# lh3/minimap2

Hardware: AMD Instinct MI355X
Metric: aligned Gbases/sec (map-ont, 10 kb reads, -a) (higher is better)
Workload: dtype int8 (ksw2 difference DP) / int32+f32 (chaining)

## Files before the change

### minimap2_amd/__init__.py

```python
import ctypes as C
import os

_HERE = os.path.dirname(os.path.abspath(__file__))
LIB_PATH = os.path.join(_HERE, "libmm2amd.so")


class Mm2AmdError(RuntimeError):
    pass


class KswJob(C.Structure):
    _fields_ = [("query", C.c_void_p), ("target", C.c_void_p), ("qlen", C.c_int32), ("tlen", C.c_int32), ("w", C.c_int32),
                ("zdrop", C.c_int32), ("end_bonus", C.c_int32), ("flag", C.c_int32)]


class FinJob(C.Structure):
    _fields_ = [("query", C.c_void_p), ("target", C.c_void_p), ("qlen", C.c_int32), ("tlen", C.c_int32), ("n_pieces", C.c_int32),
                ("piece", C.POINTER(C.POINTER(C.c_uint32))), ("piece_len", C.POINTER(C.c_int32))]


class FinRes(C.Structure):
    _fields_ = [("n_cigar", C.c_int32), ("blen", C.c_int32), ("mlen", C.c_int32), ("n_ambi", C.c_int32), ("dp_max", C.c_int32), ("qshift", C.c_int32),
                ("tshift", C.c_int32), ("is_spliced", C.c_int32), ("cigar_off", C.c_uint32)]

# ... 667 lines not shown
            q_staged.put(None)

        def mapper():
            try:
                k = 0
                while True:
                    b = q_staged.get()
                    if b is None:
                        break
                    m = max(1, len(b.items))
                    n_reg, reg, rep_len, frag_gap = (C.c_int * m)(), (C.c_void_p * m)(), (C.c_int * m)(), (C.c_int * m)()
                    t0 = time.time()
                    _check(L.mm_gpu_map_staged(n_reg, reg, rep_len, frag_gap))
                    if trace is not None:
                        trace.append(("map", k, t0, time.time()))
                    k += 1
                    q_mapped.put((b, n_reg, reg, rep_len))
            except Exception as e:
                errors.append(e)
                while True:
                    L.mm_gpu_batch_discard()
                    try:
                        if q_staged.get(timeout=0.05) is None:
                            break
                    except queue.Empty:
                        pass
            q_mapped.put(None)

        def output():
            k = -1
            while True:
                it = q_mapped.get()
                if it is None:
                    break
                b, n_reg, reg, rep_len = it
                k += 1
                t0 = time.time()
                try:
                    if not errors:
                        if on_mapped:
                            on_mapped(b, n_reg, reg, rep_len)
                        if text:
                            out, out_len = C.c_void_p(), C.c_size_t()
                            _check(L.mm_gpu_format_batch_view(b.n, b.seg_off, b.n_seg, b.arr, n_reg, reg, rep_len, C.byref(out), C.byref(out_len)))
                            total[0] += out_len.value
                            if on_text:
                                on_text(b, out.value, out_len.value)
                except Exception as e:
                    errors.append(e)
                t1 = time.time()
                L.mm2amd_free_regs(len(n_reg), n_reg, reg)
                if trace is not None:
                    trace.append(("output", k, t0, t1)), trace.append(("free", k, t1, time.time()))

        def named(f, nm):
            def g():
                try:
                    C.CDLL(None).prctl(15, nm, 0, 0, 0)
                except Exception:
                    pass
                f()
            return g
        th = [threading.Thread(target=named(f, nm)) for f, nm in ((stager, b"mm2-stager"), (mapper, b"mm2-mapper"), (output, b"mm2-output"))]
        for t in th:
            t.start()
        for t in th:
            t.join()
        self._staged = None
        if errors:
            raise errors[0]
        return total[0]

    def run(self, raw=False, cs=False, MD=False):
        if self._staged is None:
            raise Mm2AmdError("run() without stage()")
        self._active()
        n, _, items, seg_off, n_seg = self._staged
        m = max(1, len(items))
        n_reg, reg, rep_len, frag_gap = (C.c_int * m)(), (C.c_void_p * m)(), (C.c_int * m)(), (C.c_int * m)()
        _check(lib().mm_gpu_map_staged(n_reg, reg, rep_len, frag_gap))
        if raw:
            return n_reg, reg, rep_len
        out = []
        for i in range(n):
            per = []
            for k in range(seg_off[i], seg_off[i] + n_seg[i]):
                regs = C.cast(reg[k], C.POINTER(Reg1)) if n_reg[k] else None
                per.append(_regs_to_alignments(n_reg[k], regs, self.names, self.lens))
            out.append(per[0] if n_seg[i] == 1 else tuple(per))
        try:
            if cs or MD:
                flat = [a for per in out for seg in (per if isinstance(per, tuple) else (per,)) for a in seg]
                segs = [k for i in range(n) for k in range(seg_off[i], seg_off[i] + n_seg[i])]
                ptrs = [reg[k] + j * C.sizeof(Reg1) for k in segs for j in range(n_reg[k])]
                rds = [items[k][1] for k in segs for j in range(n_reg[k])]
                for want, what, field in ((cs, TXT_CS, "cs"), (MD, TXT_MD, "MD")):
                    if want and ptrs:
                        for a, t in zip(flat, hits_text(self._idx, ptrs, rds, what)):
                            setattr(a, field, t or "")
        finally:
            lib().mm2amd_free_regs(len(items), n_reg, reg)
        return out

    def free_raw(self, n_reg, reg):
        lib().mm2amd_free_regs(len(n_reg), n_reg, reg)

    def format_raw(self, n_reg, reg, rep_len=None, device=False):
        n, arr, _, seg_off, n_seg = self._staged
        out, out_len = C.c_void_p(), C.c_size_t()
        if device:
            path = C.c_int(-1)
            _check(lib().mm_gpu_format_batch_dev(n, seg_off, n_seg, arr, n_reg, reg, rep_len, C.byref(out), C.byref(out_len), C.byref(path)))
            self.last_format_path = path.value
            return C.string_at(out, out_len.value)
        _check(lib().mm_gpu_format_batch(n, seg_off, n_seg, arr, n_reg, reg, rep_len, C.byref(out), C.byref(out_len)))
        try:
            return C.string_at(out, out_len.value)
        finally:
            _libc_free(out)

    def map_batch(self, reads, cs=False, MD=False):
        self.stage(reads)
        return self.run(cs=cs, MD=MD)

    def map(self, seq, seq2=None, name="query", cs=False, MD=False):
        if seq2 is not None:
            return self.map_pairs([(name, seq, seq2)], cs=cs, MD=MD)[0]
        return self.map_batch([(name, seq)], cs=cs, MD=MD)[0]

    def seq(self, name, start=0, end=0x7fffffff):
        if not self._idx or self.index_stat()["flag"] & I_NO_SEQ or name not in self.names:
            return None
        rid = self.names.index(name)
        if start < 0 or start >= self.lens[rid] or start >= end:
            return None
        end = min(end, self.lens[rid])
        buf = C.create_string_buffer(end - start)
        rc = lib().mm2amd_idx_getseq(self._idx, rid, start, end, buf)
        if rc < 0:
            _check(rc)
        return buf.raw.translate(_CODE_TO_BASE).decode("ascii")

    def map_pairs(self, pairs, text=False, cs=False, MD=False):
        self.stage(pairs)
        if not text:
            return self.run(cs=cs, MD=MD)
        n_reg, reg, rep_len = self.run(raw=True)
        try:
            return self.format_raw(n_reg, reg, rep_len)
        finally:
            self.free_raw(n_reg, reg)

    def last_stats(self):
        v = (C.c_double * 40)()
        k = lib().mm2amd_last_stats(v, 40)
        names = ["t_seed_chain", "t_host_pre", "t_plan", "t_ksw", "t_consume", "t_finish", "n_jobs", "n_rounds", "dp_cells", "dev_allocs", "pin_allocs",
                 "alloc_ns", "cpu_seed_chain", "cpu_host_pre", "cpu_plan", "cpu_ksw", "cpu_consume", "cpu_finish", "n_long_join_dev", "n_long_join_host",
                 "drv_cpu_seed_chain", "drv_cpu_host_pre", "drv_cpu_plan", "drv_cpu_ksw", "drv_cpu_consume", "drv_cpu_finish", "n_early_sub",
                 "n_region_reads_dev", "n_region_reads_host", "n_band128", "n_band256", "n_band_widened", "n_band_rectangle",
                 "arena_dev_bytes", "arena_pin_bytes", "arena_dev_used", "arena_pin_used", "n_band512", "n_band_rectangle_big"]
        return dict(zip(names, list(v)[:k]))


def band_counters():
    L = lib()
    if not hasattr(L, "mm2amd_alloc_counter"):
        return {"band128": 0, "band256": 0, "widened": 0, "rectangle": 0, "band512": 0, "rectangle_big": 0}
    L.mm2amd_alloc_counter.restype = C.c_longlong
    L.mm2amd_alloc_counter.argtypes = [C.c_int]
    return {"band128": L.mm2amd_alloc_counter(3), "band256": L.mm2amd_alloc_counter(4), "widened": L.mm2amd_alloc_counter(5), "rectangle": L.mm2amd_alloc_counter(6),
            "band512": L.mm2amd_alloc_counter(11), "rectangle_big": L.mm2amd_alloc_counter(12)}


def profile_enable(on=True):
    lib().mm2amd_profile_enable(1 if on else 0)


def profile_get():
    arr = (KernelStat * 64)()
    n = lib().mm2amd_profile_get(arr, 64)
    return {arr[i].name.decode(): {"ms": arr[i].ms, "alg_bytes": arr[i].alg_bytes, "launches": arr[i].launches, "units": arr[i].units} for i in range(n)}
```

### minimap2_amd/csrc/backend_hip.cpp

```cpp
#include <atomic>
#include <condition_variable>
#include <algorithm>
#include <cstdio>
#include <cstring>
#include <memory>
#include <mutex>
#include <numeric>
#include <stdexcept>
#include <thread>
#include "backend.hpp"
#include "chain_dump.hpp"
#include "chain_host.hpp"
#include "device_ctx.hpp"
#include "ksw_host.hpp"
#include "seed_chain_dev.hpp"
#include "index_build.hpp"
#include "kernel_prof.hpp"
#include "threads.hpp"
#include "trace.hpp"
#include "sdust_core.hpp"
#include "sdust.hpp"

namespace mm2amd {

extern const uint8_t kNt4Table[256];

namespace {

bool env_on(const char *name) { const char *e = getenv(name); return e && *e && strcmp(e, "0") != 0; }

struct Lane {
	int id = 0;
	int set = 0;
	hipStream_t stream = nullptr;
	SeedChainBuffers B{};
	KswRunner ksw;
	DevBuf<uint64_t> d_a_off, d_mp_off, d_mz_x, d_mz_y, d_minipos, d_skey_in, d_sval_in, d_skey_out, d_sval_out;
	DevBuf<uint32_t> d_sdust_list;
	DevBuf<SdustCounters> d_sdust_cnt;
	PinBuf<SdustCounters> h_sdust_cnt;
	DevBuf<uint32_t> d_mz_cnt, d_sd_n, d_sd_off, d_sd_aoff, d_sd_qpos, d_sd_info, d_n_anchor, d_n_minipos, d_n_seedhit, d_tie;
	DevBuf<int32_t> d_rep_len, d_f, d_p, d_t;
	DevBuf<Anchor> d_anchors;
	DevBuf<uint8_t> d_tbytes;
	DevBuf<uint32_t> d_sort_list;
	PinBuf<uint32_t> h_sort_list;
	DevBuf<uint32_t> d_pieces;
	PinBuf<uint32_t> h_pieces, h_lj_pieces;
	DevBuf<Anchor> d_lj_out_a;
	DevBuf<uint64_t> d_lj_src;
	PinBuf<Anchor> h_lj_a;
	PinBuf<uint64_t> h_lj_u, h_lj_off, h_lj_aoff, h_lj_uoff;
	PinBuf<int32_t> h_lj_nu, h_lj_nv;
	PinBuf<uint32_t> h_lj_tie, h_lj_list;
	PinBuf<unsigned long long> h_lj_cursor;
	DevBuf<FinRegion> d_fin_regions; DevBuf<FinPiece> d_fin_pieces; DevBuf<uint32_t> d_fin_out; DevBuf<FinResult> d_fin_res;
	PinBuf<FinRegion> h_fin_regions; PinBuf<FinPiece> h_fin_pieces; PinBuf<uint32_t> h_fin_out; PinBuf<FinResult> h_fin_res;
	long rg_lo = 0; size_t rg_n = 0; uint64_t rg_n_v = 0, rg_n_v2 = 0, rg_n_u = 0, rg_n_u2 = 0;
	std::vector<int8_t> rg_src; std::vector<uint64_t> rg_aoff, rg_uoff; std::vector<int32_t> rg_nu, rg_nv;
	DevBuf<uint64_t> d_lj_out_u;
	bool rg_lazy = false;
	DevBuf<int32_t> d_span; PinBuf<int32_t> h_span;
	DevBuf<RgnGather> d_gather; PinBuf<RgnGather> h_gather; DevBuf<Anchor> d_fetch_a; DevBuf<uint64_t> d_fetch_mp; PinBuf<Anchor> h_fetch_a; PinBuf<uint64_t> h_fetch_mp;
	DevBuf<RgnRead> d_rg_reads; PinBuf<RgnRead> h_rg_reads;
	DevBuf<Anchor> d_rg_sq; DevBuf<ref::Reg1> d_rg_regs; DevBuf<RgnAux> d_rg_aux; DevBuf<RgnReadOut> d_rg_rout; DevBuf<unsigned int> d_rg_cur;
	DevBuf<RgnPlan> d_rg_plan; DevBuf<RgnWin> d_rg_win; DevBuf<KswJob> d_rg_jobs; DevBuf<int32_t> d_rg_sites; DevBuf<FinRegion> d_rg_fin; DevBuf<FinPiece> d_rg_pieces;
	DevBuf<FinResult> d_rg_finres; DevBuf<uint32_t> d_rg_out;
	PinBuf<ref::Reg1> h_rg_regs; PinBuf<RgnAux> h_rg_aux; PinBuf<RgnReadOut> h_rg_rout; PinBuf<unsigned int> h_rg_cur; PinBuf<RgnPlan> h_rg_plan; PinBuf<KswJob> h_rg_jobs;
	PinBuf<FinRegion> h_rg_fin; PinBuf<FinResult> h_rg_finres; PinBuf<uint32_t> h_rg_out;
	PinBuf<Anchor> h_anchors, h_redo;
	PinBuf<int32_t> h_rep, h_nu, h_nv;
	PinBuf<uint64_t> h_minipos, h_off, h_u, h_aoff, h_uoff;
	PinBuf<unsigned long long> h_cursor;
	DevBuf<unsigned long long> d_bt_cursor;
	DevBuf<Anchor> d_bt_out_a;
	DevBuf<uint64_t> d_bt_out_u, d_bt_aoff, d_bt_uoff;
	DevBuf<int32_t> d_bt_nu, d_bt_nv;
	PinBuf<uint32_t> h_na, h_nmp, h_dust_n, h_dust_s, h_dust_e, h_tie;
	std::vector<uint64_t> a_off, mp_off;
	~Lane() { if (stream) (void)hipStreamDestroy(stream); }
};

class HipBackend : public Backend {
public:
	HipBackend(const FlatIndex &fi, DeviceIndexTables *tables, int n_threads, int device, int replica, int tables_device) : T_(tables)
	{
		replica_ = replica;
		DeviceCtx &d = device_ctx(device);
		std::lock_guard<std::mutex> lk(d.mu);
		ensure_device(d);
		dev_ = d.device_id;
		stream_ = d.stream;
		n_cu_ = d.n_cu;
		n_threads_ = n_threads > 0 ? n_threads : (int)std::max(1u, std::thread::hardware_concurrency());
		if (!T_) { own_.upload(fi, stream_); T_ = &own_; }
		else if (tables_device >= 0 && tables_device != dev_) { own_.clone_from(*T_, tables_device, dev_); T_ = &own_; }
		I_.bucket_start = T_->bucket_start.p, I_.keys = T_->keys.p, I_.val_off = T_->val_off.p, I_.slots = T_->slots.p, I_.first = getenv("MM2AMD_NO_FIRST_SLOT") ? nullptr : T_->first.p, I_.pos = T_->pos.p, I_.S = T_->S.p;
		I_.bucket_bits = T_->bucket_bits, I_.key_shift = T_->key_shift;
		I_.name_rank = nullptr, I_.seq_len = nullptr;
		fi_names_ = &fi.names, fi_seq_len_ = &fi.seq_len, fi_seq_off_ = &fi.seq_off;
		while ((1ull << rid_bits_) < fi.n_seq) ++rid_bits_;
		n_lanes_ = 8;
		if (const char *e = getenv("MM2AMD_LANES")) n_lanes_ = std::max(1, std::min(kMaxProfLanes - 1, atoi(e)));
		for (int i = 0; i < n_lanes_; ++i) {
			lanes_.emplace_back(new Lane);
			lanes_.back()->id = i;
			HIP_CHECK(hipStreamCreateWithFlags(&lanes_.back()->stream, hipStreamNonBlocking));
			lanes_.back()->ksw.n_cu = n_cu_;
			lanes_.back()->ksw.disable_fast = getenv("MM2AMD_KSW_EXACT_ONLY") != nullptr;
		}
		{
			size_t free_b = 0, total_b = 0, want = arena_env_gb("MM2AMD_ARENA_DEV_GB", 112) << 30;
			if (hipMemGetInfo(&free_b, &total_b) == hipSuccess) want = std::min(want, free_b / 2);
			const size_t want_pin = arena_env_gb("MM2AMD_ARENA_PIN_GB", 4) << 30;
			const int dev = dev_;
			if (MemArena::enabled() && (want || want_pin)) std::thread([dev, want, want_pin] {
				if (hipSetDevice(dev) != hipSuccess) return;
				try { pin_arena().reserve(want_pin); dev_arena().reserve(want); } catch (...) {}
			}).detach();
		}
	}

	~HipBackend() override
	{
		(void)hipSetDevice(dev_);
		if (stage_stream_) (void)hipStreamDestroy(stage_stream_);
		for (int l = 0; l < n_lanes_; ++l) kernel_profiler(l, replica_).drop_events();
		kernel_profiler(kMaxProfLanes - 1, replica_).drop_events();
	}
	int n_lanes() const override { return n_lanes_; }
	void enable_name_rules() override
	{
		HIP_CHECK(hipSetDevice(dev_));
		if (name_rules_ || fi_names_->empty()) return;
		const std::vector<std::string> &nm = *fi_names_;
		sorted_names_ = nm;
		std::sort(sorted_names_.begin(), sorted_names_.end());
		sorted_names_.erase(std::unique(sorted_names_.begin(), sorted_names_.end()), sorted_names_.end());
		std::vector<int32_t> rank(nm.size());
		for (size_t i = 0; i < nm.size(); ++i) rank[i] = (int32_t)(std::lower_bound(sorted_names_.begin(), sorted_names_.end(), nm[i]) - sorted_names_.begin());
		d_name_rank_.ensure(nm.size()), d_ref_len_.ensure(nm.size());
		HIP_CHECK(hipMemcpyAsync(d_name_rank_.p, rank.data(), nm.size() * 4, hipMemcpyHostToDevice, stream_));
		HIP_CHECK(hipMemcpyAsync(d_ref_len_.p, fi_seq_len_->data(), nm.size() * 4, hipMemcpyHostToDevice, stream_));
		stream_wait(stream_);
		I_.name_rank = d_name_rank_.p, I_.seq_len = d_ref_len_.p;
		name_rules_ = true;
	}
	void enable_seq_len() override
	{
		HIP_CHECK(hipSetDevice(dev_));
		if (I_.seq_len) return;
		d_ref_len_.ensure(fi_seq_len_->size());
		HIP_CHECK(hipMemcpyAsync(d_ref_len_.p, fi_seq_len_->data(), fi_seq_len_->size() * 4, hipMemcpyHostToDevice, stream_));
		stream_wait(stream_);
		I_.seq_len = d_ref_len_.p;
	}
	bool supports_rmq() const override { return getenv("MM2AMD_RMQ_ON_HOST") == nullptr; }
	void set_active_lanes(int n) override { active_lanes_ = std::max(1, std::min(n, n_lanes_)); }

	void begin_batch(const std::vector<ReadView> &reads, std::vector<uint64_t> &qpool_off) override
	{
		HIP_CHECK(hipSetDevice(dev_));
		Resident &R = res_[1 - cur_];
		if (!stage_stream_) HIP_CHECK(hipStreamCreateWithFlags(&stage_stream_, hipStreamNonBlocking));
		hipStream_t stream_ = stage_stream_;
		std::vector<uint64_t> &seq_off_ = R.seq_off, &unit_off_ = R.unit_off;
		std::vector<int32_t> &unit_first_ = R.unit_first, &name_key_ = R.name_key;
		bool &has_pairs_ = R.has_pairs, &have_read_names_ = R.have_read_names;
		size_t &n_units_ = R.n_units;
		PinBuf<char> &h_ascii_ = R.h_ascii;
		DevBuf<uint8_t> &d_qpool_ = R.d_qpool;
		DevBuf<uint64_t> &d_seq_off_ = R.d_seq_off, &d_unit_off_ = R.d_unit_off;
		DevBuf<int32_t> &d_unit_first_ = R.d_unit_first, &d_name_key_ = R.d_name_key;
		std::vector<const char *> &read_names_ = R.read_names;
		const size_t n = reads.size();
		seq_off_.resize(n + 1);
		seq_off_[0] = 0;
		has_pairs_ = false;
		for (size_t i = 0; i < n; ++i) seq_off_[i + 1] = seq_off_[i] + (uint64_t)reads[i].total(), has_pairs_ |= reads[i].paired();
		const uint64_t total = seq_off_[n];
		qpool_off.resize(n);
		for (size_t i = 0; i < n; ++i) qpool_off[i] = 2 * seq_off_[i];
		char *h = h_ascii_.ensure(total + 1);
		parallel_for_side(n_threads_, (long)n, [&](long i, int) {
			memcpy(h + seq_off_[i], reads[i].seq, reads[i].len);
			if (reads[i].paired()) memcpy(h + seq_off_[i] + reads[i].len, reads[i].seq2, reads[i].len2);
		}, 64);
		d_qpool_.ensure(2 * total + 16);
		d_seq_off_.ensure(n + 1);
		n_units_ = n;
		if (has_pairs_) {
			unit_first_.resize(n + 1);
			unit_first_[0] = 0;
			for (size_t i = 0; i < n; ++i) unit_first_[i + 1] = unit_first_[i] + (reads[i].paired() ? 2 : 1);
			n_units_ = (size_t)unit_first_[n];
			unit_off_.resize(n_units_ + 1);
			for (size_t i = 0; i < n; ++i) {
				unit_off_[unit_first_[i]] = seq_off_[i];
				if (reads[i].paired()) unit_off_[unit_first_[i] + 1] = seq_off_[i] + (uint64_t)reads[i].len;
			}
			unit_off_[n_units_] = total;
			d_unit_off_.ensure(n_units_ + 1), d_unit_first_.ensure(n + 1);
			HIP_CHECK(hipMemcpyAsync(d_unit_off_.p, unit_off_.data(), (n_units_ + 1) * 8, hipMemcpyHostToDevice, stream_));
			HIP_CHECK(hipMemcpyAsync(d_unit_first_.p, unit_first_.data(), (n + 1) * 4, hipMemcpyHostToDevice, stream_));
		}
		HIP_CHECK(hipMemcpyAsync(d_seq_off_.p, seq_off_.data(), (n + 1) * 8, hipMemcpyHostToDevice, stream_));
		read_names_.clear();
		if (getenv("MM2AMD_SEED_DUMP") || chain_dump_path()) for (size_t i = 0; i < n; ++i) read_names_.push_back(reads[i].name);
		have_read_names_ = false;
		if (name_rules_ && n > 0) {
			have_read_names_ = true;
			for (size_t i = 0; i < n; ++i) if (!reads[i].name) { have_read_names_ = false; break; }
		}
		if (have_read_names_) {
			name_key_.resize(2 * n);
			parallel_for_side(n_threads_, (long)n, [&](long i, int) {
				const std::string q(reads[i].name);
				const size_t lb = (size_t)(std::lower_bound(sorted_names_.begin(), sorted_names_.end(), q) - sorted_names_.begin());
				name_key_[i] = (int32_t)lb;
				name_key_[n + i] = lb < sorted_names_.size() && sorted_names_[lb] == q ? (int32_t)lb : -1;
			}, 256);
			d_name_key_.ensure(2 * n);
			HIP_CHECK(hipMemcpyAsync(d_name_key_.p, name_key_.data(), 2 * n * 4, hipMemcpyHostToDevice, stream_));
		}
		stream_wait(stream_);
	}
	void activate_batch() override { cur_ = 1 - cur_; }
	int current_set() const override { return cur_; }
	void bind_lane(int lane, int set) override { lanes_.at(lane)->set = set; }
	bool stages_beside_mapping() const override { return true; }

	void seed_chain(const SeedChainParams &P, long lo, long hi, int lane_id, int n_threads, std::vector<ReadChains> &out) override
	{
		HIP_CHECK(hipSetDevice(dev_));
		Lane &ln = *lanes_.at(lane_id);
		hipStream_t st = ln.stream;
		SeedChainBuffers &B = ln.B;
		const Resident &R = res_[ln.set];
		const std::vector<uint64_t> &seq_off_ = R.seq_off, &unit_off_ = R.unit_off;
		const std::vector<int32_t> &unit_first_ = R.unit_first;
		const bool has_pairs_ = R.has_pairs, have_read_names_ = R.have_read_names;
		const DevBuf<uint8_t> &d_qpool_ = R.d_qpool;
		const DevBuf<uint64_t> &d_seq_off_ = R.d_seq_off, &d_unit_off_ = R.d_unit_off;
		const DevBuf<int32_t> &d_unit_first_ = R.d_unit_first, &d_name_key_ = R.d_name_key;
		const PinBuf<char> &h_ascii_ = R.h_ascii;
		const std::vector<const char *> &read_names_ = R.read_names;
		const size_t n = (size_t)(hi - lo);
		out.clear();
		out.resize(n);
		if (n == 0) return;
		B = SeedChainBuffers();
		B.n_reads = (int)n, B.seq_off = d_seq_off_.p + lo, B.ascii = h_ascii_.p, B.qpool = d_qpool_.p;
		if (have_read_names_) B.name_lb = d_name_key_.p + lo, B.name_eq = d_name_key_.p + seq_off_.size() - 1 + lo;
		KernelProfiler &kp = kernel_profiler(lane_id, replica_);
		double tt = Trace::now();
		const double L = (double)(seq_off_[hi] - seq_off_[lo]);
		SeedChainBuffers Bu = B;
		const size_t ulo = has_pairs_ ? (size_t)unit_first_[lo] : (size_t)lo, n_unit = has_pairs_ ? (size_t)unit_first_[hi] - ulo : n;
		if (has_pairs_) Bu.n_reads = (int)n_unit, Bu.seq_off = d_unit_off_.p + ulo;
		kp.begin(st); launch_encode(Bu, st); kp.end(st, "encode_kernel", 3 * L);
		const uint64_t base0 = seq_off_[lo], cap_mz = seq_off_[hi] - base0;
		ln.d_mz_cnt.ensure(n_unit);
		ln.d_mz_x.ensure(cap_mz + 1), ln.d_mz_y.ensure(cap_mz + 1);
		ln.d_sd_n.ensure(cap_mz + 1), ln.d_sd_off.ensure(cap_mz + 1), ln.d_sd_aoff.ensure(cap_mz + 1), ln.d_sd_qpos.ensure(cap_mz + 1), ln.d_sd_info.ensure(cap_mz + 1);
		B.mz_cnt = ln.d_mz_cnt.p, B.mz_off = B.seq_off, B.mz_x = ln.d_mz_x.p - base0, B.mz_y = ln.d_mz_y.p - base0;
		B.sd_n = ln.d_sd_n.p - base0, B.sd_off = ln.d_sd_off.p - base0, B.sd_aoff = ln.d_sd_aoff.p - base0, B.sd_qpos = ln.d_sd_qpos.p - base0, B.sd_info = ln.d_sd_info.p - base0;
		const double est_mz = 2.0 * L / (P.w + 1);
		Bu.mz_cnt = B.mz_cnt, Bu.mz_off = Bu.seq_off, Bu.mz_x = B.mz_x, Bu.mz_y = B.mz_y;
		int max_len = 0;
		for (size_t u = 0; u < n_unit; ++u) {
			const uint64_t l_u = has_pairs_ ? unit_off_[ulo + u + 1] - unit_off_[ulo + u] : seq_off_[lo + u + 1] - seq_off_[lo + u];
			max_len = (int)std::max<uint64_t>((uint64_t)max_len, l_u);
		}
		kp.begin(st); launch_sketch(Bu, P, max_len, st); kp.end(st, "sketch_kernel", L + 16.0 * est_mz);
		if (has_pairs_)
			B.unit_first = d_unit_first_.p + lo, B.unit_off = d_unit_off_.p, B.unit_cnt = ln.d_mz_cnt.p - ulo, B.mz_cnt = nullptr;
		const bool dev_sdust = P.sdust_thres > 0 && env_on("MM2AMD_DEVICE_SDUST"), sdust_no_narrow = env_on("MM2AMD_SDUST_NO_NARROW");
		if (dev_sdust) {
			ln.d_sdust_list.ensure(n_unit), ln.d_sdust_cnt.ensure(1);
			HIP_CHECK(hipMemsetAsync(ln.d_sdust_cnt.p, 0, sizeof(SdustCounters), st));
			SdustParams S;
			S.codes = B.qpool, S.off = Bu.seq_off, S.code_mul = 2, S.n_reads = (int)n_unit, S.T = P.sdust_thres < kSdustMaxT ? P.sdust_thres : kSdustMaxT;
			S.reg_n = B.sd_n, S.reg_s = B.sd_off, S.reg_e = B.sd_aoff, S.wide_list = ln.d_sdust_list.p, S.cnt = ln.d_sdust_cnt.p;
			const char *e_cap = getenv("MM2AMD_SDUST_NARROW_CAP");
			const long cap = e_cap && *e_cap ? strtol(e_cap, nullptr, 10) : kSdustNarrowCap;
			if (sdust_no_narrow) {
				S.cap = kSdustWideCap, S.wide = 2;
				kp.begin(st); sdust_launch(S, 0, st); kp.end(st, "sdust_kernel[wide]", 0.0);
			} else {
				S.cap = (int)(cap < 1 ? 1 : cap > kSdustWideCap ? kSdustWideCap : cap), S.wide = 0;
				kp.begin(st); sdust_launch(S, 0, st); kp.end(st, "sdust_kernel[narrow]", 0.0);
				S.cap = kSdustWideCap, S.wide = 1;
				kp.begin(st); sdust_launch(S, 0, st); kp.end(st, "sdust_kernel[wide]", 0.0);
			}
			HIP_CHECK(hipMemcpyAsync(ln.h_sdust_cnt.ensure(1), ln.d_sdust_cnt.p, sizeof(SdustCounters), hipMemcpyDeviceToHost, st));
			kp.begin(st); launch_dust_filter(B, st); kp.end(st, "dust_filter_kernel", 16.0 * est_mz);
		} else if (P.sdust_thres > 0) {
			uint32_t *h_n = ln.h_dust_n.ensure(cap_mz + 1), *h_s = ln.h_dust_s.ensure(cap_mz + 1), *h_e = ln.h_dust_e.ensure(cap_mz + 1);
			const char *asc = h_ascii_.p;
			parallel_for(n_threads, (long)n_unit, [&](long u, int) {
				const uint64_t o = has_pairs_ ? unit_off_[ulo + u] : seq_off_[lo + u];
				const int len = (int)((has_pairs_ ? unit_off_[ulo + u + 1] : seq_off_[lo + u + 1]) - o);
				thread_local std::vector<SdustState::Perf> perf(SdustState::PCAP);
				thread_local std::vector<uint8_t> codes;
				codes.resize((size_t)len + 1);
				for (int j = 0; j < len; ++j) codes[j] = kNt4Table[(uint8_t)asc[o + j]];
				SdustState S;
				S.P = perf.data();
				uint32_t k = 0;
				sdust_scan(codes.data(), len, P.sdust_thres, S, [&](int s0, int e0) { h_s[o - base0 + k] = (uint32_t)s0, h_e[o - base0 + k] = (uint32_t)e0; ++k; });
				if (len > 0) h_n[o - base0] = k;
			}, 16);
			HIP_CHECK(hipMemcpyAsync(ln.d_sd_n.p, h_n, cap_mz * 4, hipMemcpyHostToDevice, st));
			HIP_CHECK(hipMemcpyAsync(ln.d_sd_off.p, h_s, cap_mz * 4, hipMemcpyHostToDevice, st));
			HIP_CHECK(hipMemcpyAsync(ln.d_sd_aoff.p, h_e, cap_mz * 4, hipMemcpyHostToDevice, st));
			kp.begin(st); launch_dust_filter(B, st); kp.end(st, "dust_filter_kernel", 16.0 * est_mz);
		}
		ln.d_n_anchor.ensure(n), ln.d_n_minipos.ensure(n), ln.d_n_seedhit.ensure(n), ln.d_rep_len.ensure(n);
		B.n_anchor = ln.d_n_anchor.p, B.n_minipos = ln.d_n_minipos.p, B.n_seedhit = ln.d_n_seedhit.p, B.rep_len = ln.d_rep_len.p;
		kp.begin(st); launch_seed_collect(B, I_, P, st); kp.end(st, "seed_collect_kernel", 36.0 * est_mz);
		uint32_t *h_na = ln.h_na.ensure(n), *h_nmp = ln.h_nmp.ensure(n);
		int32_t *h_rep = ln.h_rep.ensure(n);
		HIP_CHECK(hipMemcpyAsync(h_na, ln.d_n_anchor.p, n * 4, hipMemcpyDeviceToHost, st));
		HIP_CHECK(hipMemcpyAsync(h_nmp, ln.d_n_minipos.p, n * 4, hipMemcpyDeviceToHost, st));
		HIP_CHECK(hipMemcpyAsync(h_rep, ln.d_rep_len.p, n * 4, hipMemcpyDeviceToHost, st));
		stream_wait(st);
		if (dev_sdust) {
			const SdustCounters &c = *ln.h_sdust_cnt.p;
			if (c.err) throw HipError("[mm2amd] sdust_kernel: a list of perfect intervals outgrew the wide capacity");
			kp.add_units("sdust_kernel[wide]", (double)c.wide_bases);
			if (!sdust_no_narrow) kp.add_units("sdust_kernel[narrow]", L - (double)c.wide_bases + (double)c.narrow_partial);
		}
		Trace::get().add(lane_id, "gpu:sketch+collect", tt, Trace::now()); tt = Trace::now();
		std::vector<uint64_t> &a_off = ln.a_off, &mp_off = ln.mp_off;
		a_off.resize(n + 1), mp_off.resize(n + 1);
		a_off[0] = mp_off[0] = 0;
		for (size_t i = 0; i < n; ++i) a_off[i + 1] = a_off[i] + h_na[i], mp_off[i + 1] = mp_off[i] + h_nmp[i];
		const uint64_t n_a = a_off[n], n_mp = mp_off[n];
		uint64_t *h_off = ln.h_off.ensure(2 * (n + 1));
		memcpy(h_off, a_off.data(), (n + 1) * 8), memcpy(h_off + n + 1, mp_off.data(), (n + 1) * 8);
		ln.d_a_off.ensure(n + 1), ln.d_mp_off.ensure(n + 1);
		HIP_CHECK(hipMemcpyAsync(ln.d_a_off.p, h_off, (n + 1) * 8, hipMemcpyHostToDevice, st));
		HIP_CHECK(hipMemcpyAsync(ln.d_mp_off.p, h_off + n + 1, (n + 1) * 8, hipMemcpyHostToDevice, st));
		ln.d_anchors.ensure(n_a + 1), ln.d_minipos.ensure(n_mp + 1), ln.d_f.ensure(n_a + 1), ln.d_p.ensure(n_a + 1), ln.d_t.ensure(n_a + 1);
		ln.d_skey_in.ensure(n_a + 1), ln.d_sval_in.ensure(n_a + 1), ln.d_skey_out.ensure(n_a + 1), ln.d_sval_out.ensure(n_a + 1), ln.d_tie.ensure(2 * n + 1);
		B.sort_key_in = ln.d_skey_in.p, B.sort_val_in = ln.d_sval_in.p, B.sort_key_out = ln.d_skey_out.p, B.sort_val_out = ln.d_sval_out.p, B.tie_flag = ln.d_tie.p;
		B.tie_list = ln.d_tie.p + n, B.tie_count = ln.d_tie.p + 2 * n;
		B.rid_bits = rid_bits_;
		int n_class[kAnchorSortClasses] = { 0 }, class_first[kAnchorSortClasses + 1] = { 0 };
		double a_class[kAnchorSortClasses] = { 0 };
		for (size_t i = 0; i < n; ++i) if (h_na[i]) { const int c = anchor_sort_class(h_na[i], rid_bits_); ++n_class[c], a_class[c] += h_na[i]; }
		for (int c = 0; c < kAnchorSortClasses; ++c) class_first[c + 1] = class_first[c] + n_class[c];
		uint32_t *h_list = ln.h_sort_list.ensure(n + 1);
		{
			int fill[kAnchorSortClasses];
			for (int c = 0; c < kAnchorSortClasses; ++c) fill[c] = class_first[c];
			for (size_t i = 0; i < n; ++i) if (h_na[i]) h_list[fill[anchor_sort_class(h_na[i], rid_bits_)]++] = (uint32_t)i;
		}
		ln.d_sort_list.ensure(n + 1);
		if (class_first[kAnchorSortClasses]) HIP_CHECK(hipMemcpyAsync(ln.d_sort_list.p, h_list, (size_t)class_first[kAnchorSortClasses] * 4, hipMemcpyHostToDevice, st));
		B.a_off = ln.d_a_off.p, B.mp_off = ln.d_mp_off.p, B.anchors = ln.d_anchors.p, B.mini_pos = ln.d_minipos.p;
		B.f = ln.d_f.p, B.p = ln.d_p.p, B.t = ln.d_t.p;
		kp.begin(st); launch_seed_expand(B, I_, P, st); kp.end(st, "seed_expand_kernel", 24.0 * n_a);
		launch_anchor_sort(B, I_, P, ln.d_sort_list.p, n_class, a_class, st, &kp);
		if (getenv("MM2AMD_TIE_COUNT")) {
			std::vector<uint32_t> tf(n);
			stream_wait(st);
			HIP_CHECK(hipMemcpy(tf.data(), ln.d_tie.p, n * 4, hipMemcpyDeviceToHost));
			size_t n_tied = 0;
			for (size_t i = 0; i < n; ++i) n_tied += tf[i] != 0;
			fprintf(stderr, "[mm2amd] anchor sort: %zu of %zu reads have duplicated keys (%d / %d / %d reads in the 7 k / 10 k / global classes)\n", n_tied, n, n_class[3], n_class[4], n_class[5]);
		}
		if (const char *dump = getenv("MM2AMD_SEED_DUMP")) {
			std::vector<Anchor> all(n_a + 1);
			stream_wait(st);
			if (n_a) HIP_CHECK(hipMemcpy(all.data(), ln.d_anchors.p, n_a * sizeof(Anchor), hipMemcpyDeviceToHost));
			static std::mutex dump_mu;
			std::lock_guard<std::mutex> lk(dump_mu);
			const bool dump_flags = getenv("MM2AMD_SEED_DUMP_FLAGS") != nullptr;
			if (FILE *fp = fopen(dump, "a")) {
				for (size_t i = 0; i < n; ++i) {
					fprintf(fp, "QR\t%s\t%d\nRS\t%d\n", read_names_.empty() || !read_names_[lo + i] ? "*" : read_names_[lo + i], P.mid_occ, h_rep[i]);
					for (uint64_t j = a_off[i]; j < a_off[i + 1]; ++j) {
						const Anchor &a = all[j];
						fprintf(fp, "SD\t%s\t%d\t%c\t%d\t%d\t%d", (*fi_names_)[a.x << 1 >> 33].c_str(), (int32_t)a.x, "+-"[a.x >> 63], (int32_t)a.y, (int32_t)(a.y >> 32 & 0xff),
						        j == a_off[i] ? 0 : ((int32_t)a.y - (int32_t)all[j - 1].y) - ((int32_t)a.x - (int32_t)all[j - 1].x));
						if (dump_flags) fprintf(fp, "\t%d", (int)(a.y >> 42 & 1));
						fputc('\n', fp);
					}
				}
				fclose(fp);
			}
		}
		const char *cdump = P.chain_dump ? chain_dump_path() : nullptr;
		auto dump_block = [&](size_t i) {
			ChainDumpBlock b;
			b.name = read_names_.empty() ? nullptr : read_names_[lo + i];
			b.qlen = (int)(seq_off_[lo + i + 1] - seq_off_[lo + i]), b.n_seg = has_pairs_ ? unit_first_[lo + i + 1] - unit_first_[lo + i] : 1;
			return b;
		};
		if (P.anchors_only) {
			Anchor *ha = ln.h_anchors.ensure(n_a + 1);
			uint64_t *hmp = ln.h_minipos.ensure(n_mp + 1);
			if (n_a) HIP_CHECK(hipMemcpyAsync(ha, ln.d_anchors.p, n_a * sizeof(Anchor), hipMemcpyDeviceToHost, st));
			if (n_mp) HIP_CHECK(hipMemcpyAsync(hmp, ln.d_minipos.p, n_mp * 8, hipMemcpyDeviceToHost, st));
			stream_wait(st);
			Trace::get().add(lane_id, "gpu:expand+sort, d2h:anchors", tt, Trace::now());
			kp.collect();
			if (cdump) {
				std::string txt;
				for (size_t i = 0; i < n; ++i) {
					ChainDumpBlock b = dump_block(i);
					b.handed_back = true, b.in = ha + a_off[i], b.n_in = (int64_t)(a_off[i + 1] - a_off[i]);
					chain_dump_format(txt, P, b);
				}
				chain_dump_flush(cdump, txt);
			}
			parallel_for(n_threads, (long)n, [&](long i, int) {
				ReadChains &c = out[i];
				c.rep_len = h_rep[i];
				c.mp_p = hmp + mp_off[i], c.n_mp = (int32_t)(mp_off[i + 1] - mp_off[i]);
				c.u_p = nullptr, c.n_u = 0, c.chained = false;
				c.a_p = ha + a_off[i], c.n_a = (int64_t)(a_off[i + 1] - a_off[i]);
			}, 64);
			return;
		}
		make_pieces(B, ln, ln.h_pieces, n, [&](size_t i) { return (uint64_t)h_na[i]; }, P.rmq ? rmq_piece_len() : fill_piece_len(), st);
		if (P.rmq) { kp.begin(st); launch_chain_rmq(B, P, st); kp.end(st, "chain_rmq_kernel", 32.0 * n_a); }
		else { kp.begin(st); launch_chain_fill(B, P, st); kp.end(st, "chain_fill_kernel", 24.0 * n_a); }
		B.pieces = nullptr, B.n_pieces = 0;
		ln.d_bt_cursor.ensure(2), ln.d_bt_out_a.ensure(n_a + 1), ln.d_bt_out_u.ensure((P.min_cnt >= 2 ? n_a / 2 : n_a) + n + 1);
		ln.d_bt_nu.ensure(n), ln.d_bt_nv.ensure(n), ln.d_bt_aoff.ensure(n), ln.d_bt_uoff.ensure(n);
		B.bt_cursor = ln.d_bt_cursor.p, B.bt_out_a = ln.d_bt_out_a.p, B.bt_out_u = ln.d_bt_out_u.p;
		B.bt_nu = ln.d_bt_nu.p, B.bt_nv = ln.d_bt_nv.p, B.bt_aoff = ln.d_bt_aoff.p, B.bt_uoff = ln.d_bt_uoff.p;
		kp.begin(st); launch_chain_backtrack(B, P, st); kp.end(st, "chain_backtrack_kernel", 8.0 * n_a);
		unsigned long long *h_cur = ln.h_cursor.ensure(2);
		int32_t *h_nu = ln.h_nu.ensure(n), *h_nv = ln.h_nv.ensure(n);
		uint64_t *h_aoff = ln.h_aoff.ensure(n), *h_uoff = ln.h_uoff.ensure(n);
		uint64_t *hmp = ln.h_minipos.ensure(n_mp + 1);
		uint32_t *h_tie = P.rmq ? ln.h_tie.ensure(n) : nullptr;
		HIP_CHECK(hipMemcpyAsync(h_cur, ln.d_bt_cursor.p, 16, hipMemcpyDeviceToHost, st));
		HIP_CHECK(hipMemcpyAsync(h_nu, ln.d_bt_nu.p, n * 4, hipMemcpyDeviceToHost, st));
		HIP_CHECK(hipMemcpyAsync(h_nv, ln.d_bt_nv.p, n * 4, hipMemcpyDeviceToHost, st));
		HIP_CHECK(hipMemcpyAsync(h_aoff, ln.d_bt_aoff.p, n * 8, hipMemcpyDeviceToHost, st));
		HIP_CHECK(hipMemcpyAsync(h_uoff, ln.d_bt_uoff.p, n * 8, hipMemcpyDeviceToHost, st));
		if (h_tie) HIP_CHECK(hipMemcpyAsync(h_tie, ln.d_tie.p, n * 4, hipMemcpyDeviceToHost, st));
		const bool lazy = P.lazy_chains != 0 && !P.anchors_only;
		ln.rg_lazy = lazy;
		int32_t *h_span = nullptr;
		if (lazy) {
			ln.d_span.ensure(2 * n), h_span = ln.h_span.ensure(2 * n);
			launch_first_chain_span((int)n, ln.d_bt_out_a.p, ln.d_bt_out_u.p, ln.d_bt_aoff.p, ln.d_bt_uoff.p, ln.d_bt_nu.p, ln.d_span.p, st);
			HIP_CHECK(hipMemcpyAsync(h_span, ln.d_span.p, 2 * n * 4, hipMemcpyDeviceToHost, st));
		} else if (n_mp) HIP_CHECK(hipMemcpyAsync(hmp, ln.d_minipos.p, n_mp * 8, hipMemcpyDeviceToHost, st));
		stream_wait(st);
		Trace::get().add(lane_id, "gpu:expand..backtrack", tt, Trace::now()); tt = Trace::now();
		const uint64_t n_v = h_cur[0], n_u = h_cur[1];
		Anchor *ha = ln.h_anchors.ensure(n_v + 1);
		uint64_t *hu = ln.h_u.ensure(n_u + 1);
		if (n_v && !lazy) HIP_CHECK(hipMemcpyAsync(ha, ln.d_bt_out_a.p, n_v * sizeof(Anchor), hipMemcpyDeviceToHost, st));
		if (n_u) HIP_CHECK(hipMemcpyAsync(hu, ln.d_bt_out_u.p, n_u * 8, hipMemcpyDeviceToHost, st));
		std::vector<std::pair<size_t, size_t>> redo;
		size_t redo_total = 0;
		if (h_tie) for (size_t i = 0; i < n; ++i) if (h_tie[i]) redo.emplace_back(i, redo_total), redo_total += (size_t)(a_off[i + 1] - a_off[i]);
		Anchor *h_redo = redo_total ? ln.h_redo.ensure(redo_total + 1) : nullptr;
		for (const auto &rd : redo) {
			const size_t cnt = (size_t)(a_off[rd.first + 1] - a_off[rd.first]);
			if (cnt) HIP_CHECK(hipMemcpyAsync(h_redo + rd.second, ln.d_anchors.p + a_off[rd.first], cnt * sizeof(Anchor), hipMemcpyDeviceToHost, st));
			const size_t n_pos = (size_t)(mp_off[rd.first + 1] - mp_off[rd.first]);
			if (lazy && n_pos) HIP_CHECK(hipMemcpyAsync(hmp + mp_off[rd.first], ln.d_minipos.p + mp_off[rd.first], n_pos * 8, hipMemcpyDeviceToHost, st));
		}
		stream_wait(st);
		if (cdump) {
			std::vector<Anchor> all(n_a + 1), bt(lazy ? n_v + 1 : 0);
			if (n_a) HIP_CHECK(hipMemcpyAsync(all.data(), ln.d_anchors.p, n_a * sizeof(Anchor), hipMemcpyDeviceToHost, st));
			if (lazy && n_v) HIP_CHECK(hipMemcpyAsync(bt.data(), ln.d_bt_out_a.p, n_v * sizeof(Anchor), hipMemcpyDeviceToHost, st));
			stream_wait(st);
			const Anchor *chained = lazy ? bt.data() : ha;
			std::string txt;
			for (size_t i = 0; i < n; ++i) {
				ChainDumpBlock b = dump_block(i);
				b.in = all.data() + a_off[i], b.n_in = (int64_t)(a_off[i + 1] - a_off[i]);
				b.handed_back = h_tie && h_tie[i];
				if (!b.handed_back) b.u = hu + h_uoff[i], b.n_u = h_nu[i], b.a = chained + h_aoff[i], b.n_a = h_nv[i];
				chain_dump_format(txt, P, b);
			}
			chain_dump_flush(cdump, txt);
		}
		Trace::get().add(lane_id, "d2h:chains", tt, Trace::now()); tt = Trace::now();
		kp.collect();
		TraceScope ts(lane_id, "host:chains->vectors");
		parallel_for(n_threads, (long)n, [&](long i, int) {
			ReadChains &c = out[i];
			c.rep_len = h_rep[i];
			c.mp_p = lazy ? nullptr : hmp + mp_off[i], c.n_mp = (int32_t)(mp_off[i + 1] - mp_off[i]);
			c.u_p = hu + h_uoff[i], c.n_u = h_nu[i];
			c.a_p = lazy ? nullptr : ha + h_aoff[i], c.n_a = h_nv[i];
			c.chained = true;
		}, 64);
		ln.rg_lo = lo, ln.rg_n = n, ln.rg_n_v = n_v, ln.rg_n_u = n_u, ln.rg_n_v2 = ln.rg_n_u2 = 0;
		for (size_t i = 0; i < n; ++i) out[i].dev_src = 0, out[i].dev_a_off = h_aoff[i], out[i].dev_u_off = h_uoff[i];
		for (const auto &rd : redo) {
			ReadChains &c = out[rd.first];
			c.u_p = nullptr, c.n_u = 0, c.chained = false, c.dev_src = -1;
			c.mp_p = hmp + mp_off[rd.first];
			c.a_p = h_redo + rd.second, c.n_a = (int64_t)(a_off[rd.first + 1] - a_off[rd.first]);
		}
		if (P.long_join && !has_pairs_ && !getenv("MM2AMD_LONG_JOIN_ON_HOST")) long_join(P, lo, n, ln, kp, out, ha, hu, h_nu, h_nv, h_aoff, h_uoff, h_span, cdump);
	}

	static int fill_piece_len() { const char *e = getenv("MM2AMD_CHAIN_PIECE"); return e ? atoi(e) : 4096; }
	static int rmq_piece_len() { const char *e = getenv("MM2AMD_RMQ_PIECE"); return e ? atoi(e) : 512; }
	template <class Count>
	static void make_pieces(SeedChainBuffers &B, Lane &ln, PinBuf<uint32_t> &hbuf, size_t n, Count count, int len, hipStream_t st)
	{
		B.pieces = nullptr, B.n_pieces = 0, B.piece_len = len;
		{ const char *e = getenv("MM2AMD_RMQ_RANK_MAX"); B.rmq_rank_max = e ? std::min(256, std::max(0, atoi(e))) : 256; }
		{ const char *e = getenv("MM2AMD_RMQ_DENSE"); B.piece_dense = e ? atoi(e) : 1024; }
		if (len <= 0) return;
		size_t n_p = 0;
		bool any = false;
		for (size_t i = 0; i < n; ++i) { const uint64_t c = count(i); n_p += (size_t)((c + len - 1) / len); any |= c > (uint64_t)len; }
		if (!any || n_p > (size_t)INT32_MAX) return;
		uint32_t *h = hbuf.ensure(2 * n_p);
		size_t k = 0;
		for (int pass = 0; pass < 2; ++pass)
			for (size_t i = 0; i < n; ++i) {
				const uint64_t c = count(i), m = (c + len - 1) / len;
				if (m == 0 || (m > 1) != (pass == 0)) continue;
				for (uint64_t q = 0; q < m; ++q) h[2 * k] = (uint32_t)i, h[2 * k + 1] = (uint32_t)q, ++k;
			}
		ln.d_pieces.ensure(2 * n_p);
		HIP_CHECK(hipMemcpyAsync(ln.d_pieces.p, h, 2 * n_p * 4, hipMemcpyHostToDevice, st));
		B.pieces = ln.d_pieces.p, B.n_pieces = (int)n_p;
		if (getenv("MM2AMD_PIECE_DEBUG")) fprintf(stderr, "[mm2amd] chaining work list: %zu reads in %zu pieces of %d anchors\n", n, n_p, len);
	}

	void long_join(const SeedChainParams &P, long lo, size_t n, Lane &ln, KernelProfiler &kp, std::vector<ReadChains> &out, const Anchor *ha, const uint64_t *hu,
	               const int32_t *h_nu, const int32_t *h_nv, const uint64_t *h_aoff, const uint64_t *h_uoff, const int32_t *h_span, const char *cdump)
	{
		const bool lazy = h_span != nullptr;
		hipStream_t st = ln.stream;
		const std::vector<uint64_t> &seq_off = res_[ln.set].seq_off;
		std::vector<uint32_t> sel;
		for (size_t i = 0; i < n; ++i) {
			ReadChains &c = out[i];
			if (!c.chained) continue;
			c.long_join_done = true;
			if (h_nu[i] <= 1) continue;
			const int qlen = (int)(seq_off[lo + i + 1] - seq_off[lo + i]);
			const int32_t a0 = lazy ? h_span[2 * i] : (int32_t)ha[h_aoff[i]].y, a1 = lazy ? h_span[2 * i + 1] : (int32_t)ha[h_aoff[i] + (uint64_t)((int32_t)hu[h_uoff[i]] - 1)].y;
			if (qlen - (a1 - a0) > P.rmq_rescue_size || a1 - a0 > qlen * P.rmq_rescue_ratio) sel.push_back((uint32_t)i);
		}
		const size_t n2 = sel.size();
		if (n2 == 0) return;
		uint64_t *h_off = ln.h_lj_off.ensure(2 * (n2 + 1));
		uint64_t *h_src = h_off + n2 + 1;
		h_off[0] = 0;
		for (size_t k = 0; k < n2; ++k) h_off[k + 1] = h_off[k] + (uint64_t)h_nv[sel[k]], h_src[k] = h_aoff[sel[k]];
		const uint64_t n_a2 = h_off[n2];
		SeedChainBuffers B2 = ln.B;
		B2.n_reads = (int)n2, B2.seq_off = nullptr, B2.mz_cnt = nullptr, B2.unit_first = nullptr;
		ln.d_lj_src.ensure(n2 + 1), ln.d_lj_out_a.ensure(n_a2 + 1);
		HIP_CHECK(hipMemcpyAsync(ln.d_a_off.p, h_off, (n2 + 1) * 8, hipMemcpyHostToDevice, st));
		HIP_CHECK(hipMemcpyAsync(ln.d_lj_src.p, h_src, n2 * 8, hipMemcpyHostToDevice, st));
		B2.a_off = ln.d_a_off.p;
		int n_class[kAnchorSortClasses] = { 0 }, class_first[kAnchorSortClasses + 1] = { 0 };
		double a_class[kAnchorSortClasses] = { 0 };
		for (size_t k = 0; k < n2; ++k) { const int c = anchor_sort_class((uint64_t)h_nv[sel[k]], rid_bits_); ++n_class[c], a_class[c] += h_nv[sel[k]]; }
		for (int c = 0; c < kAnchorSortClasses; ++c) class_first[c + 1] = class_first[c] + n_class[c];
		uint32_t *h_list = ln.h_lj_list.ensure(n2 + 1);
		{
			int fill[kAnchorSortClasses];
			for (int c = 0; c < kAnchorSortClasses; ++c) fill[c] = class_first[c];
			for (size_t k = 0; k < n2; ++k) h_list[fill[anchor_sort_class((uint64_t)h_nv[sel[k]], rid_bits_)]++] = (uint32_t)k;
		}
		HIP_CHECK(hipMemcpyAsync(ln.d_sort_list.p, h_list, n2 * 4, hipMemcpyHostToDevice, st));
		kp.begin(st); launch_rechain_gather(B2, ln.d_bt_out_a.p, ln.d_lj_src.p, st); kp.end(st, "rechain_gather_kernel", 32.0 * n_a2);
		SeedChainParams P2 = P;
		P2.rmq = 1, P2.bw = P.bw_long, P2.flag &= ~(int64_t)ref::F_HEAP_SORT;
		launch_anchor_sort(B2, I_, P2, ln.d_sort_list.p, n_class, a_class, st, &kp);
		make_pieces(B2, ln, ln.h_lj_pieces, n2, [&](size_t k) { return (uint64_t)h_nv[sel[k]]; }, rmq_piece_len(), st);
		kp.begin(st); launch_chain_rmq(B2, P2, st); kp.end(st, "chain_rmq_kernel[long-join]", 32.0 * n_a2);
		ln.d_lj_out_u.ensure((P2.min_cnt >= 2 ? n_a2 / 2 : n_a2) + n2 + 1);
		B2.bt_out_a = ln.d_lj_out_a.p, B2.bt_out_u = ln.d_lj_out_u.p;
		kp.begin(st); launch_chain_backtrack(B2, P2, st); kp.end(st, "chain_backtrack_kernel[long-join]", 8.0 * n_a2);
		unsigned long long *h_cur = ln.h_lj_cursor.ensure(2);
		int32_t *nu2 = ln.h_lj_nu.ensure(n2), *nv2 = ln.h_lj_nv.ensure(n2);
		uint64_t *aoff2 = ln.h_lj_aoff.ensure(n2), *uoff2 = ln.h_lj_uoff.ensure(n2);
		uint32_t *tie2 = ln.h_lj_tie.ensure(n2);
		HIP_CHECK(hipMemcpyAsync(h_cur, ln.d_bt_cursor.p, 16, hipMemcpyDeviceToHost, st));
		HIP_CHECK(hipMemcpyAsync(nu2, ln.d_bt_nu.p, n2 * 4, hipMemcpyDeviceToHost, st));
		HIP_CHECK(hipMemcpyAsync(nv2, ln.d_bt_nv.p, n2 * 4, hipMemcpyDeviceToHost, st));
		HIP_CHECK(hipMemcpyAsync(aoff2, ln.d_bt_aoff.p, n2 * 8, hipMemcpyDeviceToHost, st));
		HIP_CHECK(hipMemcpyAsync(uoff2, ln.d_bt_uoff.p, n2 * 8, hipMemcpyDeviceToHost, st));
		HIP_CHECK(hipMemcpyAsync(tie2, ln.d_tie.p, n2 * 4, hipMemcpyDeviceToHost, st));
		stream_wait(st);
		const uint64_t n_v2 = h_cur[0], n_u2 = h_cur[1];
		Anchor *ha2 = ln.h_lj_a.ensure(n_v2 + 1);
		uint64_t *hu2 = ln.h_lj_u.ensure(n_u2 + 1);
		if (n_v2 && !lazy) HIP_CHECK(hipMemcpyAsync(ha2, ln.d_lj_out_a.p, n_v2 * sizeof(Anchor), hipMemcpyDeviceToHost, st));
		if (n_u2) HIP_CHECK(hipMemcpyAsync(hu2, ln.d_lj_out_u.p, n_u2 * 8, hipMemcpyDeviceToHost, st));
		ln.rg_n_v2 = n_v2, ln.rg_n_u2 = n_u2;
		stream_wait(st);
		kp.collect();
		if (cdump) {
			std::vector<Anchor> bt(lazy ? n_v2 + 1 : 0);
			if (lazy && n_v2) {
				HIP_CHECK(hipMemcpyAsync(bt.data(), ln.d_lj_out_a.p, n_v2 * sizeof(Anchor), hipMemcpyDeviceToHost, st));
				stream_wait(st);
			}
			const Anchor *chained = lazy ? bt.data() : ha2;
			const Resident &R = res_[ln.set];
			std::string txt;
			for (size_t k = 0; k < n2; ++k) {
				const size_t i = sel[k];
				ChainDumpBlock b;
				b.name = R.read_names.empty() ? nullptr : R.read_names[lo + i];
				b.qlen = (int)(seq_off[lo + i + 1] - seq_off[lo + i]), b.pass = 2, b.handed_back = tie2[k] != 0;
				if (!b.handed_back) b.u = hu2 + uoff2[k], b.n_u = nu2[k], b.a = chained + aoff2[k], b.n_a = nv2[k];
				chain_dump_format(txt, P, b);
			}
			chain_dump_flush(cdump, txt);
		}
		for (size_t k = 0; k < n2; ++k) {
			ReadChains &c = out[sel[k]];
			if (tie2[k]) { c.long_join_done = false; continue; }
			c.u_p = hu2 + uoff2[k], c.n_u = nu2[k];
			c.a_p = lazy ? nullptr : ha2 + aoff2[k], c.n_a = nv2[k];
			c.long_joined = true;
			c.dev_src = 1, c.dev_a_off = aoff2[k], c.dev_u_off = uoff2[k];
		}
	}

	void ksw(const std::vector<KswJob> &jobs, const KswScoring &sc, int lane_id, int n_threads, std::vector<KswRes> &res, const uint32_t **cigar) override
	{
		HIP_CHECK(hipSetDevice(dev_));
		Lane &ln = *lanes_.at(lane_id);
		res.resize(jobs.size());
		size_t n_cig = 0;
		ln.ksw.n_threads = n_threads;
		ln.ksw.prof = &kernel_profiler(lane_id, replica_);
		size_t dir_gb = 160;
		if (const char *e = getenv("MM2AMD_DIR_BUDGET_GB")) dir_gb = atol(e) > 0 ? (size_t)atol(e) : dir_gb;
		ln.ksw.dir_budget = std::min<size_t>((dir_gb << 30) / (size_t)active_lanes_, (size_t)96 << 30);
		ln.ksw.lane = lane_id;
		const uint8_t *d_tbytes = nullptr;
		if (sc.n_tbytes) {
			ln.d_tbytes.ensure(sc.n_tbytes + 1);
			HIP_CHECK(hipMemcpyAsync(ln.d_tbytes.p, sc.tbytes, sc.n_tbytes, hipMemcpyHostToDevice, ln.stream));
			d_tbytes = ln.d_tbytes.p;
		}
		ln.ksw.run(jobs, res_[ln.set].d_qpool.p, d_tbytes, T_->S.p, sc, res.data(), cigar, &n_cig, ln.stream);
		kernel_profiler(lane_id, replica_).collect();
	}

	void fetch_chains(int lane_id, const std::vector<long> &reads, std::vector<ReadChains> &chains) override
	{
		if (reads.empty()) return;
		HIP_CHECK(hipSetDevice(dev_));
		Lane &ln = *lanes_.at(lane_id);
		hipStream_t st = ln.stream;
		RgnGather *g = ln.h_gather.ensure(reads.size());
		uint64_t na = 0, nmp = 0;
		for (size_t k = 0; k < reads.size(); ++k) {
			const ReadChains &c = chains[reads[k]];
			RgnGather &G = g[k];
			G.a_src = c.dev_a_off, G.a_dst = na, G.mp_src = ln.mp_off[reads[k]], G.mp_dst = nmp;
			G.n_a = (int32_t)c.n_a, G.n_mp = c.n_mp, G.src = c.dev_src == 1 ? 1u : 0u, G.pad = 0;
			na += (uint64_t)c.n_a, nmp += (uint64_t)c.n_mp;
		}
		ln.d_gather.ensure(reads.size()), ln.d_fetch_a.ensure(na + 1), ln.d_fetch_mp.ensure(nmp + 1);
		Anchor *ha = ln.h_fetch_a.ensure(na + 1);
		uint64_t *hmp = ln.h_fetch_mp.ensure(nmp + 1);
		HIP_CHECK(hipMemcpyAsync(ln.d_gather.p, g, reads.size() * sizeof(RgnGather), hipMemcpyHostToDevice, st));
		launch_gather_chains((int)reads.size(), ln.d_gather.p, ln.d_bt_out_a.p, ln.d_lj_out_a.p, ln.d_minipos.p, ln.d_fetch_a.p, ln.d_fetch_mp.p, st);
		if (na) HIP_CHECK(hipMemcpyAsync(ha, ln.d_fetch_a.p, na * sizeof(Anchor), hipMemcpyDeviceToHost, st));
		if (nmp) HIP_CHECK(hipMemcpyAsync(hmp, ln.d_fetch_mp.p, nmp * 8, hipMemcpyDeviceToHost, st));
		stream_wait(st);
		for (size_t k = 0; k < reads.size(); ++k) {
			ReadChains &c = chains[reads[k]];
			c.a_p = ha + g[k].a_dst, c.mp_p = hmp + g[k].mp_dst;
		}
	}

	bool aligns_regions() const override
	{
		const char *e = getenv("MM2AMD_DEVICE_REGIONS");
		return !(e && *e == '0');
	}
	void align_regions(int lane_id, const RgnOpts &O, const KswScoring &sc, bool log_gap, const std::vector<ReadChains> &chains, const std::vector<RegionReadIn> &in, int n_threads,
	                   RegionBatchOut &out) override
	{
		HIP_CHECK(hipSetDevice(dev_));
		Lane &ln = *lanes_.at(lane_id);
		hipStream_t st = ln.stream;
		const Resident &R = res_[ln.set];
		const size_t n = ln.rg_n;
		out = RegionBatchOut();
		if (n == 0 || chains.size() < n || in.size() < n) return;
		if (!ref_ready_.load(std::memory_order_acquire)) {
			std::lock_guard<std::mutex> lk(ref_mu_);
			if (!ref_ready_.load(std::memory_order_relaxed)) {
				d_ref_off_.ensure(fi_seq_off_->size() + 1), d_ref_len2_.ensure(fi_seq_len_->size() + 1);
				HIP_CHECK(hipMemcpyAsync(d_ref_off_.p, fi_seq_off_->data(), fi_seq_off_->size() * 8, hipMemcpyHostToDevice, st));
				HIP_CHECK(hipMemcpyAsync(d_ref_len2_.p, fi_seq_len_->data(), fi_seq_len_->size() * 4, hipMemcpyHostToDevice, st));
				stream_wait(st);
				ref_ready_.store(true, std::memory_order_release);
			}
		}
		KernelProfiler &kp = kernel_profiler(lane_id, replica_);
		double tt = Trace::now();
		RgnRead *hr = ln.h_rg_reads.ensure(n);
		uint64_t sq = 0, n_chain = 0;
		int max_nu = 1;
// ... 119 lines not shown
	void finish_regions(int lane_id, const std::vector<FinRegion> &regions, const std::vector<FinPiece> &pieces, size_t out_words, const int8_t *mat25, int q, int e, bool log_gap,
	                    std::vector<FinResult> &results, const uint32_t **cigars) override
	{
		HIP_CHECK(hipSetDevice(dev_));
		Lane &ln = *lanes_.at(lane_id);
		const size_t n = regions.size();
		results.resize(n);
		*cigars = nullptr;
		if (n == 0) return;
		memcpy(ln.h_fin_regions.ensure(n), regions.data(), n * sizeof(FinRegion));
		memcpy(ln.h_fin_pieces.ensure(pieces.size() + 1), pieces.data(), pieces.size() * sizeof(FinPiece));
		ln.d_fin_regions.ensure(n), ln.d_fin_pieces.ensure(pieces.size() + 1), ln.d_fin_out.ensure(out_words + 1), ln.d_fin_res.ensure(n);
		ln.h_fin_out.ensure(out_words + 1), ln.h_fin_res.ensure(n);
		HIP_CHECK(hipMemcpyAsync(ln.d_fin_regions.p, ln.h_fin_regions.p, n * sizeof(FinRegion), hipMemcpyHostToDevice, ln.stream));
		HIP_CHECK(hipMemcpyAsync(ln.d_fin_pieces.p, ln.h_fin_pieces.p, pieces.size() * sizeof(FinPiece), hipMemcpyHostToDevice, ln.stream));
		FinParams P;
		P.regions = ln.d_fin_regions.p, P.n_regions = (int)n, P.pieces = ln.d_fin_pieces.p, P.cigar_pool = ln.ksw.d_cigar.p, P.out_pool = ln.d_fin_out.p, P.results = ln.d_fin_res.p;
		P.qpool = res_[ln.set].d_qpool.p, P.S = T_->S.p;
		memcpy(P.mat, mat25, 25);
		P.q = (int8_t)q, P.e = (int8_t)e, P.log_gap = log_gap ? 1 : 0;
		uint32_t longest = 1;
		for (size_t i = 0; i < n; ++i) longest = std::max<uint32_t>(longest, (uint32_t)((i + 1 < n ? regions[i + 1].out_off : (uint32_t)out_words) - regions[i].out_off));
		P.cap_ops = (int)std::min<uint32_t>((longest + 63) & ~63u, (uint32_t)kFinMaxOps);
		KernelProfiler &prof = kernel_profiler(lane_id, replica_);
		prof.begin(ln.stream);
		region_finish_launch(P, ln.stream);
		prof.end(ln.stream, "region_finish_kernel", (double)out_words * 8.0 + (double)n * (sizeof(FinRegion) + sizeof(FinResult)), (double)n);
		HIP_CHECK(hipMemcpyAsync(ln.h_fin_res.p, ln.d_fin_res.p, n * sizeof(FinResult), hipMemcpyDeviceToHost, ln.stream));
		HIP_CHECK(hipMemcpyAsync(ln.h_fin_out.p, ln.d_fin_out.p, out_words * sizeof(uint32_t), hipMemcpyDeviceToHost, ln.stream));
		stream_wait(ln.stream);
		memcpy(results.data(), ln.h_fin_res.p, n * sizeof(FinResult));
		*cigars = ln.h_fin_out.p;
		static const bool check = getenv("MM2AMD_FIN_CHECK") != nullptr;
		if (check)
			for (size_t i = 0; i < n; ++i) {
				const FinResult &f = results[i];
				long q = f.qshift, t = f.tshift;
				for (int k = 0; k < f.n_cigar; ++k) {
					const uint32_t c = ln.h_fin_out.p[regions[i].out_off + k], op = c & 0xf, len = c >> 4;
					if (op == 0 || op == 7 || op == 8) q += len, t += len;
					else if (op == 1) q += len;
					else if (op == 2 || op == 3) t += len;
				}
				if (f.n_cigar < 0 || q != regions[i].q_len || t != regions[i].t_len)
					fprintf(stderr, "[mm2amd] FIN_CHECK lane %d region %zu of %zu: n_cigar %d qshift %d tshift %d covers %ld/%ld of %d/%d (pieces %u from %u, out_off %u)\n", lane_id, i, n,
					        f.n_cigar, f.qshift, f.tshift, q, t, regions[i].q_len, regions[i].t_len, regions[i].n_pieces, regions[i].piece0, regions[i].out_off);
			}
		prof.collect();
	}

	bool writes_records() const override { return true; }
	RecTextBufs rec_text_begin(const RecTextSizes &sz) override
	{
		HIP_CHECK(hipSetDevice(dev_));
		RecText &R = rt_;
		if (!R.stream) HIP_CHECK(hipStreamCreateWithFlags(&R.stream, hipStreamNonBlocking));
		if (!R.targets_ready) {
			const size_t n_seq = fi_seq_len_->size();
			uint64_t tot = 0;
			for (size_t i = 0; i < n_seq; ++i) tot += (*fi_names_)[i].size();
			char *nm = R.h_tnames.ensure(tot + 1);
			uint64_t *to = R.h_tname_off.ensure(n_seq + 1);
			uint32_t *tl = R.h_tlen.ensure(n_seq + 1);
			tot = 0;
			for (size_t i = 0; i < n_seq; ++i) {
				to[i] = tot, tl[i] = (*fi_seq_len_)[i];
				memcpy(nm + tot, (*fi_names_)[i].data(), (*fi_names_)[i].size());
				tot += (*fi_names_)[i].size();
			}
			to[n_seq] = tot;
			R.d_tnames.ensure(tot + 1), R.d_tname_off.ensure(n_seq + 1), R.d_tlen.ensure(n_seq + 1);
			if (tot) HIP_CHECK(hipMemcpyAsync(R.d_tnames.p, nm, tot, hipMemcpyHostToDevice, R.stream));
			HIP_CHECK(hipMemcpyAsync(R.d_tname_off.p, to, (n_seq + 1) * 8, hipMemcpyHostToDevice, R.stream));
			if (n_seq) HIP_CHECK(hipMemcpyAsync(R.d_tlen.p, tl, n_seq * 4, hipMemcpyHostToDevice, R.stream));
			stream_wait(R.stream);
			R.targets_ready = true;
		}
		R.sz = sz;
		RecTextBufs b;
		b.jobs = R.h_jobs.ensure(sz.n_jobs + 1), b.hits = R.h_hits.ensure(sz.n_hits + 1), b.names = R.h_names.ensure(sz.name_bytes + 1);
		b.q = R.h_q.ensure(sz.q_bytes + 1), b.cigar = R.h_cigar.ensure(sz.cigar_words + 1), b.off = R.h_off.ensure(sz.n_jobs + 1);
		R.h_res.ensure(sz.n_jobs + 1);
		return b;
	}
	const RecRes *rec_text_size(int64_t flag) override
	{
		HIP_CHECK(hipSetDevice(dev_));
		RecText &R = rt_;
		const RecTextSizes &sz = R.sz;
		if (sz.n_jobs == 0) return R.h_res.p;
		R.d_jobs.ensure(sz.n_jobs), R.d_hits.ensure(sz.n_hits + 1), R.d_names.ensure(sz.name_bytes + 1), R.d_q.ensure(sz.q_bytes + 1), R.d_cigar.ensure(sz.cigar_words + 1);
		R.d_res.ensure(sz.n_jobs), R.d_off.ensure(sz.n_jobs);
		HIP_CHECK(hipMemcpyAsync(R.d_jobs.p, R.h_jobs.p, sz.n_jobs * sizeof(RecJob), hipMemcpyHostToDevice, R.stream));
		if (sz.n_hits) HIP_CHECK(hipMemcpyAsync(R.d_hits.p, R.h_hits.p, sz.n_hits * sizeof(RecHit), hipMemcpyHostToDevice, R.stream));
		if (sz.name_bytes) HIP_CHECK(hipMemcpyAsync(R.d_names.p, R.h_names.p, sz.name_bytes, hipMemcpyHostToDevice, R.stream));
		if (sz.q_bytes) HIP_CHECK(hipMemcpyAsync(R.d_q.p, R.h_q.p, sz.q_bytes, hipMemcpyHostToDevice, R.stream));
		if (sz.cigar_words) HIP_CHECK(hipMemcpyAsync(R.d_cigar.p, R.h_cigar.p, sz.cigar_words * 4, hipMemcpyHostToDevice, R.stream));
		RecParams &P = R.P;
		P.jobs = R.d_jobs.p, P.n_jobs = (int)sz.n_jobs, P.hits = R.d_hits.p, P.flag = flag, P.names = R.d_names.p, P.qpool = R.d_q.p, P.S = T_->S.p, P.cigar = R.d_cigar.p;
		P.tnames = R.d_tnames.p, P.tname_off = R.d_tname_off.p, P.tlen = R.d_tlen.p, P.res = R.d_res.p, P.off = nullptr, P.out = nullptr;
		KernelProfiler &prof = kernel_profiler(kMaxProfLanes - 1, replica_);
		prof.begin(R.stream);
		rec_text_launch(P, false, R.stream);
		prof.end(R.stream, "rec_text_kernel[size]", (double)sz.cigar_words * 4.0 + (double)sz.q_bytes, (double)sz.n_jobs);
		HIP_CHECK(hipMemcpyAsync(R.h_res.p, R.d_res.p, sz.n_jobs * sizeof(RecRes), hipMemcpyDeviceToHost, R.stream));
		stream_wait(R.stream);
		prof.collect();
		return R.h_res.p;
	}
	const char *rec_text_write(uint64_t total) override
	{
		HIP_CHECK(hipSetDevice(dev_));
		RecText &R = rt_;
		const RecTextSizes &sz = R.sz;
		R.h_out.ensure(total + 1);
		if (sz.n_jobs == 0 || total == 0) return R.h_out.p;
		R.d_out.ensure(total + 8);
		HIP_CHECK(hipMemcpyAsync(R.d_off.p, R.h_off.p, sz.n_jobs * 8, hipMemcpyHostToDevice, R.stream));
		R.P.off = R.d_off.p, R.P.out = R.d_out.p;
		KernelProfiler &prof = kernel_profiler(kMaxProfLanes - 1, replica_);
		prof.begin(R.stream);
		rec_text_launch(R.P, true, R.stream);
		prof.end(R.stream, "rec_text_kernel[write]", (double)total + (double)sz.cigar_words * 4.0 + (double)sz.q_bytes, (double)sz.n_jobs);
		HIP_CHECK(hipMemcpyAsync(R.h_out.p, R.d_out.p, total, hipMemcpyDeviceToHost, R.stream));
		stream_wait(R.stream);
		prof.collect();
		return R.h_out.p;
	}

private:
	struct RecText {
		hipStream_t stream = nullptr;
		bool targets_ready = false;
		RecTextSizes sz;
		RecParams P{};
		PinBuf<char> h_tnames; PinBuf<uint64_t> h_tname_off; PinBuf<uint32_t> h_tlen;
		DevBuf<char> d_tnames; DevBuf<uint64_t> d_tname_off; DevBuf<uint32_t> d_tlen;
		PinBuf<RecJob> h_jobs; PinBuf<RecHit> h_hits; PinBuf<char> h_names; PinBuf<uint8_t> h_q; PinBuf<uint32_t> h_cigar; PinBuf<uint64_t> h_off; PinBuf<RecRes> h_res; PinBuf<char> h_out;
		DevBuf<RecJob> d_jobs; DevBuf<RecHit> d_hits; DevBuf<char> d_names; DevBuf<uint8_t> d_q; DevBuf<uint32_t> d_cigar; DevBuf<uint64_t> d_off; DevBuf<RecRes> d_res; DevBuf<char> d_out;
		~RecText() { if (stream) (void)hipStreamDestroy(stream); }
	};
	RecText rt_;
	struct DpGate {
		HipBackend &b;
		explicit DpGate(HipBackend &be) : b(be) { if (b.dp_gate_ > 0) { std::unique_lock<std::mutex> lk(b.gate_mu_); b.gate_cv_.wait(lk, [&] { return b.gate_in_ < b.dp_gate_; }); ++b.gate_in_; } }
		~DpGate() { if (b.dp_gate_ > 0) { { std::lock_guard<std::mutex> lk(b.gate_mu_); --b.gate_in_; } b.gate_cv_.notify_one(); } }
	};
	int dp_gate_ = getenv("MM2AMD_DP_GATE") ? atoi(getenv("MM2AMD_DP_GATE")) : 4, gate_in_ = 0;
	std::mutex gate_mu_;
	std::condition_variable gate_cv_;
	hipStream_t stream_ = nullptr;
	int n_threads_ = 1, n_cu_ = 256, n_lanes_ = 1, rid_bits_ = 1, dev_ = 0, replica_ = 0;
	std::atomic<int> active_lanes_{1};
	DevIndex I_{};
	DeviceIndexTables own_;
	DeviceIndexTables *T_ = nullptr;
	std::vector<std::unique_ptr<Lane>> lanes_;
	struct Resident {
		DevBuf<uint8_t> d_qpool;
		DevBuf<uint64_t> d_seq_off;
		PinBuf<char> h_ascii;
		std::vector<uint64_t> seq_off;
		bool has_pairs = false;
		size_t n_units = 0;
		std::vector<uint64_t> unit_off;
		std::vector<int32_t> unit_first;
		DevBuf<uint64_t> d_unit_off;
		DevBuf<int32_t> d_unit_first;
		bool have_read_names = false;
		std::vector<int32_t> name_key;
		DevBuf<int32_t> d_name_key;
		std::vector<const char *> read_names;
	};
	Resident res_[2];
	int cur_ = 0;
	hipStream_t stage_stream_ = nullptr;
	bool name_rules_ = false;
	const std::vector<std::string> *fi_names_ = nullptr;
	const std::vector<uint32_t> *fi_seq_len_ = nullptr;
	const std::vector<uint64_t> *fi_seq_off_ = nullptr;
	DevBuf<uint64_t> d_ref_off_;
	DevBuf<uint32_t> d_ref_len2_;
	std::mutex ref_mu_;
	std::atomic<bool> ref_ready_{false};
	std::vector<std::string> sorted_names_;
	DevBuf<int32_t> d_name_rank_;
	DevBuf<uint32_t> d_ref_len_;
};

}

Backend *make_backend(const FlatIndex &fi, void *device_tables, int n_threads, int device, int replica, int tables_device)
{
	return new HipBackend(fi, (DeviceIndexTables *)device_tables, n_threads, device, replica, tables_device);
}
void apply_hw_queue_default();
int backend_device_count() { apply_hw_queue_default(); int n = 0; return hipGetDeviceCount(&n) == hipSuccess ? n : 0; }

void *backend_build_index_tables(FlatIndex &fi, int device, int *on_device)
{
	DeviceCtx &d = device_ctx(device);
	std::lock_guard<std::mutex> lk(d.mu);
	ensure_device(d);
	std::unique_ptr<DeviceIndexTables> T(new DeviceIndexTables);
	DeviceIndexBuilder::build_from_packed(fi, *T, d.stream);
	if (on_device) *on_device = d.device_id;
	return T.release();
}
void backend_free_index_tables(void *tables) { delete (DeviceIndexTables *)tables; }
const char *backend_name() { return "hip:gfx950"; }

}
```

### minimap2_amd/csrc/capi_kernels.cpp

```cpp
#include <mutex>
#include <string>
#include <vector>
#include <cstring>
#include "../../include/mm2amd.h"
#include "hip_util.hpp"
#include "device_ctx.hpp"
#include "ksw_host.hpp"
#include "kernel_prof.hpp"
#include "region_finish.hpp"
#include "aln_text.hpp"
#include "ksw_ll.hpp"
#include "sdust.hpp"
#include "sdust_core.hpp"
#include "threads.hpp"
#include "trace.hpp"
#include "device_sort.hpp"
#include "seed_chain_dev.hpp"
#include <map>

namespace mm2amd { int capi_fail(int code, const std::string &msg); }
using namespace mm2amd;
namespace mm2amd { extern const uint8_t kNt4Table[256]; }

namespace {
// ... 474 lines not shown
				P.cap = kSdustWideCap, P.wide = 1;
				prof.begin(dc.stream);
				sdust_launch(P, (int)std::min<uint32_t>(hc.n_wide, (uint32_t)kSdustWideGrid), dc.stream);
				prof.end(dc.stream, "sdust_kernel[wide]", 0.0, 0.0);
				HIP_CHECK(hipStreamSynchronize(dc.stream));
				for (uint32_t k = 0; k < hc.n_wide; ++k) {
					if (h_list[k] >= (uint32_t)n_jobs) return fail(MM2AMD_EHIP, "[mm2amd] sdust_batch: the device listed a job outside the batch");
					res[h_list[k]].path = MM2AMD_SDUST_PATH_WIDE, wide_bases += (double)jobs[h_list[k]].len;
				}
				prof.add_units("sdust_kernel[wide]", wide_bases);
			}
			prof.add_units("sdust_kernel[narrow]", (double)total - wide_bases + (double)hc.narrow_partial);
		}
		sdust_count_launch(P, d.d_cnt_out.p, dc.stream);
		uint32_t *const h_n = h_list + n;
		HIP_CHECK(hipMemcpyAsync(h_n, d.d_cnt_out.p, n * 4, hipMemcpyDeviceToHost, dc.stream));
		HIP_CHECK(hipMemcpyAsync(&hc, d.d_cnt.p, sizeof hc, hipMemcpyDeviceToHost, dc.stream));
		HIP_CHECK(hipStreamSynchronize(dc.stream));
		prof.collect();
		if (hc.err) return fail(MM2AMD_EHIP, "[mm2amd] sdust_batch: a list of perfect intervals outgrew the wide capacity");
		uint64_t *const out_off = h_off + n + 1;
		uint64_t n_out = 0;
		for (size_t i = 0; i < n; ++i) {
			if (h_n[i] > (uint32_t)jobs[i].len) return fail(MM2AMD_EHIP, "[mm2amd] sdust_batch: more regions than bases");
			out_off[i] = n_out, res[i].off = n_out, res[i].n = h_n[i];
			n_out += h_n[i];
		}
		if (!pool || n_out == 0) return 0;
		if (n_out > pool_cap) return fail(MM2AMD_ENOMEM, "[mm2amd] sdust_batch: pool too small (a call with pool == NULL gives the counts)");
		d.d_out.ensure(n_out);
		HIP_CHECK(hipMemcpyAsync(d.d_out_off.p, out_off, n * 8, hipMemcpyHostToDevice, dc.stream));
		sdust_pack_launch(P, d.d_out_off.p, d.d_out.p, dc.stream);
		HIP_CHECK(hipMemcpyAsync(pool, d.d_out.p, n_out * 8, hipMemcpyDeviceToHost, dc.stream));
		HIP_CHECK(hipStreamSynchronize(dc.stream));
		return 0;
	});
}

int mm2amd_sdust_host_batch(int n_jobs, const mm2amd_sdust_job_t *jobs, int T, int n_threads, mm2amd_sdust_res_t *res, uint64_t *pool, size_t pool_cap,
                            double *core_seconds)
{
	if (const int rc = sdust_check_args("sdust_host_batch", n_jobs, jobs, T, res)) return rc;
	if (core_seconds) *core_seconds = 0;
	if (n_jobs == 0) return 0;
	return guarded([&]() -> int {
		std::vector<std::vector<uint64_t>> regs((size_t)n_jobs);
		std::vector<double> busy((size_t)std::max(n_threads, 1), 0.0);
		parallel_for(n_threads, (long)n_jobs, [&](long i, int tid) {
			const double t0 = Trace::now();
			thread_local std::vector<SdustState::Perf> perf(SdustState::PCAP);
			std::vector<uint8_t> codes((size_t)jobs[i].len + 1);
			for (int32_t k = 0; k < jobs[i].len; ++k) codes[k] = kNt4Table[(uint8_t)jobs[i].seq[k]];
			SdustState S;
			S.P = perf.data();
			sdust_scan(codes.data(), jobs[i].len, T, S, [&](int s0, int e0) { regs[i].push_back((uint64_t)(uint32_t)s0 << 32 | (uint32_t)e0); });
			busy[tid] += Trace::now() - t0;
		}, 1);
		uint64_t n_out = 0;
		for (int i = 0; i < n_jobs; ++i) res[i].off = n_out, res[i].n = (uint32_t)regs[i].size(), res[i].path = -1, n_out += regs[i].size();
		if (core_seconds) for (double b : busy) *core_seconds += b;
		if (!pool || n_out == 0) return 0;
		if (n_out > pool_cap) return fail(MM2AMD_ENOMEM, "[mm2amd] sdust_host_batch: pool too small (a call with pool == NULL gives the counts)");
		for (int i = 0; i < n_jobs; ++i) if (!regs[i].empty()) memcpy(pool + res[i].off, regs[i].data(), regs[i].size() * 8);
		return 0;
	});
}

int mm2amd_sort_pairs_u64(uint64_t *keys, uint64_t *vals, uint64_t n, int bits)
{
	if ((n > 0 && (!keys || !vals)) || bits < 0 || bits > 64 || n >= (1ull << 32)) return fail(MM2AMD_EINVAL, "[mm2amd] sort_pairs_u64: bad arguments (n < 2^32, 0 <= bits <= 64)");
	if (n == 0) return 0;
	return guarded([&]() -> int {
		DeviceCtx &dc = device_ctx();
		std::lock_guard<std::mutex> lk(dc.mu);
		ensure_device(dc);
		DevBuf<uint64_t> k0, v0, k1, v1;
		k0.ensure(n, 1.0), v0.ensure(n, 1.0), k1.ensure(n, 1.0), v1.ensure(n, 1.0);
		HIP_CHECK(hipMemcpyAsync(k0.p, keys, n * 8, hipMemcpyHostToDevice, dc.stream));
		HIP_CHECK(hipMemcpyAsync(v0.p, vals, n * 8, hipMemcpyHostToDevice, dc.stream));
		const int where = device_sort_pairs_u64(k0.p, v0.p, k1.p, v1.p, n, bits, dc.stream);
		HIP_CHECK(hipMemcpyAsync(keys, where ? k1.p : k0.p, n * 8, hipMemcpyDeviceToHost, dc.stream));
		HIP_CHECK(hipMemcpyAsync(vals, where ? v1.p : v0.p, n * 8, hipMemcpyDeviceToHost, dc.stream));
		HIP_CHECK(hipStreamSynchronize(dc.stream));
		return 0;
	});
}

int mm2amd_exclusive_sum_u32(const uint32_t *in, uint32_t *out, uint64_t n)
{
	if (!out || (n > 0 && !in) || n >= (1ull << 32)) return fail(MM2AMD_EINVAL, "[mm2amd] exclusive_sum_u32: bad arguments (n < 2^32)");
	return guarded([&]() -> int {
		DeviceCtx &dc = device_ctx();
		std::lock_guard<std::mutex> lk(dc.mu);
		ensure_device(dc);
		DevBuf<uint32_t> d;
		d.ensure(n + 1, 1.0);
		if (n) HIP_CHECK(hipMemcpyAsync(d.p, in, n * 4, hipMemcpyHostToDevice, dc.stream));
		device_exclusive_sum_u32(d.p, d.p, n, dc.stream);
		HIP_CHECK(hipMemcpyAsync(out, d.p, (n + 1) * 4, hipMemcpyDeviceToHost, dc.stream));
		HIP_CHECK(hipStreamSynchronize(dc.stream));
		return 0;
	});
}

int mm2amd_encode_batch(int n, const char *const *seqs, const int32_t *lens, const int32_t *lens2, uint8_t *out) { return mm2amd_encode_range(n, seqs, lens, lens2, 0, n, out); }

int mm2amd_encode_range(int n, const char *const *seqs, const int32_t *lens, const int32_t *lens2, int lo, int hi, uint8_t *out)
{
	if (n < 0 || !out || (n > 0 && (!seqs || !lens)) || lo < 0 || hi < lo || hi > n) return fail(MM2AMD_EINVAL, "[mm2amd] encode_batch: bad arguments");
	std::vector<uint64_t> unit_off(1, 0);
	std::vector<size_t> frag_unit(1, 0);
	for (int i = 0; i < n; ++i) {
		const int32_t l2 = lens2 ? lens2[i] : 0;
		if (lens[i] < 0 || l2 < 0 || (lens[i] + (int64_t)l2 > 0 && !seqs[i])) return fail(MM2AMD_EINVAL, "[mm2amd] encode_batch: bad read (negative length or null sequence)");
		unit_off.push_back(unit_off.back() + (uint64_t)lens[i]);
		if (l2 > 0) unit_off.push_back(unit_off.back() + (uint64_t)l2);
		frag_unit.push_back(unit_off.size() - 1);
	}
	const uint64_t total = unit_off.back();
	const size_t n_units = unit_off.size() - 1;
	return guarded([&]() -> int {
		DeviceCtx &dc = device_ctx();
		std::lock_guard<std::mutex> lk(dc.mu);
		ensure_device(dc);
		PinBuf<char> h_ascii;
		DevBuf<uint8_t> d_pool;
		DevBuf<uint64_t> d_off;
		char *h = h_ascii.ensure(total + 32, 1.0);
		uint64_t o = 0;
		for (int i = 0; i < n; ++i) {
			const uint64_t l = (uint64_t)lens[i] + (uint64_t)(lens2 ? lens2[i] : 0);
			if (l) memcpy(h + o, seqs[i], l);
			o += l;
		}
		d_pool.ensure(2 * total + 32, 1.0), d_off.ensure(n_units + 1, 1.0);
		HIP_CHECK(hipMemsetAsync(d_pool.p, 0xff, 2 * total + 32, dc.stream));
		HIP_CHECK(hipMemcpyAsync(d_off.p, unit_off.data(), (n_units + 1) * 8, hipMemcpyHostToDevice, dc.stream));
		SeedChainBuffers B;
		B.n_reads = (int)(frag_unit[hi] - frag_unit[lo]), B.seq_off = d_off.p + frag_unit[lo], B.ascii = h, B.qpool = d_pool.p + 16;
		launch_encode(B, dc.stream);
		HIP_CHECK(hipMemcpyAsync(out, d_pool.p, 2 * total + 32, hipMemcpyDeviceToHost, dc.stream));
		HIP_CHECK(hipStreamSynchronize(dc.stream));
		return 0;
	});
}

long long mm2amd_alloc_counter(int which)
{
	AllocStats &a = alloc_stats();
	BandCounters &b = band_counters();
	return which == 0 ? a.dev_allocs.load() : which == 1 ? a.pin_allocs.load() : which == 2 ? a.ns.load() : which == 3 ? (long long)b.n_band1.load() : which == 4 ? (long long)b.n_band2.load() :
	       which == 5 ? (long long)b.n_widened.load() : which == 6 ? (long long)b.n_retried.load() :
	       which == 7 ? (long long)dev_arena().held_bytes() : which == 8 ? (long long)pin_arena().held_bytes() : which == 9 ? (long long)dev_arena().used_bytes() : which == 10 ? (long long)pin_arena().used_bytes() :
	       which == 11 ? (long long)b.n_band4.load() : (long long)b.n_retried_big.load();
}

void mm2amd_profile_enable(int on)
{
	for (int r = 0; r < kMaxReplicas; ++r) for (int l = 0; l < kMaxProfLanes; ++l) kernel_profiler(l, r).reset();
	KernelProfiler::enabled_flag() = on != 0;
}

int mm2amd_profile_get(mm2amd_kernel_stat_t *out, int cap)
{
	std::map<std::string, KernelStat> all;
	for (int r = 0; r < kMaxReplicas; ++r) for (int l = 0; l < kMaxProfLanes; ++l)
		for (const auto &kv : kernel_profiler(l, r).stats()) {
			KernelStat &k = all[kv.first];
			k.ms += kv.second.ms, k.alg_bytes += kv.second.alg_bytes, k.units += kv.second.units, k.launches += kv.second.launches;
		}
	int n = 0;
	for (const auto &kv : all) {
		if (n >= cap) break;
		mm2amd_kernel_stat_t &o = out[n++];
		memset(&o, 0, sizeof o);
		strncpy(o.name, kv.first.c_str(), sizeof o.name - 1);
		o.ms = kv.second.ms, o.alg_bytes = kv.second.alg_bytes, o.launches = kv.second.launches, o.units = kv.second.units;
	}
	return n;
}

}
```

### minimap2_amd/csrc/capi_map.cpp

```cpp
#include <algorithm>
#include <condition_variable>
#include <cstdlib>
#include <cstring>
#include <memory>
#include <atomic>
#include <mutex>
#include <shared_mutex>
#include <string>
#include <thread>
#include "../../include/mm2amd.h"
#include "mapper.hpp"
#include "format.hpp"
#include "index_handle.hpp"
#include "threads.hpp"

namespace mm2amd {
int effective_cpus();
Backend *make_backend(const FlatIndex &fi, void *device_tables, int n_threads, int device, int replica, int tables_device);
int backend_device_count();
void *backend_build_index_tables(FlatIndex &fi, int device, int *on_device);
void backend_free_index_tables(void *tables);
const char *backend_name();
void capi_set_error(const std::string &msg);
int capi_fail(int code, const std::string &msg);
// ... 537 lines not shown
	return need;
}

int mm2amd_unpack_regs(const uint8_t *buf, int64_t size, int n_frag, int *n_reg, void **reg)
{
	if (!buf || size < 0 || n_frag < 0 || (n_frag > 0 && (!n_reg || !reg))) return capi_fail(MM2AMD_EINVAL, "[mm2amd] mm2amd_unpack_regs: bad arguments");
	for (int i = 0; i < n_frag; ++i) n_reg[i] = 0, reg[i] = nullptr;
	auto bail = [&](int code, const char *msg) { mm2amd_free_regs(n_frag, n_reg, reg); return capi_fail(code, msg); };
	const uint8_t *o = buf, *end = buf + size;
	for (int i = 0; i < n_frag; ++i) {
		int32_t n;
		if (end - o < 4) return bail(MM2AMD_EINVAL, "[mm2amd] mm2amd_unpack_regs: truncated payload");
		memcpy(&n, o, 4), o += 4;
		if (n < 0 || (int64_t)n > (end - o) / (int64_t)(sizeof(ref::Reg1) + 4)) return bail(MM2AMD_EINVAL, "[mm2amd] mm2amd_unpack_regs: hit count beyond the payload");
		if (n == 0) continue;
		ref::Reg1 *r = (ref::Reg1 *)calloc(n, sizeof(ref::Reg1));
		if (!r) return bail(MM2AMD_ENOMEM, "[mm2amd] mm2amd_unpack_regs: out of memory");
		reg[i] = r, n_reg[i] = n;
		for (int j = 0; j < n; ++j) {
			uint32_t has;
			if (end - o < (int64_t)sizeof(ref::Reg1) + 4) return bail(MM2AMD_EINVAL, "[mm2amd] mm2amd_unpack_regs: truncated payload");
			memcpy(&r[j], o, sizeof(ref::Reg1)), o += sizeof(ref::Reg1);
			memcpy(&has, o, 4), o += 4;
			r[j].p = nullptr;
			if (has) {
				ref::Extra hd;
				if (end - o < (int64_t)sizeof hd) return bail(MM2AMD_EINVAL, "[mm2amd] mm2amd_unpack_regs: truncated payload");
				memcpy(&hd, o, sizeof hd);
				const size_t nb = sizeof(ref::Extra) + 4ull * hd.n_cigar;
				if ((size_t)(end - o) < nb) return bail(MM2AMD_EINVAL, "[mm2amd] mm2amd_unpack_regs: truncated payload");
				size_t words = (nb + 3) / 4;
				if ((size_t)hd.capacity >= words && (size_t)hd.capacity <= 2 * words + 16) words = hd.capacity;
				r[j].p = (ref::Extra *)calloc(words, 4);
				if (!r[j].p) return bail(MM2AMD_ENOMEM, "[mm2amd] mm2amd_unpack_regs: out of memory");
				memcpy(r[j].p, o, nb), o += nb;
				r[j].p->capacity = (uint32_t)words;
			}
		}
	}
	return 0;
}

int mm_gpu_map_batch(int n_frag, const int *seg_off, const int *n_seg, const void *seq_, int *n_reg, void **reg, int *rep_len, int *frag_gap)
{
	std::shared_lock<std::shared_mutex> lk(g_ctx_mu);
	std::lock_guard<std::mutex> lk_map(g_map_mu);
	if (!g_ctx) return capi_fail(MM2AMD_ESTATE, "[mm2amd] mm_gpu_map_batch called before mm_gpu_init");
	if (n_frag < 0 || (n_frag > 0 && (!seg_off || !n_seg || !seq_ || !n_reg || !reg))) return capi_fail(MM2AMD_EINVAL, "[mm2amd] mm_gpu_map_batch: bad arguments");
	MapContext &c = *g_ctx;
	try {
		StagedBatch *bt;
		{
			std::lock_guard<std::mutex> lk_st(c.stage_mu);
			c.pending = false;
			bt = &c.batch[1 - c.cur];
			if (int rc = collect_views(n_frag, seg_off, n_seg, seq_, c.opt, c.n_threads, bt->views, bt->slots, bt->flipped)) return rc;
			stage_replicas(c, *bt);
			c.pending = true;
			take_staged(c);
		}
		std::vector<ReadResult> out;
		run_replicas(c, *bt, out);
		if (inject_batch_failure()) { free_results(out); throw std::runtime_error("[mm2amd] MM2AMD_INJECT_BATCH_FAILURE: this batch is reported as failed (test knob)"); }
		hand_over(bt->slots, out, n_reg, reg, rep_len, frag_gap);
		c.has_current = false;
		return 0;
	} catch (const std::invalid_argument &e) {
		return capi_fail(MM2AMD_EINVAL, e.what());
	} catch (const std::exception &e) {
		return capi_fail(MM2AMD_EHIP, e.what());
	}
}

struct TbufView { void *km; int rep_len, frag_gap; };

static std::mutex g_single_mu;

static int ensure_context_for(const void *mi, const void *opt)
{
	{
		std::shared_lock<std::shared_mutex> lk(g_ctx_mu);
		const ref::Idx *rmi = (const ref::Idx *)mi;
		if (g_ctx && g_ctx->mi_ptr == mi && memcmp(&g_ctx->opt, opt, sizeof(ref::MapOpt)) == 0 && g_ctx->mi_stamp[0] == g_stamp_hash(rmi) &&
		    g_ctx->mi_stamp[1] == (uint64_t)(uintptr_t)rmi->S && g_ctx->mi_stamp[2] == (uint64_t)(uintptr_t)rmi->seq && g_ctx->mi_stamp[3] == (uint64_t)rmi->n_alt) return 0;
	}
	return mm_gpu_init(mi, opt, 0);
}

void mm_gpu_map_frag(const void *mi, int n_segs, const int *qlens, const char **seqs, int *n_regs, void **regs, void *b, const void *opt, const char *qname)
{
	for (int s = 0; s < n_segs; ++s) n_regs[s] = 0, regs[s] = nullptr;
	if (!mi || !opt || n_segs < 1 || n_segs > 2) { capi_fail(MM2AMD_EINVAL, "[mm2amd] mm_gpu_map_frag: one or two segments, non-null index and options"); return; }
	std::lock_guard<std::mutex> lk_single(g_single_mu);
	if (ensure_context_for(mi, opt) != 0) return;
	ref::Bseq1 rec[2];
	for (int s = 0; s < n_segs; ++s) {
		rec[s].l_seq = qlens[s], rec[s].rid = s;
		rec[s].name = const_cast<char *>(qname), rec[s].seq = const_cast<char *>(seqs[s]), rec[s].qual = rec[s].comment = nullptr;
	}
	const int seg_off = 0;
	int rep_len[2] = { 0, 0 }, frag_gap[2] = { 0, 0 };
	if (mm_gpu_map_batch(1, &seg_off, &n_segs, rec, n_regs, regs, rep_len, frag_gap) != 0) {
		for (int s = 0; s < n_segs; ++s) n_regs[s] = 0, regs[s] = nullptr;
		return;
	}
	if (b) ((TbufView *)b)->rep_len = rep_len[0], ((TbufView *)b)->frag_gap = frag_gap[0];
}

int mm_gpu_map_batch_with(const void *mi, const void *opt, int n_frag, const int *seg_off, const int *n_seg, const void *seq, int *n_reg, void **reg, int *rep_len, int *frag_gap)
{
	if (!mi || !opt) return capi_fail(MM2AMD_EINVAL, "[mm2amd] mm_gpu_map_batch_with: non-null index and options");
	std::lock_guard<std::mutex> lk_single(g_single_mu);
	if (int rc = ensure_context_for(mi, opt)) return rc;
	return mm_gpu_map_batch(n_frag, seg_off, n_seg, seq, n_reg, reg, rep_len, frag_gap);
}

void *mm_gpu_map(const void *mi, int qlen, const char *seq, int *n_regs, void *b, const void *opt, const char *qname)
{
	void *regs = nullptr;
	mm_gpu_map_frag(mi, 1, &qlen, &seq, n_regs, &regs, b, opt, qname);
	return regs;
}

void mm_gpu_destroy(void)
{
	std::unique_lock<std::shared_mutex> lk(g_ctx_mu);
	g_ctx.reset();
}

int mm_gpu_destroy_if(uint64_t generation)
{
	std::unique_lock<std::shared_mutex> lk(g_ctx_mu);
	if (!g_ctx || g_ctx->generation != generation) return 0;
	g_ctx.reset();
	return 1;
}

const char *mm2amd_backend_name(void) { return backend_name(); }
int mm2amd_format_fraction(double v, char *buf) { return buf ? format_fraction_for_test(v, buf) : 0; }

int mm2amd_last_stats(double *v, int n)
{
	std::shared_lock<std::shared_mutex> lk(g_ctx_mu);
	if (!g_ctx) return 0;
	std::lock_guard<std::mutex> lk_stats(g_ctx->stats_mu);
	const MapperStats &s = g_ctx->stats;
	const double a[] = { s.t_seed_chain, s.t_host_pre, s.t_plan, s.t_ksw, s.t_consume, s.t_finish, (double)s.n_jobs, (double)s.n_rounds, s.dp_cells,
	                     (double)mm2amd_alloc_counter(0), (double)mm2amd_alloc_counter(1), (double)mm2amd_alloc_counter(2),
	                     s.c_seed_chain, s.c_host_pre, s.c_plan, s.c_ksw, s.c_consume, s.c_finish, (double)s.n_long_join_dev, (double)s.n_long_join_host,
	                     s.d_seed_chain, s.d_host_pre, s.d_plan, s.d_ksw, s.d_consume, s.d_finish, (double)s.n_early_sub,
	                     (double)s.n_region_reads_dev, (double)s.n_region_reads_host,
	                     (double)mm2amd_alloc_counter(3), (double)mm2amd_alloc_counter(4), (double)mm2amd_alloc_counter(5), (double)mm2amd_alloc_counter(6),
	                     (double)mm2amd_alloc_counter(7), (double)mm2amd_alloc_counter(8), (double)mm2amd_alloc_counter(9), (double)mm2amd_alloc_counter(10),
	                     (double)mm2amd_alloc_counter(11), (double)mm2amd_alloc_counter(12) };
	int k = 0;
	for (; k < n && k < (int)(sizeof a / sizeof a[0]); ++k) v[k] = a[k];
	return k;
}

}
```

### minimap2_amd/csrc/chain_dump.hpp

```cpp
#pragma once
#include <cstdio>
#include <cstdlib>
#include <mutex>
#include <string>

#include "backend.hpp"

namespace mm2amd {

inline const char *chain_dump_path() { return getenv("MM2AMD_CHAIN_DUMP"); }

struct ChainDumpBlock {
	const char *name = nullptr;
	int qlen = 0, n_seg = 1, pass = 1;
	bool host = false, handed_back = false;
	const Anchor *in = nullptr;
	int64_t n_in = 0;
	const uint64_t *u = nullptr;
	int32_t n_u = 0;
	const Anchor *a = nullptr;
	int64_t n_a = 0;
};

inline void chain_dump_words(std::string &s, const char *tag, int64_t n, const uint64_t *w, int64_t n_words)
{
	char buf[40];
	snprintf(buf, sizeof(buf), "%s\t%lld\t", tag, (long long)n);
	s += buf;
	for (int64_t i = 0; i < n_words; ++i) {
		snprintf(buf, sizeof(buf), i ? " %llx" : "%llx", (unsigned long long)w[i]);
		s += buf;
	}
	s += '\n';
}

inline void chain_dump_format(std::string &s, const SeedChainParams &P, const ChainDumpBlock &b)
{
	static_assert(sizeof(Anchor) == 16, "an anchor is two 64-bit words");
	char buf[512];
	int gap_ref, gap_qry;
	chain_gaps(P, b.qlen, &gap_ref, &gap_qry);
	snprintf(buf, sizeof(buf), "CH\t%s\t%d\t%d\t%s\t%s\n", b.name ? b.name : "*", b.qlen, b.pass, b.host ? "host" : "dev", b.handed_back ? "handed-back" : "chained");
	s += buf;
	snprintf(buf, sizeof(buf), "PR\t%d\t%d\t%d\t%d\t%d\t%d\t%d\t%a\t%a\t%d\t%d\t%d\t%d\t%d\t%d\t%d\n", gap_ref, gap_qry, P.bw, P.max_chain_skip, P.max_chain_iter, P.min_cnt,
	         P.min_chain_score, (double)P.chn_pen_gap, (double)P.chn_pen_skip, P.is_cdna, b.n_seg, P.rmq || P.anchors_only ? 1 : 0, P.rmq_inner_dist, P.rmq_size_cap, P.bw_long, P.mid_occ);
	s += buf;
	if (b.in) chain_dump_words(s, "IN", b.n_in, (const uint64_t *)b.in, 2 * b.n_in);
	else s += "IN\t-\n";
	int64_t n_a = 0;
	for (int32_t k = 0; k < b.n_u; ++k) n_a += (int32_t)b.u[k];
	if (n_a != b.n_a) { snprintf(buf, sizeof(buf), "ERR\tchains of %lld anchors, %lld anchors\n", (long long)n_a, (long long)b.n_a); s += buf; n_a = n_a < b.n_a ? n_a : b.n_a; }
	chain_dump_words(s, "U", b.n_u, b.u, b.n_u);
	chain_dump_words(s, "A", n_a, (const uint64_t *)b.a, 2 * n_a);
	s += "END\n";
}

inline void chain_dump_flush(const char *path, const std::string &s)
{
	static std::mutex mu;
	std::lock_guard<std::mutex> lk(mu);
	if (FILE *fp = fopen(path, "a")) {
		fwrite(s.data(), 1, s.size(), fp);
		fclose(fp);
	}
}

}
```

### minimap2_amd/csrc/hip_util.hpp

```cpp
#pragma once
#include <hip/hip_runtime.h>
#include <time.h>
#include <cstdio>
#include <cstdlib>
#include <cstdint>
#include <stdexcept>
#include <string>
#include <atomic>
#include <chrono>
#include <map>
#include <mutex>
#include <vector>
#include <iterator>

#ifdef MM2AMD_WAVE_EMU
#define MM2_DYN_LDS(T, name) T *const name = (T *)wave_emu::dyn_shared()
#define MM2_LOCKSTEP() __builtin_amdgcn_wave_barrier()
#else
#define MM2_DYN_LDS(T, name) extern __shared__ __attribute__((aligned(16))) T name[]
#define MM2_LOCKSTEP() ((void)0)
#endif

namespace mm2amd {

struct HipError : std::runtime_error {
	using std::runtime_error::runtime_error;
};

inline void hip_check(hipError_t e, const char *what, const char *file, int line)
{
	if (e != hipSuccess) {
		char buf[512];
		snprintf(buf, sizeof buf, "[mm2amd] HIP error %d (%s) at %s:%d: %s", (int)e, hipGetErrorString(e), file, line, what);
		throw HipError(buf);
	}
}
#define HIP_CHECK(x) ::mm2amd::hip_check((x), #x, __FILE__, __LINE__)

inline void stream_wait(hipStream_t s)
{
	struct PerDevice { int dev = -1; hipEvent_t ev = nullptr; ~PerDevice() { if (ev) (void)hipEventDestroy(ev); } };
	thread_local PerDevice cache[4];
	int dev = 0;
	HIP_CHECK(hipGetDevice(&dev));
	PerDevice *slot = nullptr;
	for (PerDevice &c : cache) if (c.dev == dev) { slot = &c; break; }
	if (!slot) {
		for (PerDevice &c : cache) if (c.dev < 0) { slot = &c; break; }
		if (!slot) { HIP_CHECK(hipStreamSynchronize(s)); return; }
		HIP_CHECK(hipEventCreateWithFlags(&slot->ev, hipEventDisableTiming));
		slot->dev = dev;
	}
	HIP_CHECK(hipEventRecord(slot->ev, s));
	static const long max_ns = [] { const char *e = getenv("MM2AMD_WAIT_MAX_US"); const long us = e ? atol(e) : 500; return (us < 20 ? 20 : us) * 1000L; }();
	long ns = 20000;
	for (int it = 0;; ++it) {
		const hipError_t e = hipEventQuery(slot->ev);
		if (e == hipSuccess) return;
		if (e != hipErrorNotReady) HIP_CHECK(e);
		if (it < 4) continue;
		timespec ts = { 0, ns };
		nanosleep(&ts, nullptr);
		if (ns < max_ns) ns += ns / 2;
	}
}

int effective_cpus();

struct AllocStats { std::atomic<long> dev_allocs{0}, pin_allocs{0}; std::atomic<double> dummy{0}; std::atomic<long long> dev_bytes{0}, pin_bytes{0}; std::atomic<long long> ns{0}; };
inline AllocStats &alloc_stats() { static AllocStats s; return s; }
struct BandCounters { std::atomic<unsigned long long> n_band1{0}, n_band2{0}, n_band4{0}, n_widened{0}, n_retried{0}, n_retried_big{0}; };
inline BandCounters &band_counters() { static BandCounters s; return s; }

class MemArena {
public:
	MemArena(bool pinned, size_t chunk_bytes) : pinned_(pinned), chunk_bytes_(chunk_bytes) {}
	~MemArena() { for (Chunk &c : chunks_) raw_free(c.base); for (auto &kv : solo_) raw_free(kv.first); }
	static bool enabled()
	{
#ifdef MM2AMD_WAVE_EMU
		static const bool on = getenv("MM2AMD_ARENA") != nullptr;
#else
		static const bool on = getenv("MM2AMD_NO_ARENA") == nullptr;
#endif
		return on;
	}
	void *alloc(size_t bytes)
	{
		bytes = (bytes + 255) & ~(size_t)255;
		if (bytes == 0) bytes = 256;
		int dev = 0;
		(void)hipGetDevice(&dev);
		if (!enabled() || bytes > chunk_bytes_ / 2) {
			char *p = raw_alloc(bytes);
			std::lock_guard<std::mutex> lk(mu_);
			solo_[p] = bytes;
			return p;
		}
		for (int pass = 0;; ++pass) {
			{
				std::lock_guard<std::mutex> lk(mu_);
				for (Chunk &c : chunks_) {
					if (c.dev != dev) continue;
					for (auto it = c.free_.begin(); it != c.free_.end(); ++it) {
						if (it->second < bytes) continue;
						const size_t off = it->first, len = it->second;
						c.free_.erase(it);
						if (len > bytes) c.free_[off + bytes] = len - bytes;
						c.used[off] = bytes;
						return c.base + off;
					}
				}
			}
			if (pass >= 2) throw HipError("[mm2amd] MemArena: fresh chunks did not hold the request");
			add_chunk(dev);
		}
	}
	void release(void *p)
	{
		if (!p) return;
		std::lock_guard<std::mutex> lk(mu_);
		auto so = solo_.find((char *)p);
		if (so != solo_.end()) { raw_free(so->first); solo_.erase(so); return; }
		for (Chunk &c : chunks_) {
			if ((char *)p < c.base || (char *)p >= c.base + c.size) continue;
			const size_t off = (size_t)((char *)p - c.base);
			auto u = c.used.find(off);
			if (u == c.used.end()) return;
			size_t len = u->second, beg = off;
			c.used.erase(u);
			auto nx = c.free_.lower_bound(beg);
			if (nx != c.free_.end() && nx->first == beg + len) { len += nx->second; nx = c.free_.erase(nx); }
			if (nx != c.free_.begin()) { auto pv = std::prev(nx); if (pv->first + pv->second == beg) { beg = pv->first, len += pv->second; c.free_.erase(pv); } }
			c.free_[beg] = len;
			return;
		}
	}
	size_t held_bytes() { std::lock_guard<std::mutex> lk(mu_); size_t n = 0; for (const Chunk &c : chunks_) n += c.size; return n; }
	size_t used_bytes() { std::lock_guard<std::mutex> lk(mu_); size_t n = 0; for (const Chunk &c : chunks_) for (auto &u : c.used) n += u.second; return n; }
	void reserve(size_t bytes)
	{
		if (!enabled()) return;
		int dev = 0;
		(void)hipGetDevice(&dev);
		for (;;) {
			size_t have = 0;
			{ std::lock_guard<std::mutex> lk(mu_); for (const Chunk &c : chunks_) if (c.dev == dev) have += c.size; }
			if (have >= bytes) return;
			add_chunk(dev);
		}
	}
private:
	struct Chunk { char *base; size_t size; int dev; std::map<size_t, size_t> free_, used; };
	char *raw_alloc(size_t bytes)
	{
		void *p = nullptr;
		const auto t0_ = std::chrono::steady_clock::now();
		if (pinned_) { HIP_CHECK(hipHostMalloc(&p, bytes, hipHostMallocDefault)); alloc_stats().pin_allocs++, alloc_stats().pin_bytes += (long long)bytes; }
		else { HIP_CHECK(hipMalloc(&p, bytes)); alloc_stats().dev_allocs++, alloc_stats().dev_bytes += (long long)bytes; }
		alloc_stats().ns += std::chrono::duration_cast<std::chrono::nanoseconds>(std::chrono::steady_clock::now() - t0_).count();
		return (char *)p;
	}
	void raw_free(char *p) { if (pinned_) (void)hipHostFree(p); else (void)hipFree(p); }
	void add_chunk(int dev)
	{
		Chunk c;
		c.base = raw_alloc(chunk_bytes_), c.size = chunk_bytes_, c.dev = dev;
		c.free_[0] = chunk_bytes_;
		std::lock_guard<std::mutex> lk(mu_);
		chunks_.push_back(std::move(c));
	}
	const bool pinned_;
	const size_t chunk_bytes_;
	std::mutex mu_;
	std::vector<Chunk> chunks_;
	std::map<char *, size_t> solo_;
};
inline size_t arena_env_gb(const char *name, size_t dflt) { const char *e = getenv(name); return e ? (size_t)atol(e) : dflt; }
inline MemArena &dev_arena() { static MemArena *a = new MemArena(false, (size_t)4 << 30); return *a; }
inline MemArena &pin_arena() { static MemArena *a = new MemArena(true, (size_t)1 << 30); return *a; }

template <typename T>
struct DevBuf {
	T *p = nullptr;
	size_t cap = 0;
	DevBuf() = default;
	DevBuf(const DevBuf &) = delete;
	DevBuf &operator=(const DevBuf &) = delete;
	~DevBuf() { if (p) dev_arena().release(p); }
	T *ensure(size_t n, double slack = 1.25)
	{
		if (n > cap) {
			if (p) dev_arena().release(p);
			p = nullptr;
			cap = (size_t)(n * slack) + 64;
			p = (T *)dev_arena().alloc(cap * sizeof(T));
		}
		return p;
	}
	void release() { if (p) dev_arena().release(p); p = nullptr; cap = 0; }
};

template <typename T>
struct PinBuf {
	T *p = nullptr;
	size_t cap = 0;
	PinBuf() = default;
	PinBuf(const PinBuf &) = delete;
	PinBuf &operator=(const PinBuf &) = delete;
	~PinBuf() { if (p) pin_arena().release(p); }
	T *ensure(size_t n, double slack = 1.25)
	{
		if (n > cap) {
			if (p) pin_arena().release(p);
			p = nullptr;
			cap = (size_t)(n * slack) + 64;
			p = (T *)pin_arena().alloc(cap * sizeof(T));
		}
		return p;
	}
};

}
```

### minimap2_amd/csrc/kernel_prof.hpp

```cpp
#pragma once
#include <map>
#include <string>
#include <vector>
#include "hip_util.hpp"

namespace mm2amd {

struct KernelStat { double ms = 0, alg_bytes = 0, units = 0; long launches = 0; };

class KernelProfiler {
public:
	static bool &enabled_flag() { static bool on = false; return on; }
	bool active_ = false;
	void begin(hipStream_t s)
	{
		active_ = enabled_flag();
		if (!active_) return;
		Pending p;
		p.e0 = get_event(), p.e1 = get_event();
		HIP_CHECK(hipEventRecord(p.e0, s));
		pending_.push_back(p);
	}
	void end(hipStream_t s, const char *name, double alg_bytes, double units = 0)
	{
		if (!active_) return;
		Pending &p = pending_.back();
		p.name = name, p.bytes = alg_bytes, p.units = units;
		HIP_CHECK(hipEventRecord(p.e1, s));
	}
	void add_units(const char *name, double units) { if (enabled_flag()) stats_[name].units += units; }
	void collect()
	{
		for (Pending &p : pending_) {
			float ms = 0;
			if (p.name && hipEventElapsedTime(&ms, p.e0, p.e1) == hipSuccess) {
				KernelStat &k = stats_[p.name];
				k.ms += ms, k.alg_bytes += p.bytes, k.units += p.units, ++k.launches;
			}
			free_.push_back(p.e0), free_.push_back(p.e1);
		}
		pending_.clear();
	}
	void reset() { collect(); stats_.clear(); }
	void drop_events() { collect(); for (hipEvent_t e : free_) (void)hipEventDestroy(e); free_.clear(); }
	const std::map<std::string, KernelStat> &stats() const { return stats_; }
private:
	struct Pending { hipEvent_t e0, e1; const char *name = nullptr; double bytes = 0, units = 0; };
	hipEvent_t get_event()
	{
		if (!free_.empty()) { hipEvent_t e = free_.back(); free_.pop_back(); return e; }
		hipEvent_t e;
		HIP_CHECK(hipEventCreate(&e));
		return e;
	}
	std::vector<Pending> pending_;
	std::vector<hipEvent_t> free_;
	std::map<std::string, KernelStat> stats_;
};

constexpr int kMaxProfLanes = 16, kMaxReplicas = 16;
KernelProfiler &kernel_profiler(int lane = 0, int replica = 0);

}
```

### minimap2_amd/csrc/seed_chain.hip

```cpp
#include <hip/hip_runtime.h>
#include "hip_util.hpp"
#include "seed_chain_dev.hpp"
#include "index_build.hpp"
#include "heap_order.hpp"
#include "sdust_core.hpp"
#include "sketch_dev.hpp"
#include "sdust_dev.hpp"
#include "kernel_prof.hpp"

namespace mm2amd {

#define WAVE_SYNC() do { __builtin_amdgcn_fence(__ATOMIC_ACQ_REL, "wavefront"); __builtin_amdgcn_wave_barrier(); } while (0)

__constant__ uint8_t c_nt4[256];
extern const uint8_t kNt4Table[256];
static bool g_nt4_uploaded = false;

static void upload_tables(hipStream_t s)
{
	if (g_nt4_uploaded) return;
	HIP_CHECK(hipMemcpyToSymbolAsync(HIP_SYMBOL(c_nt4), kNt4Table, 256, 0, hipMemcpyHostToDevice, s));
	g_nt4_uploaded = true;
}

// ... 927 lines not shown
							if (p == regB) s.put(p, s.get(fr.b + (int32_t)posx[0]));
							else if (pf) s.put(p, s.get(fr.b + (int32_t)posx[cz]));
							else s.put(p, k > 0 ? el[k > 0 ? k - 1 : 0] : prev_el);
						}
					}
					if (fmask >> k & 1u) ++r;
				}
			}
			__syncthreads();
			{
				uint32_t r = base;
#pragma unroll
				for (int k = 0; k < TWO_PER; ++k) {
					const int32_t p = p0 + k;
					if (fmask >> k & 1u) {
						if (p >= regB) s.put(fr.b + (int32_t)posx[r - m], el[k]);
						++r;
					}
				}
			}
			__syncthreads();
		}
		if (tape.cap > 0 && tape.tab[768]) {
#ifdef MM2AMD_WAVE_EMU
			if (tid == 0 && getenv("MM2AMD_TWO_BUCKET_TRACE")) fprintf(stderr, "[mm2amd] tape walk: %d elements at shift %d\n", (int)len, (int)fr.shift);
#endif
			uint16_t *const tpos = tape.pos, *const via = tape.via;
			uint8_t *const tdig = tape.dig;
			uint32_t *const ent = head;
			uint32_t *const Fs = tape.tab, *const Fe = tape.tab + 256, *const m1 = tape.tab + 512, *const wave_tot = tape.tab + 769, *const has_tape = tape.tab + 785;
			const int32_t per = (len + nt - 1) / nt, p0 = fr.b + tid * per, p1 = p0 + per < fr.e ? p0 + per : fr.e;
			typename S::Elem el[TWO_PER];
			uint32_t rg[TWO_PER];
			uint32_t fmask = 0, mine = 0;
			if (tid < 256) Fs[tid] = 0, Fe[tid] = 0;
			if (tid < 8) has_tape[tid] = 0;
			{
				int32_t reg = 0;
				if (p0 < p1) {
					const uint32_t q0 = (uint32_t)(p0 - fr.b);
					int lo = 0, hi = 255;
					while (lo < hi) { const int mid = (lo + hi) >> 1; if (cnt[mid] > q0) hi = mid; else lo = mid + 1; }
					reg = lo;
				}
#pragma unroll
				for (int k = 0; k < TWO_PER; ++k) {
					const int32_t p = p0 + k;
					el[k] = typename S::Elem();
					rg[k] = 0;
					if (p < p1) {
						while (cnt[reg] <= (uint32_t)(p - fr.b)) ++reg;
						rg[k] = (uint32_t)reg;
						el[k] = s.get(p);
						if ((uint32_t)(s.xk(el[k]) >> fr.shift & 255) != (uint32_t)reg) fmask |= 1u << k, ++mine;
					}
				}
			}
			const uint32_t incl = wave_prefix_add_u32(mine);
			const int wv = tid >> 6, n_wv = (nt + 63) >> 6;
			if ((tid & 63) == 63) wave_tot[wv] = incl;
			__syncthreads();
			uint32_t base = incl - mine, total = 0;
			for (int w2 = 0; w2 < n_wv; ++w2) { const uint32_t t = wave_tot[w2]; if (w2 < wv) base += t; total += t; }
			{
				uint32_t r = base;
#pragma unroll
				for (int k = 0; k < TWO_PER; ++k) {
					const int32_t p = p0 + k;
					if (p < p1) {
						const uint32_t q = (uint32_t)(p - fr.b);
						if (q == start[rg[k]]) Fs[rg[k]] = r;
						if (fmask >> k & 1u) { tpos[r] = (uint16_t)q, tdig[r] = (uint8_t)(s.xk(el[k]) >> fr.shift & 255); ++r; }
						if (q + 1 == cnt[rg[k]]) Fe[rg[k]] = r;
					}
				}
			}
			__syncthreads();
			if (tid < 256) {
				ent[tid] = Fs[tid] << 8 | (Fs[tid] < Fe[tid] ? (uint32_t)tdig[Fs[tid]] : 0u);
				m1[tid] = Fs[tid];
				if (Fs[tid] < Fe[tid]) atomicOr(&has_tape[tid >> 5], 1u << (tid & 31));
			}
			__syncthreads();
			if (tid == 0) {
				const uint32_t last = total ? total - 1 : 0;
				for (uint32_t kw = 0; kw < 8; ++kw)
				for (uint32_t km = has_tape[kw]; km; km &= km - 1) {
					const uint32_t k = kw * 32 + (uint32_t)__builtin_ctz(km);
					uint32_t wk = ent[k];
					const uint32_t fe = Fe[k];
					m1[k] = wk >> 8;
					while ((wk >> 8) < fe) {
						const uint32_t e0 = wk >> 8, nk = e0 + 1;
						uint32_t dst = wk & 255u, src = e0;
						uint32_t w2 = ent[dst];
						wk = nk << 8 | (nk < fe ? (uint32_t)tdig[nk] : 0u);
						for (;;) {
							const uint32_t t = w2 >> 8, nxt = w2 & 255u;
							uint32_t w3 = 0;
							if (nxt != k) w3 = ent[nxt];
							const uint32_t nd = tdig[t < last ? t + 1 : t];
							via[src] = (uint16_t)t;
							ent[dst] = (t + 1) << 8 | nd;
							src = t;
							if (nxt == k) break;
							dst = nxt, w2 = w3;
						}
						via[src] = (uint16_t)e0;
					}
				}
			}
			__syncthreads();
			{
				uint32_t r = base;
				int32_t dpos[TWO_PER];
#pragma unroll
				for (int k = 0; k < TWO_PER; ++k) {
					const int32_t p = p0 + k;
					dpos[k] = -1;
					if (p < p1) {
						const uint32_t q = (uint32_t)(p - fr.b);
						if (fmask >> k & 1u) {
							const uint32_t d = (uint32_t)(s.xk(el[k]) >> fr.shift & 255), t = via[r];
							if (t < m1[d]) dpos[k] = t == Fs[d] ? (int32_t)start[d] : (int32_t)tpos[t - 1] + 1;
							else dpos[k] = (int32_t)tpos[t];
							++r;
						} else dpos[k] = (int32_t)q + (r < m1[rg[k]] ? 1 : 0);
					}
				}
#pragma unroll
				for (int k = 0; k < TWO_PER; ++k) if (dpos[k] >= 0 && dpos[k] != p0 + k - fr.b) s.put(fr.b + dpos[k], el[k]);
			}
			__syncthreads();
		}
		if (fr.shift == 0) continue;
		const int ns = fr.shift > 8 ? fr.shift - 8 : 0;
		if (tid == 0) head[0] = (uint32_t)sp;
		__syncthreads();
		for (int k = tid; k < 256; k += nt) {
			const int32_t cb = fr.b + (int32_t)start[k], ce = fr.b + (int32_t)cnt[k];
			if (ce - cb <= 1) continue;
			if (!replay_all && !(child_mask[k >> 5] >> (k & 31) & 1u)) continue;
			if (ce - cb > 64) {
				const uint32_t slot = atomicAdd(&head[0], 1u);
				if ((int)slot < stack_cap) stack[slot] = TieFrame{cb, ce, ns};
			} else insertion(cb, ce);
		}
		__syncthreads();
		sp = (int)head[0] < stack_cap ? (int)head[0] : stack_cap;
	}
}

template <int THREADS, int ROUNDS, bool IN_LDS>
__global__ void __launch_bounds__(THREADS, (THREADS == 1024 && IN_LDS && ROUNDS <= 7) ? 8 : 4)  anchor_sort_kernel(SeedChainBuffers B, const uint32_t *list, int heap_sort)
{
	MM2_DYN_LDS(uint64_t, as_lds);
	__shared__ uint32_t tab[(THREADS / 64) * 256];
	__shared__ uint32_t dig_tot[256], child_mask[8];
	__shared__ uint64_t tied[TIE_MAX_KEYS];
	__shared__ TieFrame lstack[AS_STACK];
	__shared__ uint32_t n_tied_s;
	uint32_t *const cnt = tab, *const head = tab + 256, *const start = tab + 512;
	const int32_t tid = (int32_t)threadIdx.x;
	const int r = (int)list[blockIdx.x];
	const uint64_t ao = B.a_off[r];
	const int32_t n = (int32_t)(B.a_off[r + 1] - ao);
	const uint64_t *kin = B.sort_key_in + ao, *vin = B.sort_val_in + ao;
	Anchor *out = B.anchors + ao;
	if (n == 0) return;
	auto run = [&](auto s, TieFrame *stack, int stack_cap) {
		for (int32_t i = tid; i < n; i += THREADS) s.set(i, kin[i], (uint32_t)i);
		if (tid == 0) n_tied_s = 0;
		__syncthreads();
		if constexpr (IN_LDS) lds_radix_sort<THREADS, ROUNDS>(as_lds, n, 33 + B.rid_bits, tab, dig_tot);
		else bitonic_sort(s, n);
		for (int32_t i = tid; i < n; i += THREADS) {
			const uint64_t x = s.xkey(i);
			Anchor a;
			a.x = x, a.y = vin[s.index(i)];
			out[i] = a;
			if (i + 1 < n && s.xkey(i + 1) == x && (i == 0 || s.xkey(i - 1) != x)) {
				const uint32_t slot = atomicAdd(&n_tied_s, 1u);
				if (slot < (uint32_t)TIE_MAX_KEYS) tied[slot] = x;
			}
		}
		__syncthreads();
		const uint32_t n_tied_all = n_tied_s;
#ifdef MM2AMD_WAVE_EMU
		if (tid == 0 && getenv("MM2AMD_TIE_TRACE")) fprintf(stderr, "[mm2amd] anchor sort: read %d, %d anchors, %u duplicated keys\n", r, (int)n, n_tied_all);
#endif
		if (n_tied_all == 0) return;
		if (tid == 0) B.tie_flag[r] = 1u;
		if (heap_sort & 1) return;
		if (IN_LDS && (heap_sort & 4)) {
			if (tid == 0) B.tie_list[atomicAdd(B.tie_count, 1u)] = (uint32_t)r;
			return;
		}
		const bool replay_all = n_tied_all > (uint32_t)TIE_MAX_KEYS;
		const int n_tied = replay_all ? TIE_MAX_KEYS : (int)n_tied_all;
		for (int32_t i = tid; i < n; i += THREADS) s.set(i, kin[i], (uint32_t)i);
		__syncthreads();
		tie_exact_replay<decltype(s), ROUNDS>(s, n, tied, n_tied, replay_all, cnt, head, start, child_mask, stack, stack_cap, IN_LDS && !(heap_sort & 2) ? tab + 768 : nullptr, IN_LDS ? ((THREADS / 64) * 256 - 768 - 20) * 2 : 0);
		for (int32_t i = tid; i < n; i += THREADS) {
			const uint64_t x = s.xkey(i);
			bool dup = replay_all;
			for (int t = 0; t < n_tied && !dup; ++t) dup = tied[t] == x;
			if (dup) { Anchor a; a.x = x, a.y = vin[s.index(i)]; out[i] = a; }
		}
	};
	if (IN_LDS) run(PackedStore{as_lds, B.rid_bits}, lstack, AS_STACK);
	else {
		uint32_t *I = (uint32_t *)(B.sort_val_out + ao);
		run(SplitStore{B.sort_key_out + ao, I, B.rid_bits}, (TieFrame *)(I + n), (int)((size_t)n * 4 / sizeof(TieFrame)));
	}
}

constexpr int AST_THREADS = 1024, AST_PER = AS_LDS_MAX / AST_THREADS;
constexpr size_t AST_LDS_BYTES = (size_t)AS_LDS_MAX * (8 + 2 + 2 + 1);
__global__ void __launch_bounds__(AST_THREADS, 4) anchor_sort_ties_kernel(SeedChainBuffers B, int mode)
{
	MM2_DYN_LDS(uint64_t, ast_lds);
	__shared__ uint32_t tab[768], tape_tab[768 + 32], child_mask[8];
	__shared__ uint64_t tied[TIE_MAX_KEYS];
	__shared__ TieFrame lstack[AS_STACK];
	__shared__ uint32_t n_tied_s;
	const int32_t tid = (int32_t)threadIdx.x;
	TapeScratch tape;
	tape.pos = (uint16_t *)(ast_lds + AS_LDS_MAX), tape.via = tape.pos + AS_LDS_MAX, tape.dig = (uint8_t *)(tape.via + AS_LDS_MAX), tape.tab = tape_tab, tape.cap = AS_LDS_MAX;
	const bool split = !(mode & 16);
	const uint32_t n_list = *B.tie_count * (split ? 2u : 1u);
	for (uint32_t li = blockIdx.x; li < n_list; li += gridDim.x) {
		const int r = (int)B.tie_list[split ? li >> 1 : li];
		const uint64_t strand = li & 1u;
		const uint64_t ao = B.a_off[r];
		const int32_t n = (int32_t)(B.a_off[r + 1] - ao);
		const uint64_t *kin = B.sort_key_in + ao, *vin = B.sort_val_in + ao;
		Anchor *out = B.anchors + ao;
		PackedStore s{ast_lds, B.rid_bits};
		__syncthreads();
		if (tid == 0) n_tied_s = 0;
		__syncthreads();
		for (int32_t i = tid; i < n; i += AST_THREADS) {
			const uint64_t x = out[i].x;
			if (i + 1 < n && out[i + 1].x == x && (i == 0 || out[i - 1].x != x) && (!split || x >> 63 == strand)) {
				const uint32_t slot = atomicAdd(&n_tied_s, 1u);
				if (slot < (uint32_t)TIE_MAX_KEYS) tied[slot] = x;
			}
			s.set(i, kin[i], (uint32_t)i);
		}
		__syncthreads();
		const uint32_t n_tied_all = n_tied_s;
		if (n_tied_all == 0) continue;
		const bool replay_all = n_tied_all > (uint32_t)TIE_MAX_KEYS;
		const int n_tied = replay_all ? TIE_MAX_KEYS : (int)n_tied_all;
		tie_exact_replay<PackedStore, AST_PER>(s, n, tied, n_tied, replay_all, tab, tab + 256, tab + 512, child_mask, lstack, AS_STACK,
		                                       (mode & 2) ? nullptr : (uint32_t *)tape.via, AS_LDS_MAX - 40, (mode & 8) ? TapeScratch() : tape);
		for (int32_t i = tid; i < n; i += AST_THREADS) {
			const uint64_t x = s.xkey(i);
			bool dup = replay_all;
			for (int t = 0; t < n_tied && !dup; ++t) dup = tied[t] == x;
			if (dup) { Anchor a; a.x = x, a.y = vin[s.index(i)]; out[i] = a; }
		}
	}
}

__global__ void __launch_bounds__(64) anchor_heap_order_kernel(SeedChainBuffers B, DevIndex I, SeedChainParams P)
{
	for (int r = blockIdx.x * 64 + threadIdx.x; r < B.n_reads; r += gridDim.x * 64) {
		if (!B.tie_flag[r]) continue;
		const uint64_t mo = B.mz_off[r], ao = B.a_off[r];
		const uint32_t *sd_n = B.sd_n + mo, *sd_off = B.sd_off + mo, *sd_aoff = B.sd_aoff + mo, *sd_qpos = B.sd_qpos + mo, *sd_info = B.sd_info + mo;
		const uint32_t n_m0 = B.n_seedhit[r];
		const int qlen = (int)(B.seq_off[r + 1] - B.seq_off[r]);
		const uint32_t n = (uint32_t)(B.a_off[r + 1] - ao);
		HIT_RULES_SETUP();
		Anchor *out = B.anchors + ao;
		uint32_t n_for = 0, n_rev = 0;
		heap_merge_order(n_m0, B.mz_x + mo, B.mz_y + mo,
			[&](uint32_t i, uint32_t *cnt) { *cnt = sd_aoff[i] == 0xffffffffu ? 0u : sd_n[i]; return I.pos + sd_off[i]; },
			[&](uint32_t i, uint64_t rr) {
				const uint32_t info = sd_info[i], span = info & 0xff, qp = sd_qpos[i], rpos = (uint32_t)rr >> 1;
				bool is_self = false;
				if (hit_rules && skip_hit(P.flag, rr, qp, qlen, nm_lb, nm_eq, I, &is_self)) return;
				Anchor p;
				if ((rr & 1) == (qp & 1)) {
					p.x = (rr & 0xffffffff00000000ULL) | rpos;
					p.y = (uint64_t)span << 32 | (uint64_t)(qp >> 1);
				} else {
					p.x = 1ULL << 63 | (rr & 0xffffffff00000000ULL) | rpos;
					p.y = (uint64_t)span << 32 | (uint64_t)(uint32_t)(qlen - ((int)(qp >> 1) + 1 - (int)span) - 1);
				}
				if (info & SD_SEG1) p.y |= 1ULL << ref::SEED_SEG_SHIFT;
				if (info & SD_TANDEM) p.y |= ref::SEED_TANDEM;
				if (is_self) p.y |= ref::SEED_SELF;
				if (p.x >> 63) { if (n_for + n_rev < n) out[n - (++n_rev)] = p; }
				else if (n_for + n_rev < n) out[n_for++] = p;
			});
		for (uint32_t j = 0; j < n_rev >> 1; ++j) {
			const Anchor t = out[n - 1 - j];
			out[n - 1 - j] = out[n - n_rev + j];
			out[n - n_rev + j] = t;
		}
	}
}

const int kAnchorSortCap[kAnchorSortClasses] = { 1024, 2048, 4096, 7168, AS_LDS_MAX, 0 };

int anchor_sort_class(uint64_t n_anchors, int rid_bits)
{
	static const int force = getenv("MM2AMD_SORT_MIN_CLASS") ? atoi(getenv("MM2AMD_SORT_MIN_CLASS")) : 0;
	if (33 + rid_bits + AS_IDX_BITS > 64) return kAnchorSortClasses - 1;
	if (force > 0) { for (int c = std::min(force, kAnchorSortClasses - 1); c + 1 < kAnchorSortClasses; ++c) if (n_anchors <= (uint64_t)kAnchorSortCap[c]) return c; return kAnchorSortClasses - 1; }
	for (int c = 0; c + 1 < kAnchorSortClasses; ++c) if (n_anchors <= (uint64_t)kAnchorSortCap[c]) return c;
	return kAnchorSortClasses - 1;
}

void launch_anchor_sort(const SeedChainBuffers &B, const DevIndex &I, const SeedChainParams &P, const uint32_t *d_list, const int *n_class, const double *anchors_in_class, void *stream,
                        KernelProfiler *kp)
{
	hipStream_t s = (hipStream_t)stream;
	KernelProfiler none;
	if (!kp) kp = &none;
	HIP_CHECK(hipMemsetAsync(B.tie_flag, 0, (size_t)B.n_reads * 4, s));
	static const char *kNames[kAnchorSortClasses] = { "anchor_sort_kernel[n1k]", "anchor_sort_kernel[n2k]", "anchor_sort_kernel[n4k]", "anchor_sort_kernel[n7k]", "anchor_sort_kernel[n10k]", "anchor_sort_kernel[global]" };
	if (n_class[4] > 0) HIP_CHECK(hipFuncSetAttribute((const void *)anchor_sort_kernel<1024, 10, true>, hipFuncAttributeMaxDynamicSharedMemorySize, AS_LDS_MAX * 8));
	static const bool no_replay = getenv("MM2AMD_SORT_NO_REPLAY") != nullptr;
	const bool walk_only = getenv("MM2AMD_NO_TWO_BUCKET") != nullptr;
	static const bool replay_inline = getenv("MM2AMD_TIE_REPLAY_INLINE") != nullptr;
	const bool no_tape = getenv("MM2AMD_NO_TAPE_WALK") != nullptr;
	const bool no_split = getenv("MM2AMD_TIE_NO_STRAND_SPLIT") != nullptr;
	const int heap = ((P.flag & ref::F_HEAP_SORT) || no_replay ? 1 : 0) | (walk_only ? 2 : 0) | (replay_inline ? 0 : 4) | (no_tape ? 8 : 0) | (no_split ? 16 : 0);
	if (heap & 4) HIP_CHECK(hipMemsetAsync(B.tie_count, 0, 4, s));
	int first = 0;
	for (int c = 0; c < kAnchorSortClasses; first += n_class[c], ++c) {
		if (n_class[c] == 0) continue;
		kp->begin(s);
		const size_t lds = (size_t)kAnchorSortCap[c] * 8;
		const dim3 grid(n_class[c]);
		if (c == 0) hipLaunchKernelGGL((anchor_sort_kernel<256, 4, true>), grid, dim3(256), lds, s, B, d_list + first, heap);
		else if (c == 1) hipLaunchKernelGGL((anchor_sort_kernel<256, 8, true>), grid, dim3(256), lds, s, B, d_list + first, heap);
		else if (c == 2) hipLaunchKernelGGL((anchor_sort_kernel<512, 8, true>), grid, dim3(512), lds, s, B, d_list + first, heap);
		else if (c == 3) hipLaunchKernelGGL((anchor_sort_kernel<1024, 7, true>), grid, dim3(1024), lds, s, B, d_list + first, heap);
		else if (c == 4) hipLaunchKernelGGL((anchor_sort_kernel<1024, 10, true>), grid, dim3(1024), lds, s, B, d_list + first, heap);
		else hipLaunchKernelGGL((anchor_sort_kernel<1024, 1, false>), grid, dim3(1024), 0, s, B, d_list + first, heap);
		kp->end(s, kNames[c], 32.0 * anchors_in_class[c]);
		HIP_CHECK(hipGetLastError());
	}
	const int n_lds = n_class[0] + n_class[1] + n_class[2] + n_class[3] + n_class[4];
	if ((heap & 4) && !(heap & 1) && n_lds > 0) {
		kp->begin(s);
		HIP_CHECK(hipFuncSetAttribute((const void *)anchor_sort_ties_kernel, hipFuncAttributeMaxDynamicSharedMemorySize, (int)AST_LDS_BYTES));
		hipLaunchKernelGGL(anchor_sort_ties_kernel, dim3(std::min(2 * n_lds, 512)), dim3(AST_THREADS), AST_LDS_BYTES, s, B, heap);
		kp->end(s, "anchor_sort_kernel[ties]", 0.0);
		HIP_CHECK(hipGetLastError());
	}
	if (P.flag & ref::F_HEAP_SORT) {
		kp->begin(s);
		hipLaunchKernelGGL(anchor_heap_order_kernel, dim3(std::min((B.n_reads + 63) / 64, 4096)), dim3(64), 0, s, B, I, P);
		kp->end(s, "anchor_heap_order_kernel", 0.0);
		HIP_CHECK(hipGetLastError());
	}
}

__device__ __forceinline__ float fast_log2_dev(float x)
{
	uint32_t zi = __float_as_uint(x);
	float l = (float)((int)((zi >> 23) & 255) - 128);
	zi &= ~(255u << 23);
	zi += 127u << 23;
	const float zf = __uint_as_float(zi);
	l += (-0.34484843f * zf + 2.02466578f) * zf - 0.67487759f;
	return l;
}

template <bool PAIRS>
__device__ __forceinline__ int32_t link_score(uint64_t ix, uint64_t iy, uint64_t jx, uint64_t jy, int32_t max_dist_x, int32_t max_dist_y, int32_t bw,
                                              float pen_gap, float pen_skip, int is_cdna, int n_seg)
{
	const int32_t dq = (int32_t)iy - (int32_t)jy;
	const bool same = PAIRS ? ((iy ^ jy) & ref::SEED_SEG_MASK) == 0 : true;
	if (dq <= 0 || dq > max_dist_x) return INT32_MIN;
	const int32_t dr = (int32_t)(ix - jx);
	if (same && (dr == 0 || dq > max_dist_y)) return INT32_MIN;
	const int32_t dd = dr > dq ? dr - dq : dq - dr;
	if (same && dd > bw) return INT32_MIN;
	if (n_seg > 1 && !is_cdna && same && dr > max_dist_y) return INT32_MIN;
	const int32_t dg = dr < dq ? dr : dq, span = (int32_t)(jy >> 32 & 0xff);
	int32_t sc = span < dg ? span : dg;
	if (dd || dg > span) {
		const float lin = pen_gap * (float)dd + pen_skip * (float)dg;
		const float lg = dd >= 1 ? fast_log2_dev((float)(dd + 1)) : 0.0f;
		if (is_cdna || !same) {
			if (!same && dr == 0) ++sc;
			else if (dr > dq || !same) sc -= (int)(lin < lg ? lin : lg);
			else sc -= (int)(lin + .5f * lg);
		} else sc -= (int)(lin + .5f * lg);
	}
	return sc;
}

constexpr int CF_RING = 256;

__device__ __forceinline__ int64_t chain_first_head(const Anchor *a, int64_t n, int64_t from, int32_t max_dist, int lane)
{
	for (int64_t base = from; base < n; base += 64) {
		const int64_t g = base + lane;
		bool head = false;
		if (g < n) { const uint64_t gx = a[g].x, px = a[g - 1].x; head = gx >> 32 != px >> 32 || gx > px + (uint64_t)(int64_t)max_dist; }
		const unsigned long long m = __ballot(head);
		if (m) return base + (__ffsll((long long)m) - 1);
	}
	return n;
}

__device__ __forceinline__ void chain_piece_bounds(const Anchor *a, int64_t n, int64_t k, int64_t len, int32_t max_dist, int lane, int64_t *lo, int64_t *hi)
{
	*lo = k == 0 ? 0 : (k * len < n ? chain_first_head(a, n, k * len, max_dist, lane) : n);
	*hi = (k + 1) * len < n ? chain_first_head(a, n, (k + 1) * len, max_dist, lane) : n;
}

template <bool PAIRS, int RING>
__global__ void __launch_bounds__(256) chain_fill_kernel(SeedChainBuffers B, SeedChainParams P)
{
	constexpr int RN = RING ? RING : 1, RM = RN - 1;
	__shared__ uint64_t s_x[4][RN], s_y[4][RN];
	__shared__ int32_t s_f[4][RN], s_p[4][RN], s_t[4][RN];
	const int wave = threadIdx.x >> 6, lane = lane_id();
	const int w = blockIdx.x * 4 + wave;
	if (w >= (B.pieces ? B.n_pieces : B.n_reads)) return;
	const int r = B.pieces ? (int)B.pieces[2 * w] : w;
	uint64_t *const rx = s_x[wave], *const ry = s_y[wave];
	int32_t *const rf = s_f[wave], *const rp = s_p[wave], *const rt = s_t[wave];
	const Anchor *a = B.anchors + B.a_off[r];
	const int64_t n_all = (int64_t)(B.a_off[r + 1] - B.a_off[r]);
	int32_t *f = B.f + B.a_off[r], *p = B.p + B.a_off[r], *t = B.t + B.a_off[r];
	int32_t max_dist_x, max_dist_y;
	chain_gaps(P, (int)(B.seq_off[r + 1] - B.seq_off[r]), &max_dist_x, &max_dist_y);
	max_dist_x = __builtin_amdgcn_readfirstlane(max_dist_x), max_dist_y = __builtin_amdgcn_readfirstlane(max_dist_y);
	const int n_seg = PAIRS ? B.unit_first[r + 1] - B.unit_first[r] : 1;
	const int32_t bw = P.bw;
	if (max_dist_x < bw) max_dist_x = bw;
	if (max_dist_y < bw && !P.is_cdna) max_dist_y = bw;
	int64_t lo = 0, n = n_all;
	if (B.pieces) chain_piece_bounds(a, n_all, (int64_t)B.pieces[2 * w + 1], (int64_t)B.piece_len, max_dist_x, lane, &lo, &n);
	if (lo >= n) return;
	for (int64_t i = lo + lane; i < n; i += 64) t[i] = 0;
	__threadfence_block();

	int64_t st = lo, max_ii = -1;
	uint64_t mii_x = 0, mii_y = 0;
	int32_t mii_f = 0;
	uint64_t last_x = 0, last_y = 0;
	bool last_iso = false;
	for (int64_t blk = lo; blk < n; blk += 64) {
		const int64_t g = blk + lane;
		const int64_t ring_lo = RING ? (blk + 64 - lo > RN ? blk + 64 - RN : lo) : INT64_MAX;
		auto ax = [&](int64_t j) { return j >= ring_lo ? rx[j & RM] : a[j].x; };
		auto ay = [&](int64_t j) { return j >= ring_lo ? ry[j & RM] : a[j].y; };
		auto af = [&](int64_t j) { return j >= ring_lo ? rf[j & RM] : f[j]; };
		auto ap = [&](int64_t j) { return j >= ring_lo ? rp[j & RM] : p[j]; };
		uint64_t bx = 0, by = 0;
		if (g < n) { const Anchor v = a[g]; bx = v.x, by = v.y; }
		const uint64_t px = wave_shr1_u64(last_x, bx), py = wave_shr1_u64(last_y, by);
		const bool iso = g < n && (g == lo || (bx >> 32 != px >> 32 || bx > px + (uint64_t)(int64_t)max_dist_x));
		if (iso) f[g] = (int32_t)(by >> 32 & 0xff), p[g] = -1;
		if (RING && g < n) {
			rx[g & RM] = bx, ry[g & RM] = by, rt[g & RM] = -1;
			if (iso) rf[g & RM] = (int32_t)(by >> 32 & 0xff), rp[g & RM] = -1;
		}
		__threadfence_block();
		unsigned long long todo = __ballot(g < n && !iso);
		const unsigned long long iso_mask = __ballot(iso);
		while (todo) {
			const int bl = __ffsll((long long)todo) - 1;
			todo &= todo - 1;
			const int64_t i = blk + bl;
			const uint64_t ix = lane_get_u64(bx, bl), iy = lane_get_u64(by, bl);
			const bool head_before = bl == 0 ? last_iso : (iso_mask >> (bl - 1) & 1) != 0;
			if (head_before) {
				const uint64_t hx = lane_get_u64(px, bl), hy = lane_get_u64(py, bl);
				st = i - 1, max_ii = i - 1, mii_x = hx, mii_y = hy, mii_f = (int32_t)(hy >> 32 & 0xff);
			}
			while (st < i) {
				const int64_t c = st + lane;
				bool stop = true;
				if (c < i) { const uint64_t cx = ax(c); stop = !(ix >> 32 != cx >> 32 || ix > cx + (uint64_t)(int64_t)max_dist_x); }
				const unsigned long long m = __ballot(stop);
				if (m) { st += __ffsll((long long)m) - 1; break; }
				st += 64;
			}
			if (st > i) st = i;
			if (i - st > P.max_chain_iter) st = i - P.max_chain_iter;

			int32_t max_f = (int32_t)(iy >> 32 & 0xff), n_skip = 0;
			int64_t max_j = -1, end_j = st - 1;
			bool broke = false;
			for (int64_t base = i - 1; base >= st && !broke; base -= 64) {
				const int64_t j = base - lane;
				int32_t sc = INT32_MIN, pj = -1;
				if (j >= st) {
					sc = link_score<PAIRS>(ix, iy, ax(j), ay(j), max_dist_x, max_dist_y, bw, P.chn_pen_gap, P.chn_pen_skip, P.is_cdna, n_seg);
					if (sc != INT32_MIN) sc += af(j), pj = ap(j);
				}
				const bool has = sc != INT32_MIN;
				int32_t excl = wave_shr1_i32(INT32_MIN, wave_prefix_max_i32(has ? sc : INT32_MIN));
				excl = excl > max_f ? excl : max_f;
				const bool improve = has && sc > excl;
				if (has && pj >= 0) { if (pj >= ring_lo) rt[pj & RM] = (int32_t)i; else t[pj] = (int32_t)i; }
				__threadfence_block();
				const int64_t jm = j >= st ? j : st;
				const bool marked = has && !improve && (jm >= ring_lo ? rt[jm & RM] : t[jm]) == (int32_t)i;
				unsigned long long imp = __ballot(improve);
				const unsigned long long mk = __ballot(marked);
				int stop_lane = 64;
				for (int pos = 0; pos < 64;) {
					const unsigned long long later = imp >> pos;
					const int ni = later ? pos + (__ffsll((long long)later) - 1) : 64;
					unsigned long long seg = (mk >> pos) << pos;
					if (ni < 64) seg &= (1ull << ni) - 1ull;
					const int c = __popcll(seg);
					if (n_skip + c > P.max_chain_skip) {
						for (int k = P.max_chain_skip - n_skip; k > 0; --k) seg &= seg - 1;
						stop_lane = __ffsll((long long)seg) - 1;
						break;
					}
					n_skip += c;
					if (ni == 64) break;
					if (n_skip > 0) --n_skip;
					pos = ni + 1;
				}
				if (stop_lane < 64) {
					broke = true;
					end_j = base - stop_lane;
					imp &= (1ull << stop_lane) - 1ull;
				}
				if (imp) {
					const int last = 63 - __clzll((long long)imp);
					max_f = lane_get_i32(sc, last);
					max_j = base - last;
				}
			}
			bool recompute = max_ii < 0;
			if (!recompute) recompute = ix - mii_x > (uint64_t)(int64_t)max_dist_x;
			if (recompute) {
				long long best = INT64_MIN;
				for (int64_t base = i - 1; base >= st; base -= 64) {
					const int64_t j = base - lane;
					if (j >= st) { const long long key = (long long)af(j) << 32 | (long long)(uint32_t)j; best = key > best ? key : best; }
				}
				for (int o = 32; o > 0; o >>= 1) { const long long v = __shfl_xor(best, o, 64); best = v > best ? v : best; }
				max_ii = best == INT64_MIN ? -1 : (int64_t)(uint32_t)(best & 0xffffffffLL);
				if (max_ii >= 0) mii_x = ax(max_ii), mii_y = ay(max_ii), mii_f = (int32_t)(best >> 32);
			}
			if (max_ii >= 0 && max_ii < end_j) {
				const int32_t tmp = link_score<PAIRS>(ix, iy, mii_x, mii_y, max_dist_x, max_dist_y, bw, P.chn_pen_gap, P.chn_pen_skip, P.is_cdna, n_seg);
				if (tmp != INT32_MIN && max_f < tmp + mii_f) max_f = tmp + mii_f, max_j = max_ii;
			}
			if (RING) { if (lane == 0) rf[i & RM] = max_f, rp[i & RM] = (int32_t)max_j; WAVE_SYNC(); }
			else { if (lane == 0) f[i] = max_f, p[i] = (int32_t)max_j; __threadfence_block(); }
			if (max_ii < 0 || (ix - mii_x <= (uint64_t)(int64_t)max_dist_x && mii_f < max_f)) max_ii = i, mii_x = ix, mii_y = iy, mii_f = max_f;
		}
		if (RING) {
			if (g < n && !iso) f[g] = rf[g & RM], p[g] = rp[g & RM];
			__threadfence_block();
		}
		const int last_lane = (int)((n - blk < 64 ? n - blk : 64) - 1);
		last_x = lane_get_u64(bx, last_lane), last_y = lane_get_u64(by, last_lane);
		last_iso = (iso_mask >> last_lane & 1) != 0;
	}
}

void launch_chain_fill(const SeedChainBuffers &B, const SeedChainParams &P, void *stream)
{
	const char *ring_env = getenv("MM2AMD_CHAIN_RING");
	const int ring = getenv("MM2AMD_CHAIN_FILL_GLOBAL") ? 0 : ring_env ? atoi(ring_env) : CF_RING;
	const dim3 grid(((B.pieces ? B.n_pieces : B.n_reads) + 3) / 4), block(256);
	hipStream_t s = (hipStream_t)stream;
	if (B.unit_first) {
		if (ring == 0) hipLaunchKernelGGL((chain_fill_kernel<true, 0>), grid, block, 0, s, B, P);
		else if (ring == 128) hipLaunchKernelGGL((chain_fill_kernel<true, 128>), grid, block, 0, s, B, P);
		else hipLaunchKernelGGL((chain_fill_kernel<true, CF_RING>), grid, block, 0, s, B, P);
	} else {
		if (ring == 0) hipLaunchKernelGGL((chain_fill_kernel<false, 0>), grid, block, 0, s, B, P);
		else if (ring == 128) hipLaunchKernelGGL((chain_fill_kernel<false, 128>), grid, block, 0, s, B, P);
		else hipLaunchKernelGGL((chain_fill_kernel<false, CF_RING>), grid, block, 0, s, B, P);
	}
	HIP_CHECK(hipGetLastError());
}

constexpr int RMQ_NEAR_CAP = 4096;
constexpr int RMQ_RANK_MAX = 256;
constexpr int RMQ_NEAR_SMALL = 1024;

__device__ __forceinline__ int32_t simple_score_dev(uint64_t ix, uint64_t iy, uint64_t jx, uint64_t jy, float pen_gap, float pen_skip, bool *exact, int32_t *width)
{
// ... 289 lines not shown
			if (!exact && max_dist_inner > 0 && st_in < i0 && y_i > 0) {
				if (tid == 0) s_cnt = 0;
				__syncthreads();
				for (int64_t base = st_in; base < i0; base += THREADS) {
					const int64_t j = base + tid;
					bool in = false;
					int32_t y_j = 0;
					if (j < i0) { y_j = (int32_t)a[j].y; in = y_j <= y_i - 1 && y_j >= y_i - max_dist_inner; }
					const unsigned long long m = __ballot(in);
					int first = 0;
					if (lane == 0 && m) first = atomicAdd(&s_cnt, (int)__popcll(m));
					first = __shfl(first, 0, 64);
					if (in) { const int d = first + popc_below(m, lane); if (d < RMQ_NEAR_CAP) s_near[d] = (uint64_t)(uint32_t)y_j << 32 | (uint64_t)(uint32_t)j; }
				}
				__syncthreads();
				const int n_c = s_cnt;
				if (n_c > RMQ_NEAR_CAP) { give_up = true; break; }
				const uint64_t *sorted = s_near;
				if (n_c <= B.rmq_rank_max) {
					for (int e = tid; e < n_c; e += THREADS) {
						const uint64_t key = s_near[e];
						int rank = 0;
						for (int k = 0; k < n_c; ++k) rank += s_near[k] > key;
						s_rank[rank] = key;
					}
					sorted = s_rank;
					__syncthreads();
				} else {
				int n_pad = 64;
				while (n_pad < n_c) n_pad <<= 1;
				for (int k = n_c + tid; k < n_pad; k += THREADS) s_near[k] = 0;
				__syncthreads();
				for (int k2 = 2; k2 <= n_pad; k2 <<= 1)
					for (int j2 = k2 >> 1; j2 > 0; j2 >>= 1) {
						for (int e = tid; e < n_pad; e += THREADS) {
							const int partner = e ^ j2;
							if (partner > e) {
								const uint64_t u0 = s_near[e], u1 = s_near[partner];
								const bool desc = (e & k2) == 0;
								if (desc ? u0 < u1 : u0 > u1) s_near[e] = u1, s_near[partner] = u0;
							}
						}
						__syncthreads();
					}
				}
				if (wv == 0) {
					int32_t n_skip = 0;
					bool broke = false;
					for (int base = 0; base < n_c && !broke; base += 64) {
						const int c = base + lane;
						int32_t scc = INT32_MIN, pj = -1;
						int64_t j = -1;
						if (c < n_c) {
							j = (int64_t)(uint32_t)sorted[c];
							bool ex;
							int32_t wd;
							const Anchor cj = a[j];
							const int32_t v = simple_score_dev(ix, iy, cj.x, cj.y, P.chn_pen_gap, P.chn_pen_skip, &ex, &wd);
							if (wd <= bw) scc = f[j] + v, pj = p[j];
						}
						const bool has = scc != INT32_MIN;
						int32_t pm = has ? scc : INT32_MIN;
						for (int o = 1; o < 64; o <<= 1) { const int32_t v = __shfl_up(pm, o, 64); if (lane >= o) pm = v > pm ? v : pm; }
						int32_t excl = __shfl_up(pm, 1, 64);
						if (lane == 0) excl = INT32_MIN;
						excl = excl > max_f ? excl : max_f;
						const bool improve = has && scc > excl;
						if (has && pj >= 0) t[pj] = (int32_t)i;
						__threadfence_block();
						const bool marked = has && !improve && t[j] == (int32_t)i;
						unsigned long long imp = __ballot(improve), mk = __ballot(marked), ev = imp | mk;
						int stop_lane = 64;
						while (ev) {
							const int b = __ffsll((long long)ev) - 1;
							ev &= ev - 1;
							if (imp >> b & 1) { if (n_skip > 0) --n_skip; }
							else if (++n_skip > P.max_chain_skip) { stop_lane = b; break; }
						}
						if (stop_lane < 64) broke = true, imp &= (1ull << stop_lane) - 1ull;
						if (imp) {
							const int last = 63 - __clzll((long long)imp);
							max_f = __shfl(scc, last, 64);
							max_j = __shfl(j, last, 64);
						}
					}
				}
			}
		}
		if (tid == 0) f[i] = max_f, p[i] = (int32_t)max_j;
		__threadfence_block();
		__syncthreads();
	}
	if (tid == 0 && give_up) atomicOr(&B.tie_flag[r], 1u);
}

void launch_chain_rmq(const SeedChainBuffers &B, const SeedChainParams &P, void *stream)
{
	hipStream_t s = (hipStream_t)stream;
	const dim3 grid(B.pieces ? B.n_pieces : B.n_reads);
	HIP_CHECK(hipMemsetAsync(B.tie_flag, 0, (size_t)B.n_reads * 4, s));
	uint64_t *timing = nullptr;
	const int n_w = (int)grid.x < (1 << 20) ? (int)grid.x : 1 << 20;
	if (getenv("MM2AMD_RMQ_TIMING")) { HIP_CHECK(hipMalloc((void **)&timing, (size_t)n_w * 16)); HIP_CHECK(hipMemsetAsync(timing, 0, (size_t)n_w * 16, s)); }
	if (getenv("MM2AMD_RMQ_NEAR_TINY")) hipLaunchKernelGGL(chain_rmq_kernel<64>, grid, dim3(64), 0, s, B, P, timing);
	else hipLaunchKernelGGL(chain_rmq_kernel<RMQ_NEAR_SMALL>, grid, dim3(64), 0, s, B, P, timing);
	if (timing) {
		std::vector<uint64_t> h((size_t)n_w * 2);
		HIP_CHECK(hipStreamSynchronize(s));
		HIP_CHECK(hipMemcpy(h.data(), timing, h.size() * 8, hipMemcpyDeviceToHost));
		HIP_CHECK(hipFree(timing));
		std::vector<int> order(n_w);
		for (int i = 0; i < n_w; ++i) order[i] = i;
		std::sort(order.begin(), order.end(), [&](int x, int y) { return h[2 * x] > h[2 * y]; });
		double sum = 0, anchors = 0;
		for (int i = 0; i < n_w; ++i) sum += (double)h[2 * i], anchors += (double)(h[2 * i + 1] >> 32);
		fprintf(stderr, "[mm2amd] chain_rmq_kernel: %d wavefronts (%d reads), %.0f anchors, %.1f ms of wavefront time in all; the longest:", n_w, B.n_reads, anchors, sum / 1e5);
		for (int i = 0; i < 6 && i < n_w; ++i) fprintf(stderr, " %.2f ms / %llu anchors (read %u)", (double)h[2 * order[i]] / 1e5, (unsigned long long)(h[2 * order[i] + 1] >> 32), (unsigned)h[2 * order[i] + 1]);
		fprintf(stderr, "\n");
	}
	if (B.pieces && B.piece_dense > 0) {
		const char *e = getenv("MM2AMD_RMQ_DENSE_BIG");
		const int big = B.piece_dense * (e && atoi(e) > 0 ? atoi(e) : 4);
		hipLaunchKernelGGL(chain_rmq_wide_kernel<256>, grid, dim3(256), 0, s, B, P, B.piece_dense, big);
		hipLaunchKernelGGL(chain_rmq_wide_kernel<1024>, grid, dim3(1024), 0, s, B, P, big, INT32_MAX);
	}
	hipLaunchKernelGGL(chain_rmq_kernel<RMQ_NEAR_CAP>, grid, dim3(64), 0, s, B, P, (uint64_t *)nullptr);
	HIP_CHECK(hipGetLastError());
}

#ifndef MM2AMD_BT_LDS_CAP
#define MM2AMD_BT_LDS_CAP 512
#endif
constexpr int BT_LDS_CAP = MM2AMD_BT_LDS_CAP;
constexpr int BT_STACK = BT_LDS_CAP / 65 + 2;
constexpr int BT_PATH_CAP = 2048;

__device__ void bt_sort(uint64_t *K, uint32_t *I, int32_t n, uint32_t *cnt, uint32_t *head, uint32_t *start, uint32_t *child_mask, TieFrame *stack, int stack_cap)
{
	tie_exact_replay(SplitStore{K, I, -1}, n, nullptr, 0, true, cnt, head, start, child_mask, stack, stack_cap);
}

__global__ void __launch_bounds__(64) chain_backtrack_kernel(SeedChainBuffers B, int min_cnt, int min_sc, int max_drop, int rmq)
{
	__shared__ uint64_t lK[BT_LDS_CAP];
	__shared__ uint32_t lI[BT_LDS_CAP];
	__shared__ uint32_t cnt[256], head[256], start[256], child_mask[8];
	__shared__ TieFrame stack[BT_STACK];
	__shared__ uint16_t path[BT_PATH_CAP];
	__shared__ int32_t s_nu, s_nv;
	__shared__ uint64_t s_aoff, s_uoff;
	const int lane = threadIdx.x;
	const int r = blockIdx.x;
	const uint64_t ao = B.a_off[r];
	const int32_t n = (int32_t)(B.a_off[r + 1] - ao);
	const Anchor *a = B.anchors + ao;
	const int32_t *f = B.f + ao, *p = B.p + ao;
	int32_t *t = B.t + ao;
	if (rmq) {
		const uint32_t fl = B.tie_flag[r];
		if (lane == 0 && fl != (fl & 1u)) B.tie_flag[r] = fl & 1u;
		if (fl & 1u) { if (lane == 0) B.bt_nu[r] = 0, B.bt_nv[r] = 0, B.bt_aoff[r] = 0, B.bt_uoff[r] = 0; return; }
	}
	if (n == 0) { if (lane == 0) B.bt_nu[r] = 0, B.bt_nv[r] = 0, B.bt_aoff[r] = 0, B.bt_uoff[r] = 0; return; }
	int32_t n_z = 0;
	for (int32_t i = lane; i < n; i += 64) { t[i] = 0; n_z += f[i] >= min_sc; }
	for (int o = 32; o > 0; o >>= 1) n_z += __shfl_xor(n_z, o, 64);
	if (n_z == 0) { if (lane == 0) B.bt_nu[r] = 0, B.bt_nv[r] = 0, B.bt_aoff[r] = 0, B.bt_uoff[r] = 0; return; }
	uint64_t *K = n_z <= BT_LDS_CAP ? lK : B.sort_key_out + ao;
	uint32_t *I = n_z <= BT_LDS_CAP ? lI : (uint32_t *)(B.sort_val_out + ao);
	int32_t *v = (int32_t *)(B.sort_val_in + ao);
	uint64_t *u = B.sort_key_in + ao;
	{
		int32_t dst = 0;
		for (int32_t base = 0; base < n; base += 64) {
			const int32_t i = base + lane;
			const bool keep = i < n && f[i] >= min_sc;
			const unsigned long long m = __ballot(keep);
			if (keep) { const int32_t d = dst + popc_below(m, lane); K[d] = (uint64_t)(uint32_t)f[i], I[d] = (uint32_t)i; }
			dst += __popcll(m);
		}
	}
	__threadfence_block();
	__syncthreads();
	TieFrame *big_stack = (TieFrame *)(B.sort_val_in + ao + ((size_t)n + 1) / 2);
	const int big_cap = (int)(((size_t)n - ((size_t)n + 1) / 2) * 8 / sizeof(TieFrame));
	bt_sort(K, I, n_z, cnt, head, start, child_mask, n_z <= BT_LDS_CAP ? stack : big_stack, n_z <= BT_LDS_CAP ? BT_STACK : big_cap);
	__threadfence_block();
	__syncthreads();
	int32_t n_v = 0, n_u_acc = 0;
	const int32_t pcap = n <= 65536 ? BT_PATH_CAP : 0;
	for (int32_t k0 = n_z - 1; k0 >= 0; k0 -= 64) {
		const int32_t k = k0 - lane;
		int32_t zi = 0, zx = 0;
		if (k >= 0) zi = (int32_t)I[k], zx = (int32_t)K[k];
		unsigned long long todo = __ballot(k >= 0 && t[zi] == 0);
		while (todo) {
			const int src = __ffsll((long long)todo) - 1;
			const int32_t czi = __shfl(zi, src, 64), czx = __shfl(zx, src, 64);
			int32_t keep = 0, max_s = 0;
			if (lane == 0) {
				int32_t i = czi, pi = p[czi], len = 0;
				for (;;) {
					if (len < pcap) path[len] = (uint16_t)i;
					++len;
					const int32_t nxt = pi;
					int32_t fn = 0, tn = 0, pn = -1;
					if (nxt >= 0) fn = f[nxt], tn = t[nxt], pn = p[nxt];
					const int32_t sc = nxt < 0 ? czx : czx - fn;
					if (sc > max_s) max_s = sc, keep = len;
					else if (max_s - sc > max_drop) break;
					if (nxt < 0 || tn != 0) break;
					i = nxt, pi = pn;
				}
			}
			keep = __builtin_amdgcn_readfirstlane(keep), max_s = __builtin_amdgcn_readfirstlane(max_s);
			WAVE_SYNC();
			const int32_t n_rec = keep < pcap ? keep : pcap;
			for (int32_t q = lane; q < n_rec; q += 64) { const int32_t idx = path[q]; v[n_v + q] = idx, t[idx] = 1; }
			if (keep > pcap && lane == 0) {
				int32_t i = pcap > 0 ? p[path[pcap - 1]] : czi;
				for (int32_t q = pcap; q < keep; ++q) { v[n_v + q] = i, t[i] = 1; i = p[i]; }
			}
			if (max_s >= min_sc && keep > 0 && keep >= min_cnt) {
				if (lane == 0) u[n_u_acc] = (uint64_t)(uint32_t)max_s << 32 | (uint64_t)(uint32_t)keep;
				++n_u_acc, n_v += keep;
			}
			__threadfence_block();
			WAVE_SYNC();
			todo &= ~((2ull << src) - 1ull);
			todo = __ballot((todo >> lane & 1ull) != 0 && t[zi] == 0);
		}
	}
	if (lane == 0) {
		s_nu = n_u_acc, s_nv = n_v;
		s_aoff = n_v ? atomicAdd((unsigned long long *)&B.bt_cursor[0], (unsigned long long)n_v) : 0;
		s_uoff = n_u_acc ? atomicAdd((unsigned long long *)&B.bt_cursor[1], (unsigned long long)n_u_acc) : 0;
		B.bt_nu[r] = n_u_acc, B.bt_nv[r] = n_v, B.bt_aoff[r] = s_aoff, B.bt_uoff[r] = s_uoff;
	}
	__threadfence_block();
	__syncthreads();
	const int32_t n_u = s_nu;
	if (n_u == 0) return;
	uint32_t *cst = (uint32_t *)t;
	if (lane == 0) { uint32_t k = 0; for (int32_t i = 0; i < n_u; ++i) { cst[i] = k; k += (uint32_t)u[i]; } }
	__threadfence_block();
	__syncthreads();
	uint64_t *K2 = n_u <= BT_LDS_CAP ? lK : B.sort_key_out + ao;
	uint32_t *I2 = n_u <= BT_LDS_CAP ? lI : (uint32_t *)(B.sort_val_out + ao);
	for (int32_t i = lane; i < n_u; i += 64) {
		const uint32_t ni = (uint32_t)u[i];
		K2[i] = a[v[cst[i] + ni - 1]].x, I2[i] = (uint32_t)i;
	}
	__threadfence_block();
	__syncthreads();
	bt_sort(K2, I2, n_u, cnt, head, start, child_mask, n_u <= BT_LDS_CAP ? stack : big_stack, n_u <= BT_LDS_CAP ? BT_STACK : big_cap);
	__threadfence_block();
	__syncthreads();
	Anchor *oa = B.bt_out_a + s_aoff;
	uint64_t *ou = B.bt_out_u + s_uoff;
	uint32_t k = 0;
	for (int32_t i = 0; i < n_u; ++i) {
		const uint32_t j = I2[i], c = (uint32_t)u[j], s0 = cst[j];
		if (lane == 0) ou[i] = u[j];
		for (uint32_t q = lane; q < c; q += 64) oa[k + q] = a[v[s0 + (c - 1 - q)]];
		k += c;
	}
}

__global__ void __launch_bounds__(256) rechain_gather_kernel(SeedChainBuffers B, const Anchor *src, const uint64_t *src_off)
{
	const int r = blockIdx.x;
	const uint64_t ao = B.a_off[r], so = src_off[r];
	const int64_t n = (int64_t)(B.a_off[r + 1] - ao);
	const uint64_t low_mask = (1ULL << (32 + B.rid_bits)) - 1ULL;
	for (int64_t i = threadIdx.x; i < n; i += 256) {
		const Anchor a = src[so + (uint64_t)i];
		B.sort_key_in[ao + (uint64_t)i] = (a.x >> 63) << (32 + B.rid_bits) | (a.x & low_mask);
		B.sort_val_in[ao + (uint64_t)i] = a.y;
	}
}

void launch_rechain_gather(const SeedChainBuffers &B, const Anchor *src, const uint64_t *src_off, void *stream)
{
	if (B.n_reads <= 0) return;
	hipLaunchKernelGGL(rechain_gather_kernel, dim3(B.n_reads), dim3(256), 0, (hipStream_t)stream, B, src, src_off);
	HIP_CHECK(hipGetLastError());
}

void launch_chain_backtrack(const SeedChainBuffers &B, const SeedChainParams &P, void *stream)
{
	const int max_drop = P.is_cdna ? INT32_MAX : P.bw;
	HIP_CHECK(hipMemsetAsync(B.bt_cursor, 0, 16, (hipStream_t)stream));
	hipLaunchKernelGGL(chain_backtrack_kernel, dim3(B.n_reads), dim3(64), 0, (hipStream_t)stream, B, P.min_cnt, P.min_chain_score, max_drop, P.rmq);
	HIP_CHECK(hipGetLastError());
}


}
```

### minimap2_amd/csrc/seed_chain_dev.hpp

```cpp
#pragma once
#include <cstdint>
#include <cstddef>
#include "types.hpp"
#include "backend.hpp"

namespace mm2amd {

struct DevIndex {
	const uint32_t *bucket_start;
	const uint64_t *keys;
	const uint32_t *val_off;
	const struct IdxSlot *slots;
	const struct IdxSlot *first;
	const uint64_t *pos;
	const uint32_t *S;
	int bucket_bits, key_shift;
	const int32_t *name_rank;
	const uint32_t *seq_len;
};

struct SeedChainBuffers {
	int n_reads;
	const uint64_t *seq_off;
	const char *ascii;
	uint8_t *qpool;
	const int32_t *name_lb, *name_eq;
	const int32_t *unit_first;
	const uint64_t *unit_off;
	const uint32_t *unit_cnt;
	uint32_t *mz_cnt;
	const uint64_t *mz_off;
	uint64_t *mz_x, *mz_y;
	uint32_t *sd_n, *sd_off, *sd_aoff, *sd_qpos, *sd_info;
	uint32_t *n_anchor, *n_minipos, *n_seedhit;
	int32_t *rep_len;
	const uint64_t *a_off;
	const uint64_t *mp_off;
	Anchor *anchors;
	uint64_t *sort_key_in, *sort_val_in;
	uint64_t *sort_key_out, *sort_val_out;
	uint32_t *tie_flag;
	uint32_t *tie_list, *tie_count;
	int rid_bits;
	uint64_t *mini_pos;
	int32_t *f, *p, *t;
	const uint32_t *pieces = nullptr;
	int n_pieces = 0, piece_len = 0;
	int rmq_rank_max = 256;
	int piece_dense = 0;
	unsigned long long *bt_cursor;
	Anchor *bt_out_a;
	uint64_t *bt_out_u;
	int32_t *bt_nu, *bt_nv;
	uint64_t *bt_aoff, *bt_uoff;
};

void launch_encode(const SeedChainBuffers &B, void *stream);
void launch_chain_rmq(const SeedChainBuffers &B, const SeedChainParams &P, void *stream);
void launch_sketch(const SeedChainBuffers &B, const SeedChainParams &P, int max_len, void *stream);
void launch_dust_filter(const SeedChainBuffers &B, void *stream);
void launch_seed_collect(const SeedChainBuffers &B, const DevIndex &I, const SeedChainParams &P, void *stream);
void launch_seed_expand(const SeedChainBuffers &B, const DevIndex &I, const SeedChainParams &P, void *stream);
class KernelProfiler;
constexpr int kAnchorSortClasses = 6;
int anchor_sort_class(uint64_t n_anchors, int rid_bits);
void launch_anchor_sort(const SeedChainBuffers &B, const DevIndex &I, const SeedChainParams &P, const uint32_t *d_list, const int *n_class, const double *anchors_in_class, void *stream,
                        KernelProfiler *kp);
void launch_chain_fill(const SeedChainBuffers &B, const SeedChainParams &P, void *stream);
void launch_chain_backtrack(const SeedChainBuffers &B, const SeedChainParams &P, void *stream);
void launch_rechain_gather(const SeedChainBuffers &B, const Anchor *src, const uint64_t *src_off, void *stream);

}
```

Measured before the change: 3.647.

## Prune anchors that cannot chain during sort, with adaptive redo fallback

Adds an anchor_sort_prune_kernel that sorts anchors and keeps only those that have neighbours inside the chaining window, recording a per-read kept count. Chain fill and backtrack then read that count, so they process fewer anchors. When a read's survivors overflow the kernel's LDS capacity, the read is queued for a full redo with the original sort kernel, which now walks a device-counted list. A host-side heuristic turns pruning off for the next 15 batches when more than half the reads need a redo. The aim is to cut DP work in the O(n·window) chain fill, at the cost of an extra pass, a redo launch and the risk of differing chains if the pruning test is wrong.

```diff
diff --git a/minimap2_amd/__init__.py b/minimap2_amd/__init__.py
--- a/minimap2_amd/__init__.py
+++ b/minimap2_amd/__init__.py
@@ -843,13 +843,14 @@
             self.free_raw(n_reg, reg)
 
     def last_stats(self):
-        v = (C.c_double * 40)()
-        k = lib().mm2amd_last_stats(v, 40)
+        v = (C.c_double * 48)()
+        k = lib().mm2amd_last_stats(v, 48)
         names = ["t_seed_chain", "t_host_pre", "t_plan", "t_ksw", "t_consume", "t_finish", "n_jobs", "n_rounds", "dp_cells", "dev_allocs", "pin_allocs",
                  "alloc_ns", "cpu_seed_chain", "cpu_host_pre", "cpu_plan", "cpu_ksw", "cpu_consume", "cpu_finish", "n_long_join_dev", "n_long_join_host",
                  "drv_cpu_seed_chain", "drv_cpu_host_pre", "drv_cpu_plan", "drv_cpu_ksw", "drv_cpu_consume", "drv_cpu_finish", "n_early_sub",
                  "n_region_reads_dev", "n_region_reads_host", "n_band128", "n_band256", "n_band_widened", "n_band_rectangle",
-                 "arena_dev_bytes", "arena_pin_bytes", "arena_dev_used", "arena_pin_used", "n_band512", "n_band_rectangle_big"]
+                 "arena_dev_bytes", "arena_pin_bytes", "arena_dev_used", "arena_pin_used", "n_band512", "n_band_rectangle_big",
+                 "n_anchors_prune_in", "n_anchors_prune_kept", "n_reads_prune_redo"]
         return dict(zip(names, list(v)[:k]))
 
 
diff --git a/minimap2_amd/csrc/backend_hip.cpp b/minimap2_amd/csrc/backend_hip.cpp
--- a/minimap2_amd/csrc/backend_hip.cpp
+++ b/minimap2_amd/csrc/backend_hip.cpp
@@ -39,12 +39,13 @@
 	DevBuf<uint32_t> d_sdust_list;
 	DevBuf<SdustCounters> d_sdust_cnt;
 	PinBuf<SdustCounters> h_sdust_cnt;
-	DevBuf<uint32_t> d_mz_cnt, d_sd_n, d_sd_off, d_sd_aoff, d_sd_qpos, d_sd_info, d_n_anchor, d_n_minipos, d_n_seedhit, d_tie;
+	DevBuf<uint32_t> d_mz_cnt, d_sd_n, d_sd_off, d_sd_aoff, d_sd_qpos, d_sd_info, d_n_anchor, d_n_minipos, d_n_seedhit, d_tie, d_nkept;
 	DevBuf<int32_t> d_rep_len, d_f, d_p, d_t;
 	DevBuf<Anchor> d_anchors;
 	DevBuf<uint8_t> d_tbytes;
 	DevBuf<uint32_t> d_sort_list;
 	PinBuf<uint32_t> h_sort_list;
+	DevBuf<Anchor> d_dump_anchors;
 	DevBuf<uint32_t> d_pieces;
 	PinBuf<uint32_t> h_pieces, h_lj_pieces;
 	DevBuf<Anchor> d_lj_out_a;
@@ -76,7 +77,7 @@
 	DevBuf<Anchor> d_bt_out_a;
 	DevBuf<uint64_t> d_bt_out_u, d_bt_aoff, d_bt_uoff;
 	DevBuf<int32_t> d_bt_nu, d_bt_nv;
-	PinBuf<uint32_t> h_na, h_nmp, h_dust_n, h_dust_s, h_dust_e, h_tie;
+	PinBuf<uint32_t> h_na, h_nmp, h_dust_n, h_dust_s, h_dust_e, h_tie, h_nkept;
 	std::vector<uint64_t> a_off, mp_off;
 	~Lane() { if (stream) (void)hipStreamDestroy(stream); }
 };
@@ -347,6 +348,16 @@
 		B.sort_key_in = ln.d_skey_in.p, B.sort_val_in = ln.d_sval_in.p, B.sort_key_out = ln.d_skey_out.p, B.sort_val_out = ln.d_sval_out.p, B.tie_flag = ln.d_tie.p;
 		B.tie_list = ln.d_tie.p + n, B.tie_count = ln.d_tie.p + 2 * n;
 		B.rid_bits = rid_bits_;
+		static const bool prune_env = !(getenv("MM2AMD_ANCHOR_PRUNE") && atoi(getenv("MM2AMD_ANCHOR_PRUNE")) == 0);
+		static const bool prune_adapt = !getenv("MM2AMD_PRUNE_BINS") && !getenv("MM2AMD_PRUNE_CAP");
+		const bool prune_can = prune_env && !P.rmq && !P.anchors_only && !has_pairs_ && !P.is_hpc && P.k < P.min_chain_score && !(P.flag & ref::F_HEAP_SORT) && !getenv("MM2AMD_SEED_DUMP");
+		const bool prune = prune_can && !(prune_adapt && prune_rest_.load() > 0 && prune_rest_.fetch_sub(1) > 0);
+		if (prune) {
+			ln.d_nkept.ensure(2 * n + 8);
+			B.n_kept = ln.d_nkept.p, B.redo_count = ln.d_nkept.p + n, B.redo_list = ln.d_nkept.p + n + 8;
+			static const int bins_env = getenv("MM2AMD_PRUNE_BINS") ? atoi(getenv("MM2AMD_PRUNE_BINS")) : 0, cap_env = getenv("MM2AMD_PRUNE_CAP") ? atoi(getenv("MM2AMD_PRUNE_CAP")) : 0;
+			B.prune_bins = bins_env, B.prune_cap = cap_env;
+		}
 		int n_class[kAnchorSortClasses] = { 0 }, class_first[kAnchorSortClasses + 1] = { 0 };
 		double a_class[kAnchorSortClasses] = { 0 };
 		for (size_t i = 0; i < n; ++i) if (h_na[i]) { const int c = anchor_sort_class(h_na[i], rid_bits_); ++n_class[c], a_class[c] += h_na[i]; }
@@ -362,6 +373,12 @@
 		B.a_off = ln.d_a_off.p, B.mp_off = ln.d_mp_off.p, B.anchors = ln.d_anchors.p, B.mini_pos = ln.d_minipos.p;
 		B.f = ln.d_f.p, B.p = ln.d_p.p, B.t = ln.d_t.p;
 		kp.begin(st); launch_seed_expand(B, I_, P, st); kp.end(st, "seed_expand_kernel", 24.0 * n_a);
+		const bool dump_full = prune && P.chain_dump && chain_dump_path();
+		if (dump_full) {
+			SeedChainBuffers Bd = B;
+			Bd.anchors = ln.d_dump_anchors.ensure(n_a + 1), Bd.n_kept = nullptr, Bd.redo_list = Bd.redo_count = nullptr;
+			launch_anchor_sort(Bd, I_, P, ln.d_sort_list.p, n_class, a_class, st, nullptr);
+		}
 		launch_anchor_sort(B, I_, P, ln.d_sort_list.p, n_class, a_class, st, &kp);
 		if (getenv("MM2AMD_TIE_COUNT")) {
 			std::vector<uint32_t> tf(n);
@@ -427,13 +444,13 @@
 		}
 		make_pieces(B, ln, ln.h_pieces, n, [&](size_t i) { return (uint64_t)h_na[i]; }, P.rmq ? rmq_piece_len() : fill_piece_len(), st);
 		if (P.rmq) { kp.begin(st); launch_chain_rmq(B, P, st); kp.end(st, "chain_rmq_kernel", 32.0 * n_a); }
-		else { kp.begin(st); launch_chain_fill(B, P, st); kp.end(st, "chain_fill_kernel", 24.0 * n_a); }
+		else { kp.begin(st); launch_chain_fill(B, P, st); kp.end(st, "chain_fill_kernel", prune ? 0.0 : 24.0 * n_a); }
 		B.pieces = nullptr, B.n_pieces = 0;
 		ln.d_bt_cursor.ensure(2), ln.d_bt_out_a.ensure(n_a + 1), ln.d_bt_out_u.ensure((P.min_cnt >= 2 ? n_a / 2 : n_a) + n + 1);
 		ln.d_bt_nu.ensure(n), ln.d_bt_nv.ensure(n), ln.d_bt_aoff.ensure(n), ln.d_bt_uoff.ensure(n);
 		B.bt_cursor = ln.d_bt_cursor.p, B.bt_out_a = ln.d_bt_out_a.p, B.bt_out_u = ln.d_bt_out_u.p;
 		B.bt_nu = ln.d_bt_nu.p, B.bt_nv = ln.d_bt_nv.p, B.bt_aoff = ln.d_bt_aoff.p, B.bt_uoff = ln.d_bt_uoff.p;
-		kp.begin(st); launch_chain_backtrack(B, P, st); kp.end(st, "chain_backtrack_kernel", 8.0 * n_a);
+		kp.begin(st); launch_chain_backtrack(B, P, st); kp.end(st, "chain_backtrack_kernel", prune ? 0.0 : 8.0 * n_a);
 		unsigned long long *h_cur = ln.h_cursor.ensure(2);
 		int32_t *h_nu = ln.h_nu.ensure(n), *h_nv = ln.h_nv.ensure(n);
 		uint64_t *h_aoff = ln.h_aoff.ensure(n), *h_uoff = ln.h_uoff.ensure(n);
@@ -445,6 +462,8 @@
 		HIP_CHECK(hipMemcpyAsync(h_aoff, ln.d_bt_aoff.p, n * 8, hipMemcpyDeviceToHost, st));
 		HIP_CHECK(hipMemcpyAsync(h_uoff, ln.d_bt_uoff.p, n * 8, hipMemcpyDeviceToHost, st));
 		if (h_tie) HIP_CHECK(hipMemcpyAsync(h_tie, ln.d_tie.p, n * 4, hipMemcpyDeviceToHost, st));
+		uint32_t *h_nkept = prune ? ln.h_nkept.ensure(2 * n + 8) : nullptr;
+		if (prune) HIP_CHECK(hipMemcpyAsync(h_nkept, ln.d_nkept.p, ((P.chain_dump && chain_dump_path() ? 2 * n : n) + 8) * 4, hipMemcpyDeviceToHost, st));
 		const bool lazy = P.lazy_chains != 0 && !P.anchors_only;
 		ln.rg_lazy = lazy;
 		int32_t *h_span = nullptr;
@@ -455,6 +474,18 @@
 		} else if (n_mp) HIP_CHECK(hipMemcpyAsync(hmp, ln.d_minipos.p, n_mp * 8, hipMemcpyDeviceToHost, st));
 		stream_wait(st);
 		Trace::get().add(lane_id, "gpu:expand..backtrack", tt, Trace::now()); tt = Trace::now();
+		if (prune) {
+			double kept_class[kAnchorSortClasses] = { 0 }, kept = 0;
+			unsigned long long n_redone = 0;
+			for (int c = 0; c + 1 < kAnchorSortClasses; ++c) n_redone += h_nkept[n + c];
+			for (size_t i = 0; i < n; ++i) if (h_na[i]) kept_class[anchor_sort_class(h_na[i], rid_bits_)] += h_nkept[i], kept += h_nkept[i];
+			size_t n_sorted = 0;
+			for (size_t i = 0; i < n; ++i) n_sorted += h_na[i] != 0;
+			if (prune_adapt && n_redone * 2 > n_sorted) prune_rest_.store(15);
+			prune_counters().n_in += n_a, prune_counters().n_kept += (unsigned long long)kept, prune_counters().n_redo += n_redone;
+			for (int c = 0; c + 1 < kAnchorSortClasses; ++c) if (kept_class[c] > 0) kp.add_bytes(kAnchorSortNames[c], 24.0 * kept_class[c]);
+			kp.add_bytes("chain_fill_kernel", 24.0 * kept), kp.add_bytes("chain_backtrack_kernel", 8.0 * kept);
+		}
 		const uint64_t n_v = h_cur[0], n_u = h_cur[1];
 		Anchor *ha = ln.h_anchors.ensure(n_v + 1);
 		uint64_t *hu = ln.h_u.ensure(n_u + 1);
@@ -473,14 +504,17 @@
 		stream_wait(st);
 		if (cdump) {
 			std::vector<Anchor> all(n_a + 1), bt(lazy ? n_v + 1 : 0);
-			if (n_a) HIP_CHECK(hipMemcpyAsync(all.data(), ln.d_anchors.p, n_a * sizeof(Anchor), hipMemcpyDeviceToHost, st));
+			if (n_a) HIP_CHECK(hipMemcpyAsync(all.data(), dump_full ? ln.d_dump_anchors.p : ln.d_anchors.p, n_a * sizeof(Anchor), hipMemcpyDeviceToHost, st));
 			if (lazy && n_v) HIP_CHECK(hipMemcpyAsync(bt.data(), ln.d_bt_out_a.p, n_v * sizeof(Anchor), hipMemcpyDeviceToHost, st));
 			stream_wait(st);
 			const Anchor *chained = lazy ? bt.data() : ha;
+			std::vector<bool> redone(n, false);
+			if (prune) for (int c = 0; c + 1 < kAnchorSortClasses; ++c) for (uint32_t q = 0; q < h_nkept[n + c]; ++q) redone[h_nkept[n + 8 + class_first[c] + q]] = true;
 			std::string txt;
 			for (size_t i = 0; i < n; ++i) {
 				ChainDumpBlock b = dump_block(i);
 				b.in = all.data() + a_off[i], b.n_in = (int64_t)(a_off[i + 1] - a_off[i]);
+				if (prune) b.n_kept = (int64_t)h_nkept[i], b.redone = redone[i];
 				b.handed_back = h_tie && h_tie[i];
 				if (!b.handed_back) b.u = hu + h_uoff[i], b.n_u = h_nu[i], b.a = chained + h_aoff[i], b.n_a = h_nv[i];
 				chain_dump_format(txt, P, b);
@@ -561,6 +595,7 @@
 		const uint64_t n_a2 = h_off[n2];
 		SeedChainBuffers B2 = ln.B;
 		B2.n_reads = (int)n2, B2.seq_off = nullptr, B2.mz_cnt = nullptr, B2.unit_first = nullptr;
+		B2.n_kept = nullptr, B2.redo_list = B2.redo_count = nullptr;
 		ln.d_lj_src.ensure(n2 + 1), ln.d_lj_out_a.ensure(n_a2 + 1);
 		HIP_CHECK(hipMemcpyAsync(ln.d_a_off.p, h_off, (n2 + 1) * 8, hipMemcpyHostToDevice, st));
 		HIP_CHECK(hipMemcpyAsync(ln.d_lj_src.p, h_src, n2 * 8, hipMemcpyHostToDevice, st));
@@ -986,6 +1021,7 @@
 	hipStream_t stream_ = nullptr;
 	int n_threads_ = 1, n_cu_ = 256, n_lanes_ = 1, rid_bits_ = 1, dev_ = 0, replica_ = 0;
 	std::atomic<int> active_lanes_{1};
+	std::atomic<int> prune_rest_{0};
 	DevIndex I_{};
 	DeviceIndexTables own_;
 	DeviceIndexTables *T_ = nullptr;
diff --git a/minimap2_amd/csrc/capi_kernels.cpp b/minimap2_amd/csrc/capi_kernels.cpp
--- a/minimap2_amd/csrc/capi_kernels.cpp
+++ b/minimap2_amd/csrc/capi_kernels.cpp
@@ -650,7 +650,8 @@
 	return which == 0 ? a.dev_allocs.load() : which == 1 ? a.pin_allocs.load() : which == 2 ? a.ns.load() : which == 3 ? (long long)b.n_band1.load() : which == 4 ? (long long)b.n_band2.load() :
 	       which == 5 ? (long long)b.n_widened.load() : which == 6 ? (long long)b.n_retried.load() :
 	       which == 7 ? (long long)dev_arena().held_bytes() : which == 8 ? (long long)pin_arena().held_bytes() : which == 9 ? (long long)dev_arena().used_bytes() : which == 10 ? (long long)pin_arena().used_bytes() :
-	       which == 11 ? (long long)b.n_band4.load() : (long long)b.n_retried_big.load();
+	       which == 11 ? (long long)b.n_band4.load() : which == 12 ? (long long)b.n_retried_big.load() :
+	       which == 13 ? (long long)prune_counters().n_in.load() : which == 14 ? (long long)prune_counters().n_kept.load() : (long long)prune_counters().n_redo.load();
 }
 
 void mm2amd_profile_enable(int on)
diff --git a/minimap2_amd/csrc/capi_map.cpp b/minimap2_amd/csrc/capi_map.cpp
--- a/minimap2_amd/csrc/capi_map.cpp
+++ b/minimap2_amd/csrc/capi_map.cpp
@@ -713,7 +713,8 @@
 	                     (double)s.n_region_reads_dev, (double)s.n_region_reads_host,
 	                     (double)mm2amd_alloc_counter(3), (double)mm2amd_alloc_counter(4), (double)mm2amd_alloc_counter(5), (double)mm2amd_alloc_counter(6),
 	                     (double)mm2amd_alloc_counter(7), (double)mm2amd_alloc_counter(8), (double)mm2amd_alloc_counter(9), (double)mm2amd_alloc_counter(10),
-	                     (double)mm2amd_alloc_counter(11), (double)mm2amd_alloc_counter(12) };
+	                     (double)mm2amd_alloc_counter(11), (double)mm2amd_alloc_counter(12),
+	                     (double)mm2amd_alloc_counter(13), (double)mm2amd_alloc_counter(14), (double)mm2amd_alloc_counter(15) };
 	int k = 0;
 	for (; k < n && k < (int)(sizeof a / sizeof a[0]); ++k) v[k] = a[k];
 	return k;
diff --git a/minimap2_amd/csrc/chain_dump.hpp b/minimap2_amd/csrc/chain_dump.hpp
--- a/minimap2_amd/csrc/chain_dump.hpp
+++ b/minimap2_amd/csrc/chain_dump.hpp
@@ -16,6 +16,8 @@
 	bool host = false, handed_back = false;
 	const Anchor *in = nullptr;
 	int64_t n_in = 0;
+	int64_t n_kept = -1;
+	bool redone = false;
 	const uint64_t *u = nullptr;
 	int32_t n_u = 0;
 	const Anchor *a = nullptr;
@@ -47,6 +49,8 @@
 	s += buf;
 	if (b.in) chain_dump_words(s, "IN", b.n_in, (const uint64_t *)b.in, 2 * b.n_in);
 	else s += "IN\t-\n";
+	static const bool kept_lines = getenv("MM2AMD_CHAIN_DUMP_KEPT") != nullptr;
+	if (kept_lines && b.n_kept >= 0) { snprintf(buf, sizeof(buf), "KP\t%lld\t%d\n", (long long)b.n_kept, b.redone ? 1 : 0); s += buf; }
 	int64_t n_a = 0;
 	for (int32_t k = 0; k < b.n_u; ++k) n_a += (int32_t)b.u[k];
 	if (n_a != b.n_a) { snprintf(buf, sizeof(buf), "ERR\tchains of %lld anchors, %lld anchors\n", (long long)n_a, (long long)b.n_a); s += buf; n_a = n_a < b.n_a ? n_a : b.n_a; }
diff --git a/minimap2_amd/csrc/hip_util.hpp b/minimap2_amd/csrc/hip_util.hpp
--- a/minimap2_amd/csrc/hip_util.hpp
+++ b/minimap2_amd/csrc/hip_util.hpp
@@ -71,6 +71,8 @@
 inline AllocStats &alloc_stats() { static AllocStats s; return s; }
 struct BandCounters { std::atomic<unsigned long long> n_band1{0}, n_band2{0}, n_band4{0}, n_widened{0}, n_retried{0}, n_retried_big{0}; };
 inline BandCounters &band_counters() { static BandCounters s; return s; }
+struct PruneCounters { std::atomic<unsigned long long> n_in{0}, n_kept{0}, n_redo{0}; };
+inline PruneCounters &prune_counters() { static PruneCounters s; return s; }
 
 class MemArena {
 public:
diff --git a/minimap2_amd/csrc/kernel_prof.hpp b/minimap2_amd/csrc/kernel_prof.hpp
--- a/minimap2_amd/csrc/kernel_prof.hpp
+++ b/minimap2_amd/csrc/kernel_prof.hpp
@@ -29,6 +29,7 @@
 		HIP_CHECK(hipEventRecord(p.e1, s));
 	}
 	void add_units(const char *name, double units) { if (enabled_flag()) stats_[name].units += units; }
+	void add_bytes(const char *name, double alg_bytes) { if (enabled_flag()) stats_[name].alg_bytes += alg_bytes; }
 	void collect()
 	{
 		for (Pending &p : pending_) {
diff --git a/minimap2_amd/csrc/seed_chain.hip b/minimap2_amd/csrc/seed_chain.hip
--- a/minimap2_amd/csrc/seed_chain.hip
+++ b/minimap2_amd/csrc/seed_chain.hip
@@ -1103,7 +1103,7 @@
 }
 
 template <int THREADS, int ROUNDS, bool IN_LDS>
-__global__ void __launch_bounds__(THREADS, (THREADS == 1024 && IN_LDS && ROUNDS <= 7) ? 8 : 4)  anchor_sort_kernel(SeedChainBuffers B, const uint32_t *list, int heap_sort)
+__global__ void __launch_bounds__(THREADS, (THREADS == 1024 && IN_LDS && ROUNDS <= 7) ? 8 : 4)  anchor_sort_kernel(SeedChainBuffers B, const uint32_t *list, const uint32_t *count, int heap_sort)
 {
 	MM2_DYN_LDS(uint64_t, as_lds);
 	__shared__ uint32_t tab[(THREADS / 64) * 256];
@@ -1113,12 +1113,16 @@
 	__shared__ uint32_t n_tied_s;
 	uint32_t *const cnt = tab, *const head = tab + 256, *const start = tab + 512;
 	const int32_t tid = (int32_t)threadIdx.x;
-	const int r = (int)list[blockIdx.x];
+	const uint32_t n_list = count ? *count : gridDim.x;
+	for (uint32_t li = blockIdx.x; li < n_list; li += gridDim.x) {
+	if (li != blockIdx.x) __syncthreads();
+	const int r = (int)list[li];
 	const uint64_t ao = B.a_off[r];
 	const int32_t n = (int32_t)(B.a_off[r + 1] - ao);
 	const uint64_t *kin = B.sort_key_in + ao, *vin = B.sort_val_in + ao;
 	Anchor *out = B.anchors + ao;
-	if (n == 0) return;
+	if (n == 0) continue;
+	if (B.n_kept && tid == 0) B.n_kept[r] = (uint32_t)n;
 	auto run = [&](auto s, TieFrame *stack, int stack_cap) {
 		for (int32_t i = tid; i < n; i += THREADS) s.set(i, kin[i], (uint32_t)i);
 		if (tid == 0) n_tied_s = 0;
@@ -1163,6 +1167,97 @@
 	else {
 		uint32_t *I = (uint32_t *)(B.sort_val_out + ao);
 		run(SplitStore{B.sort_key_out + ao, I, B.rid_bits}, (TieFrame *)(I + n), (int)((size_t)n * 4 / sizeof(TieFrame)));
+	}
+	}
+}
+
+__device__ __forceinline__ void chain_window(const SeedChainBuffers &B, const SeedChainParams &P, int r, int32_t *max_dist_x, int32_t *max_dist_y)
+{
+	chain_gaps(P, (int)(B.seq_off[r + 1] - B.seq_off[r]), max_dist_x, max_dist_y);
+	if (*max_dist_x < P.bw) *max_dist_x = P.bw;
+	if (*max_dist_y < P.bw && !P.is_cdna) *max_dist_y = P.bw;
+}
+
+template <int THREADS, int ROUNDS, int CAP>
+__global__ void __launch_bounds__(THREADS, THREADS == 1024 ? 8 : 4) anchor_sort_prune_kernel(SeedChainBuffers B, SeedChainParams P, const uint32_t *list, uint32_t *redo_list, uint32_t *redo_count)
+{
+	constexpr int S_MAX = CAP * 3 / 8, NW = THREADS / 64;
+	constexpr uint32_t W_MAX = (uint32_t)(CAP - S_MAX) * 2u;
+	static_assert(S_MAX <= THREADS * ROUNDS, "a wavefront's segment of the survivors fits its rounds");
+	MM2_DYN_LDS(uint64_t, as_lds);
+	__shared__ uint32_t tab[NW * 256];
+	__shared__ uint32_t dig_tot[256], wave_tot[NW];
+	__shared__ uint32_t n_surv_s, redo_s;
+	const int32_t tid = (int32_t)threadIdx.x;
+	const int lane = tid & 63, w = tid >> 6;
+	const int r = (int)list[blockIdx.x];
+	const uint64_t ao = B.a_off[r];
+	const int32_t n = (int32_t)(B.a_off[r + 1] - ao);
+	const uint64_t *kin = B.sort_key_in + ao, *vin = B.sort_val_in + ao;
+	Anchor *out = B.anchors + ao;
+	if (n == 0) return;
+	int32_t max_dist, max_dist_y;
+	chain_window(B, P, r, &max_dist, &max_dist_y);
+	int s = 0;
+	while (s < 31 && (1u << s) < (uint32_t)max_dist + 1u) ++s;
+	const uint32_t s_cap = B.prune_cap > 0 && B.prune_cap < S_MAX ? (uint32_t)B.prune_cap : (uint32_t)S_MAX;
+	const uint32_t bins = B.prune_bins > 0 && (uint32_t)B.prune_bins < W_MAX * 16u ? (uint32_t)B.prune_bins : W_MAX * 16u;
+	uint32_t *const bt = (uint32_t *)(as_lds + S_MAX);
+	auto bin_of = [&](uint64_t q) { return (uint32_t)((uint64_t)(((uint32_t)q ^ (uint32_t)(q >> 32) * 0x85ebca6bu) * 0x9e3779b1u) * bins >> 32); };
+	for (uint32_t i = (uint32_t)tid; i < (bins + 15u) / 16u; i += THREADS) bt[i] = 0;
+	if (tid == 0) n_surv_s = 0, redo_s = 0;
+	__syncthreads();
+	for (int32_t i = tid; i < n; i += THREADS) {
+		const uint32_t b = bin_of(kin[i] >> s), sh = (b & 15u) * 2u;
+		const uint32_t old = atomicOr(&bt[b >> 4], 1u << sh);
+		if (old >> sh & 1u) atomicOr(&bt[b >> 4], 2u << sh);
+	}
+	__syncthreads();
+	for (int32_t base = 0; base < n; base += THREADS) {
+		const int32_t i = base + tid;
+		uint64_t key = 0;
+		bool keep = false;
+		if (i < n) {
+			key = kin[i];
+			const uint64_t q = key >> s;
+			const uint32_t b = bin_of(q), lo = bin_of(q - 1), hi = bin_of(q + 1);
+			keep = (bt[b >> 4] >> ((b & 15u) * 2u) & 2u) != 0 || (bt[lo >> 4] >> ((lo & 15u) * 2u) & 1u) != 0 || (bt[hi >> 4] >> ((hi & 15u) * 2u) & 1u) != 0;
+		}
+		const unsigned long long m = __ballot(keep);
+		uint32_t first = 0;
+		if (lane == 0 && m) first = atomicAdd(&n_surv_s, (uint32_t)__popcll(m));
+		first = (uint32_t)__shfl((int)first, 0, 64);
+		if (keep) { const uint32_t slot = first + (uint32_t)popc_below(m, lane); if (slot < s_cap) as_lds[slot] = key << AS_IDX_BITS | (uint64_t)(uint32_t)i; }
+	}
+	__syncthreads();
+	const uint32_t n_surv = n_surv_s;
+	if (n_surv > s_cap) { if (tid == 0) redo_list[atomicAdd(redo_count, 1u)] = (uint32_t)r; return; }
+	if (n_surv == 0) { if (tid == 0) B.n_kept[r] = 0; return; }
+	const int32_t m = (int32_t)n_surv;
+	lds_radix_sort<THREADS, ROUNDS>(as_lds, m, 33 + B.rid_bits, tab, dig_tot);
+	auto near = [&](uint64_t a, uint64_t b) { return a >> 32 == b >> 32 && b - a <= (uint64_t)(int64_t)max_dist; };
+	uint32_t n_out = 0;
+	for (int32_t base = 0; base < m; base += THREADS) {
+		const int32_t i = base + tid;
+		uint64_t e = 0, k = 0;
+		bool keep = false;
+		if (i < m) {
+			e = as_lds[i], k = e >> AS_IDX_BITS;
+			if (i > 0) { const uint64_t kp = as_lds[i - 1] >> AS_IDX_BITS; keep = near(kp, k); if (kp == k) redo_s = 1u; }
+			if (i + 1 < m) keep = keep || near(k, as_lds[i + 1] >> AS_IDX_BITS);
+		}
+		const unsigned long long mk = __ballot(keep);
+		if (lane == 0) wave_tot[w] = (uint32_t)__popcll(mk);
+		__syncthreads();
+		uint32_t before = 0, total = 0;
+		for (int w2 = 0; w2 < NW; ++w2) { const uint32_t t = wave_tot[w2]; if (w2 < w) before += t; total += t; }
+		if (keep) { Anchor a; a.x = key_to_x(k, B.rid_bits), a.y = vin[(uint32_t)e & ((1u << AS_IDX_BITS) - 1u)]; out[n_out + before + (uint32_t)popc_below(mk, lane)] = a; }
+		n_out += total;
+		__syncthreads();
+	}
+	if (tid == 0) {
+		if (redo_s) redo_list[atomicAdd(redo_count, 1u)] = (uint32_t)r;
+		else B.n_kept[r] = n_out;
 	}
 }
 
@@ -1256,6 +1351,7 @@
 }
 
 const int kAnchorSortCap[kAnchorSortClasses] = { 1024, 2048, 4096, 7168, AS_LDS_MAX, 0 };
+const char *const kAnchorSortNames[kAnchorSortClasses] = { "anchor_sort_kernel[n1k]", "anchor_sort_kernel[n2k]", "anchor_sort_kernel[n4k]", "anchor_sort_kernel[n7k]", "anchor_sort_kernel[n10k]", "anchor_sort_kernel[global]" };
 
 int anchor_sort_class(uint64_t n_anchors, int rid_bits)
 {
@@ -1273,7 +1369,7 @@
 	KernelProfiler none;
 	if (!kp) kp = &none;
 	HIP_CHECK(hipMemsetAsync(B.tie_flag, 0, (size_t)B.n_reads * 4, s));
-	static const char *kNames[kAnchorSortClasses] = { "anchor_sort_kernel[n1k]", "anchor_sort_kernel[n2k]", "anchor_sort_kernel[n4k]", "anchor_sort_kernel[n7k]", "anchor_sort_kernel[n10k]", "anchor_sort_kernel[global]" };
+	const char *const *kNames = kAnchorSortNames;
 	if (n_class[4] > 0) HIP_CHECK(hipFuncSetAttribute((const void *)anchor_sort_kernel<1024, 10, true>, hipFuncAttributeMaxDynamicSharedMemorySize, AS_LDS_MAX * 8));
 	static const bool no_replay = getenv("MM2AMD_SORT_NO_REPLAY") != nullptr;
 	const bool walk_only = getenv("MM2AMD_NO_TWO_BUCKET") != nullptr;
@@ -1282,22 +1378,57 @@
 	const bool no_split = getenv("MM2AMD_TIE_NO_STRAND_SPLIT") != nullptr;
 	const int heap = ((P.flag & ref::F_HEAP_SORT) || no_replay ? 1 : 0) | (walk_only ? 2 : 0) | (replay_inline ? 0 : 4) | (no_tape ? 8 : 0) | (no_split ? 16 : 0);
 	if (heap & 4) HIP_CHECK(hipMemsetAsync(B.tie_count, 0, 4, s));
+	const bool prune = B.n_kept != nullptr;
+	if (prune) {
+		HIP_CHECK(hipMemsetAsync(B.n_kept, 0, (size_t)B.n_reads * 4, s));
+		HIP_CHECK(hipMemsetAsync(B.redo_count, 0, 4 * kAnchorSortClasses, s));
+		if (n_class[4] > 0) HIP_CHECK(hipFuncSetAttribute((const void *)anchor_sort_prune_kernel<1024, 4, AS_LDS_MAX>, hipFuncAttributeMaxDynamicSharedMemorySize, AS_LDS_MAX * 8));
+	}
 	int first = 0;
 	for (int c = 0; c < kAnchorSortClasses; first += n_class[c], ++c) {
 		if (n_class[c] == 0) continue;
 		kp->begin(s);
 		const size_t lds = (size_t)kAnchorSortCap[c] * 8;
 		const dim3 grid(n_class[c]);
-		if (c == 0) hipLaunchKernelGGL((anchor_sort_kernel<256, 4, true>), grid, dim3(256), lds, s, B, d_list + first, heap);
-		else if (c == 1) hipLaunchKernelGGL((anchor_sort_kernel<256, 8, true>), grid, dim3(256), lds, s, B, d_list + first, heap);
-		else if (c == 2) hipLaunchKernelGGL((anchor_sort_kernel<512, 8, true>), grid, dim3(512), lds, s, B, d_list + first, heap);
-		else if (c == 3) hipLaunchKernelGGL((anchor_sort_kernel<1024, 7, true>), grid, dim3(1024), lds, s, B, d_list + first, heap);
-		else if (c == 4) hipLaunchKernelGGL((anchor_sort_kernel<1024, 10, true>), grid, dim3(1024), lds, s, B, d_list + first, heap);
-		else hipLaunchKernelGGL((anchor_sort_kernel<1024, 1, false>), grid, dim3(1024), 0, s, B, d_list + first, heap);
+		const uint32_t *none_counted = nullptr;
+		if (prune && c + 1 < kAnchorSortClasses) {
+			if (c == 0) hipLaunchKernelGGL((anchor_sort_prune_kernel<256, 2, 1024>), grid, dim3(256), lds, s, B, P, d_list + first, B.redo_list + first, B.redo_count + c);
+			else if (c == 1) hipLaunchKernelGGL((anchor_sort_prune_kernel<256, 3, 2048>), grid, dim3(256), lds, s, B, P, d_list + first, B.redo_list + first, B.redo_count + c);
+			else if (c == 2) hipLaunchKernelGGL((anchor_sort_prune_kernel<512, 3, 4096>), grid, dim3(512), lds, s, B, P, d_list + first, B.redo_list + first, B.redo_count + c);
+			else if (c == 3) hipLaunchKernelGGL((anchor_sort_prune_kernel<1024, 3, 7168>), grid, dim3(1024), lds, s, B, P, d_list + first, B.redo_list + first, B.redo_count + c);
+			else hipLaunchKernelGGL((anchor_sort_prune_kernel<1024, 4, AS_LDS_MAX>), grid, dim3(1024), lds, s, B, P, d_list + first, B.redo_list + first, B.redo_count + c);
+			kp->end(s, kNames[c], 16.0 * anchors_in_class[c]);
+			HIP_CHECK(hipGetLastError());
+			continue;
+		}
+		if (c == 0) hipLaunchKernelGGL((anchor_sort_kernel<256, 4, true>), grid, dim3(256), lds, s, B, d_list + first, none_counted, heap);
+		else if (c == 1) hipLaunchKernelGGL((anchor_sort_kernel<256, 8, true>), grid, dim3(256), lds, s, B, d_list + first, none_counted, heap);
+		else if (c == 2) hipLaunchKernelGGL((anchor_sort_kernel<512, 8, true>), grid, dim3(512), lds, s, B, d_list + first, none_counted, heap);
+		else if (c == 3) hipLaunchKernelGGL((anchor_sort_kernel<1024, 7, true>), grid, dim3(1024), lds, s, B, d_list + first, none_counted, heap);
+		else if (c == 4) hipLaunchKernelGGL((anchor_sort_kernel<1024, 10, true>), grid, dim3(1024), lds, s, B, d_list + first, none_counted, heap);
+		else hipLaunchKernelGGL((anchor_sort_kernel<1024, 1, false>), grid, dim3(1024), 0, s, B, d_list + first, none_counted, heap);
 		kp->end(s, kNames[c], 32.0 * anchors_in_class[c]);
 		HIP_CHECK(hipGetLastError());
 	}
 	const int n_lds = n_class[0] + n_class[1] + n_class[2] + n_class[3] + n_class[4];
+	if (prune && n_lds > 0) {
+		kp->begin(s);
+		if (n_class[4] > 0) HIP_CHECK(hipFuncSetAttribute((const void *)anchor_sort_kernel<1024, 10, true>, hipFuncAttributeMaxDynamicSharedMemorySize, AS_LDS_MAX * 8));
+		int at = 0;
+		for (int c = 0; c + 1 < kAnchorSortClasses; at += n_class[c], ++c) {
+			if (n_class[c] == 0) continue;
+			const size_t lds = (size_t)kAnchorSortCap[c] * 8;
+			const dim3 grid(std::min(n_class[c], 1024));
+			const uint32_t *rl = B.redo_list + at, *rc = B.redo_count + c;
+			if (c == 0) hipLaunchKernelGGL((anchor_sort_kernel<256, 4, true>), grid, dim3(256), lds, s, B, rl, rc, heap);
+			else if (c == 1) hipLaunchKernelGGL((anchor_sort_kernel<256, 8, true>), grid, dim3(256), lds, s, B, rl, rc, heap);
+			else if (c == 2) hipLaunchKernelGGL((anchor_sort_kernel<512, 8, true>), grid, dim3(512), lds, s, B, rl, rc, heap);
+			else if (c == 3) hipLaunchKernelGGL((anchor_sort_kernel<1024, 7, true>), grid, dim3(1024), lds, s, B, rl, rc, heap);
+			else hipLaunchKernelGGL((anchor_sort_kernel<1024, 10, true>), grid, dim3(1024), lds, s, B, rl, rc, heap);
+			HIP_CHECK(hipGetLastError());
+		}
+		kp->end(s, "anchor_sort_kernel[redo]", 0.0);
+	}
 	if ((heap & 4) && !(heap & 1) && n_lds > 0) {
 		kp->begin(s);
 		HIP_CHECK(hipFuncSetAttribute((const void *)anchor_sort_ties_kernel, hipFuncAttributeMaxDynamicSharedMemorySize, (int)AST_LDS_BYTES));
@@ -1383,15 +1514,13 @@
 	uint64_t *const rx = s_x[wave], *const ry = s_y[wave];
 	int32_t *const rf = s_f[wave], *const rp = s_p[wave], *const rt = s_t[wave];
 	const Anchor *a = B.anchors + B.a_off[r];
-	const int64_t n_all = (int64_t)(B.a_off[r + 1] - B.a_off[r]);
+	const int64_t n_all = B.n_kept ? (int64_t)B.n_kept[r] : (int64_t)(B.a_off[r + 1] - B.a_off[r]);
 	int32_t *f = B.f + B.a_off[r], *p = B.p + B.a_off[r], *t = B.t + B.a_off[r];
 	int32_t max_dist_x, max_dist_y;
-	chain_gaps(P, (int)(B.seq_off[r + 1] - B.seq_off[r]), &max_dist_x, &max_dist_y);
+	chain_window(B, P, r, &max_dist_x, &max_dist_y);
 	max_dist_x = __builtin_amdgcn_readfirstlane(max_dist_x), max_dist_y = __builtin_amdgcn_readfirstlane(max_dist_y);
 	const int n_seg = PAIRS ? B.unit_first[r + 1] - B.unit_first[r] : 1;
 	const int32_t bw = P.bw;
-	if (max_dist_x < bw) max_dist_x = bw;
-	if (max_dist_y < bw && !P.is_cdna) max_dist_y = bw;
 	int64_t lo = 0, n = n_all;
 	if (B.pieces) chain_piece_bounds(a, n_all, (int64_t)B.pieces[2 * w + 1], (int64_t)B.piece_len, max_dist_x, lane, &lo, &n);
 	if (lo >= n) return;
@@ -1987,7 +2116,7 @@
 	const int lane = threadIdx.x;
 	const int r = blockIdx.x;
 	const uint64_t ao = B.a_off[r];
-	const int32_t n = (int32_t)(B.a_off[r + 1] - ao);
+	const int32_t n = B.n_kept ? (int32_t)B.n_kept[r] : (int32_t)(B.a_off[r + 1] - ao);
 	const Anchor *a = B.anchors + ao;
 	const int32_t *f = B.f + ao, *p = B.p + ao;
 	int32_t *t = B.t + ao;
diff --git a/minimap2_amd/csrc/seed_chain_dev.hpp b/minimap2_amd/csrc/seed_chain_dev.hpp
--- a/minimap2_amd/csrc/seed_chain_dev.hpp
+++ b/minimap2_amd/csrc/seed_chain_dev.hpp
@@ -42,6 +42,9 @@
 	uint32_t *tie_flag;
 	uint32_t *tie_list, *tie_count;
 	int rid_bits;
+	uint32_t *n_kept = nullptr;
+	uint32_t *redo_list = nullptr, *redo_count = nullptr;
+	int prune_bins = 0, prune_cap = 0;
 	uint64_t *mini_pos;
 	int32_t *f, *p, *t;
 	const uint32_t *pieces = nullptr;
@@ -63,6 +66,7 @@
 void launch_seed_expand(const SeedChainBuffers &B, const DevIndex &I, const SeedChainParams &P, void *stream);
 class KernelProfiler;
 constexpr int kAnchorSortClasses = 6;
+extern const char *const kAnchorSortNames[kAnchorSortClasses];
 int anchor_sort_class(uint64_t n_anchors, int rid_bits);
 void launch_anchor_sort(const SeedChainBuffers &B, const DevIndex &I, const SeedChainParams &P, const uint32_t *d_list, const int *n_class, const double *anchors_in_class, void *stream,
                         KernelProfiler *kp);
```

Measured after the change: 3.764, median of 6. 1.03x the previous value.
